# tkwa/iit

Hardware: AMD Instinct MI355X
Metric: IIT (base,source) intervened pairs/sec, IOI GPT-2-small, IOI_ModelPair IIT+strict+behavior step (higher is better)
Workload: dtype bf16; 1 GPU; model=gpt2-small 12L/768d/12H (TL GPT-2 cfg, LNPre, gelu_new, V=50257), global_batch=256, seq_len=16, parallelism=dp1, engine=native, graphs=True

## Files before the change

### csrc/ioi_hl.hip

```cpp
#include "common.h"

namespace {

constexpr int MAXS = 64;

__global__ __launch_bounds__(64) void ioi_hl_label_kernel(const long* __restrict__ base, const long* __restrict__ src,
                                                          const float* __restrict__ name_table, int table_n, int B,
                                                          int S, int V, int node, long* __restrict__ label) {
  __shared__ long tok_s[MAXS], dtok_s[MAXS], key_s[2 * MAXS];
  __shared__ float d_s[2 * MAXS];
  const int b = blockIdx.x, lane = threadIdx.x;
  const long* tb = base + (long)b * S;
  const long* ts = src + (long)b * S;
  const long* tok = (node == 0 || node == 3) ? ts : tb;
  const long* dtok = (node == 1 || node == 2) ? ts : tok;
  if (lane < S) {
    tok_s[lane] = tok[lane];
    dtok_s[lane] = dtok[lane];
  }
  __syncthreads();
  if (lane < S) {
    int dup = -1;
    for (int j = 0; j < lane; ++j)
      if (dtok_s[j] == dtok_s[lane]) dup = j;
    const long inh = dup == -1 ? -1 : (node == 1 ? tok_s[lane] : dtok_s[lane]);
    const long v = tok_s[lane];
    key_s[lane] = v;
    d_s[lane] = (v >= 0 && v < table_n && name_table[v] != 0.f) ? 10.f : 0.f;
    key_s[S + lane] = inh != -1 ? inh : (long)(V - 1);
    d_s[S + lane] = inh != -1 ? -15.f : 0.f;
  }
  __syncthreads();
  const int n = 2 * S;
  float my_val = -INFINITY, my_zero_key = INFINITY;
  long my_key = -1;
  for (int e = lane; e < n; e += 64) {
    const long k = key_s[e];
    float sum = 0.f;
    for (int f = 0; f < n; ++f)
      if (key_s[f] == k) sum += d_s[f];
    if (sum > my_val || (sum == my_val && k < my_key)) {
      my_val = sum;
      my_key = k;
    }
    if (sum == 0.f) my_zero_key = fminf(my_zero_key, (float)k);
  }
  float untouched = INFINITY;
  for (int u = lane; u <= n; u += 64) {
    bool hit = false;
    for (int f = 0; f < n; ++f) hit |= key_s[f] == (long)u;
    if (!hit) untouched = fminf(untouched, (float)u);
  }
  for (int off = 32; off > 0; off >>= 1) {
    const float ov = __shfl_xor(my_val, off);
    const long ok = __shfl_xor(my_key, off);
    if (ov > my_val || (ov == my_val && ok >= 0 && (my_key < 0 || ok < my_key))) {
      my_val = ov;
      my_key = ok;
    }
    my_zero_key = fminf(my_zero_key, __shfl_xor(my_zero_key, off));
    untouched = fminf(untouched, __shfl_xor(untouched, off));
  }
  if (lane == 0) {
    long out;
    if (my_val > 0.f) {
      out = my_key;
    } else {
      out = (long)untouched;
      if (my_zero_key < untouched) out = (long)my_zero_key;
    }
    label[b] = out;
  }
}

}

IIT_EXPORT int iit_ioi_hl_label(const void* base, const void* src, const float* name_table, int table_n, int B, int S,
                                int V, int node, void* label, void* stream) {
  if (S < 1 || S > MAXS || node < 0 || node > 3 || V <= 2 * S) return (int)hipErrorInvalidValue;
  hipLaunchKernelGGL(ioi_hl_label_kernel, dim3(B), dim3(64), 0, (hipStream_t)stream,
                     (const long*)base, (const long*)src, name_table, table_n, B, S, V, node, (long*)label);
  return hipGetLastError();
}
```

### csrc/kernels.hip

```cpp
#include "common.h"
#include <stdlib.h>

__global__ void embed_pos_fwd_kernel(const long* __restrict__ tok, const float* __restrict__ WE,
                                     const float* __restrict__ Wpos, float* __restrict__ out, int T, int S, int d) {
  const int t = blockIdx.x;
  if (t >= T) return;
  const long v = tok[t];
  const int s = t % S;
  const float4* e = (const float4*)(WE + v * (long)d);
  const float4* p = (const float4*)(Wpos + (long)s * d);
  float4* o = (float4*)(out + (long)t * d);
  for (int i = threadIdx.x; i < d / 4; i += blockDim.x) {
    float4 a = e[i], b = p[i];
    o[i] = make_float4(a.x + b.x, a.y + b.y, a.z + b.z, a.w + b.w);
  }
}

__global__ void embed_pos_fwd_scalar_kernel(const long* __restrict__ tok, const float* __restrict__ WE,
                                            const float* __restrict__ Wpos, float* __restrict__ out, int T, int S,
                                            int d) {
  const int t = blockIdx.x;
  if (t >= T) return;
  const float* e = WE + tok[t] * (long)d;
  const float* p = Wpos + (long)(t % S) * d;
  float* o = out + (long)t * d;
  for (int i = threadIdx.x; i < d; i += blockDim.x) o[i] = e[i] + p[i];
}

IIT_EXPORT int iit_embed_pos_fwd(const long* tok, const float* WE, const float* Wpos, float* out, int T, int S,
                                 int d, void* stream) {
  if (d % 4 == 0 && ((((uintptr_t)WE) | ((uintptr_t)Wpos) | ((uintptr_t)out)) & 15) == 0)
    hipLaunchKernelGGL(embed_pos_fwd_kernel, dim3(T), dim3(64), 0, (hipStream_t)stream, tok, WE, Wpos, out, T, S, d);
  else
    hipLaunchKernelGGL(embed_pos_fwd_scalar_kernel, dim3(T), dim3(256), 0, (hipStream_t)stream, tok, WE, Wpos, out,
                       T, S, d);
  return hipGetLastError();
}

__global__ void embed_bwd_kernel(const long* __restrict__ tok, const float* __restrict__ g, float* __restrict__ dWE,
                                 int T, int d) {
  const int t = blockIdx.x;
  const long v = tok[t];
  for (int i = threadIdx.x; i < d; i += blockDim.x) atomicAdd(dWE + v * (long)d + i, g[(long)t * d + i]);
}

constexpr int EB = 32;
__global__ __launch_bounds__(256) void embed_bwd_pos_kernel(const long* __restrict__ tok, const float* __restrict__ g,
                                                            float* __restrict__ dWE, int B, int S, int d) {
  const int s = blockIdx.x, c = blockIdx.y * 256 + threadIdx.x, b0 = blockIdx.z * EB;
  if (c >= d) return;
  const int b1 = min(B, b0 + EB);
  long cur = -1;
  float acc = 0.f;
  for (int bb = b0; bb < b1; bb += 8) {
    long vv[8];
    float xx[8];
#pragma unroll
    for (int k = 0; k < 8; ++k) {
      const int b = bb + k;
      vv[k] = -1;
      xx[k] = 0.f;
      if (b < b1) {
        const long t = (long)b * S + s;
        vv[k] = tok[t];
        xx[k] = g[t * d + c];
      }
    }
#pragma unroll
    for (int k = 0; k < 8; ++k) {
      if (vv[k] < 0) break;
      if (vv[k] != cur) {
        if (cur >= 0) atomicAdd(dWE + cur * (long)d + c, acc);
        cur = vv[k];
        acc = xx[k];
      } else {
        acc += xx[k];
      }
    }
  }
  if (cur >= 0) atomicAdd(dWE + cur * (long)d + c, acc);
}

__global__ __launch_bounds__(256) void pos_bwd_kernel(const float* __restrict__ g, float* __restrict__ dWpos, int B,
                                                      int S, int d) {
  __shared__ float part[4][64 * 4];
  const int s = blockIdx.x, w = threadIdx.x >> 6, lane = threadIdx.x & 63;
  const int c = blockIdx.y * 256 + lane * 4;
  float4 acc = make_float4(0.f, 0.f, 0.f, 0.f);
  if (c < d)
#pragma unroll 8
    for (int b = w; b < B; b += 4) {
      const float4 v = *(const float4*)(g + ((long)b * S + s) * d + c);
      acc.x += v.x; acc.y += v.y; acc.z += v.z; acc.w += v.w;
    }
  *(float4*)&part[w][lane * 4] = acc;
  __syncthreads();
  const int col = blockIdx.y * 256 + threadIdx.x;
  if (col < d)
    dWpos[(long)s * d + col] += part[0][threadIdx.x] + part[1][threadIdx.x] + part[2][threadIdx.x] + part[3][threadIdx.x];
}

__global__ void pos_bwd_scalar_kernel(const float* __restrict__ g, float* __restrict__ dWpos, int B, int S, int d) {
  const int s = blockIdx.x;
  for (int i = threadIdx.x; i < d; i += blockDim.x) {
    float acc = 0.f;
    for (int b = 0; b < B; ++b) acc += g[((long)b * S + s) * d + i];
    dWpos[(long)s * d + i] += acc;
  }
}

IIT_EXPORT int iit_embed_pos_bwd(const long* tok, const float* g, float* dWE, float* dWpos, int B, int S, int d,
                                 void* stream) {
  hipStream_t st = (hipStream_t)stream;
  static const bool pos_major = [] {
    const char* e = getenv("IIT_EMBED_BWD_POS");
    return !(e && e[0] == '0');
  }();
  if (dWE && pos_major)
    hipLaunchKernelGGL(embed_bwd_pos_kernel, dim3(S, (d + 255) / 256, (B + EB - 1) / EB), dim3(256), 0, st, tok, g,
                       dWE, B, S, d);
  else if (dWE)
    hipLaunchKernelGGL(embed_bwd_kernel, dim3(B * S), dim3(256), 0, st, tok, g, dWE, B * S, d);
  if (dWpos) {
    if (d % 4 == 0 && (((uintptr_t)g) & 15) == 0)
      hipLaunchKernelGGL(pos_bwd_kernel, dim3(S, (d + 255) / 256), dim3(256), 0, st, g, dWpos, B, S, d);
    else
      hipLaunchKernelGGL(pos_bwd_scalar_kernel, dim3(S), dim3(256), 0, st, g, dWpos, B, S, d);
  }
  return hipGetLastError();
}

constexpr size_t kAttnSmallLdsMax = 160 * 1024;
__global__ __launch_bounds__(64) void attn_small_fwd_kernel(const __bf16* __restrict__ qkv, __bf16* __restrict__ z,
                                                            float* __restrict__ lse, const __bf16* __restrict__ zsrc,
                                                            unsigned long long head_mask, int B, int S, int H, int dh,
                                                            long ld_qkv, long ld_z, long ld_src, float scale, int causal) {
  extern __shared__ __attribute__((aligned(16))) float sm[];
  const int bh = blockIdx.x, b = bh / H, h = bh % H;
  const int lane = threadIdx.x;
  const int HD = H * dh;
  const long row0 = (long)b * S;
  if ((head_mask >> h) & 1ull) {
    for (int i = lane; i < S * dh; i += 64) {
      const int s = i / dh, e = i % dh;
      z[(row0 + s) * ld_z + h * dh + e] = zsrc[(row0 + s) * ld_src + h * dh + e];
    }
    if (lse)
      for (int s = lane; s < S; s += 64) lse[(long)bh * S + s] = 0.f;
    return;
  }
  const int P = dh + 1;
  float* q = sm;
  float* k = q + S * P;
  float* v = k + S * P;
  float* pr = v + S * P;
  for (int i = lane; i < S * dh; i += 64) {
    const int s = i / dh, e = i % dh;
    const __bf16* r = qkv + (row0 + s) * ld_qkv + h * dh + e;
    q[s * P + e] = bf2f(r[0]);
    k[s * P + e] = bf2f(r[HD]);
    v[s * P + e] = bf2f(r[2 * HD]);
  }
  __syncthreads();
  const int SP = S + 1;
  for (int i = lane; i < S * S; i += 64) {
    const int qi = i / S, kj = i % S;
    float acc = -INFINITY;
    if (!causal || kj <= qi) {
      acc = 0.f;
      for (int e = 0; e < dh; ++e) acc += q[qi * P + e] * k[kj * P + e];
      acc *= scale;
    }
    pr[qi * SP + kj] = acc;
  }
  __syncthreads();
  for (int qi = lane; qi < S; qi += 64) {
    float m = -INFINITY;
    for (int kj = 0; kj < S; ++kj) m = fmaxf(m, pr[qi * SP + kj]);
    float sum = 0.f;
    for (int kj = 0; kj < S; ++kj) {
      const float e = pr[qi * SP + kj] == -INFINITY ? 0.f : __expf(pr[qi * SP + kj] - m);
      pr[qi * SP + kj] = e;
      sum += e;
    }
    const float inv = sum > 0.f ? 1.f / sum : 0.f;
    for (int kj = 0; kj < S; ++kj) pr[qi * SP + kj] *= inv;
    if (lse) lse[(long)bh * S + qi] = m + __logf(sum);
  }
  __syncthreads();
  for (int i = lane; i < S * dh; i += 64) {
    const int qi = i / dh, e = i % dh;
    float acc = 0.f;
    const int kmax = causal ? qi + 1 : S;
    for (int kj = 0; kj < kmax; ++kj) acc += pr[qi * SP + kj] * v[kj * P + e];
    z[(row0 + qi) * ld_z + h * dh + e] = f2bf(acc);
  }
}

IIT_EXPORT int iit_attn_small_fwd(const void* qkv, void* z, float* lse, const void* zsrc, unsigned long long head_mask,
                                  int B, int S, int H, int dh, long ld_qkv, long ld_z, long ld_src, float scale,
                                  int causal, void* stream) {
  if (S > 64 || dh > 128) return (int)hipErrorInvalidValue;
  const size_t lds = (size_t)(3 * S * (dh + 1) + S * (S + 1)) * sizeof(float);
  if (lds > kAttnSmallLdsMax) return (int)hipErrorInvalidValue;
  hipLaunchKernelGGL(attn_small_fwd_kernel, dim3(B * H), dim3(64), lds, (hipStream_t)stream, (const __bf16*)qkv,
                     (__bf16*)z, lse, (const __bf16*)zsrc, head_mask, B, S, H, dh, ld_qkv, ld_z, ld_src, scale, causal);
  return hipGetLastError();
}

__global__ __launch_bounds__(64) void attn_small_bwd_kernel(const __bf16* __restrict__ qkv, const __bf16* __restrict__ dz,
                                                            const float* __restrict__ lse, __bf16* __restrict__ dqkv,
                                                            unsigned long long head_mask, int B, int S, int H, int dh,
                                                            long ld_qkv, long ld_dz, float scale, int causal) {
  extern __shared__ __attribute__((aligned(16))) float sm[];
  const int bh = blockIdx.x, b = bh / H, h = bh % H;
  const int lane = threadIdx.x;
  const int HD = H * dh;
  const long row0 = (long)b * S;
  if ((head_mask >> h) & 1ull) {
    for (int i = lane; i < S * dh; i += 64) {
      const int s = i / dh, e = i % dh;
      __bf16* r = dqkv + (row0 + s) * ld_qkv + h * dh + e;
      r[0] = f2bf(0.f);
      r[HD] = f2bf(0.f);
      r[2 * HD] = f2bf(0.f);
    }
    return;
  }
  const int P = dh + 1, SP = S + 1;
  float* q = sm;
  float* k = q + S * P;
  float* v = k + S * P;
  float* g = v + S * P;
  float* pm = g + S * P;
  float* ds = pm + S * SP;
  for (int i = lane; i < S * dh; i += 64) {
    const int s = i / dh, e = i % dh;
    const __bf16* r = qkv + (row0 + s) * ld_qkv + h * dh + e;
    q[s * P + e] = bf2f(r[0]);
    k[s * P + e] = bf2f(r[HD]);
    v[s * P + e] = bf2f(r[2 * HD]);
    g[s * P + e] = bf2f(dz[(row0 + s) * ld_dz + h * dh + e]);
  }
  __syncthreads();
  for (int i = lane; i < S * S; i += 64) {
    const int qi = i / S, kj = i % S;
    float p = 0.f, dp = 0.f;
    if (!causal || kj <= qi) {
      float sc = 0.f;
      for (int e = 0; e < dh; ++e) sc += q[qi * P + e] * k[kj * P + e];
      p = __expf(sc * scale - lse[(long)bh * S + qi]);
      for (int e = 0; e < dh; ++e) dp += g[qi * P + e] * v[kj * P + e];
    }
    pm[qi * SP + kj] = p;
    ds[qi * SP + kj] = dp;
  }
  __syncthreads();
  for (int qi = lane; qi < S; qi += 64) {
    float dsum = 0.f;
    for (int kj = 0; kj < S; ++kj) dsum += pm[qi * SP + kj] * ds[qi * SP + kj];
    for (int kj = 0; kj < S; ++kj) ds[qi * SP + kj] = pm[qi * SP + kj] * (ds[qi * SP + kj] - dsum) * scale;
  }
  __syncthreads();
  for (int i = lane; i < S * dh; i += 64) {
    const int s = i / dh, e = i % dh;
    float dq = 0.f, dk = 0.f, dv = 0.f;
    for (int j = 0; j < S; ++j) {
      dq += ds[s * SP + j] * k[j * P + e];
      dk += ds[j * SP + s] * q[j * P + e];
      dv += pm[j * SP + s] * g[j * P + e];
    }
    __bf16* r = dqkv + (row0 + s) * ld_qkv + h * dh + e;
    r[0] = f2bf(dq);
    r[HD] = f2bf(dk);
    r[2 * HD] = f2bf(dv);
  }
}

IIT_EXPORT int iit_attn_small_bwd(const void* qkv, const void* dz, const float* lse, void* dqkv,
                                  unsigned long long head_mask, int B, int S, int H, int dh, long ld_qkv, long ld_dz,
                                  float scale, int causal, void* stream) {
  if (S > 64 || dh > 128) return (int)hipErrorInvalidValue;
  const size_t lds = (size_t)(4 * S * (dh + 1) + 2 * S * (S + 1)) * sizeof(float);
  if (lds > kAttnSmallLdsMax) return (int)hipErrorInvalidValue;
  hipLaunchKernelGGL(attn_small_bwd_kernel, dim3(B * H), dim3(64), lds, (hipStream_t)stream, (const __bf16*)qkv,
                     (const __bf16*)dz, lse, (__bf16*)dqkv, head_mask, B, S, H, dh, ld_qkv, ld_dz, scale, causal);
  return hipGetLastError();
}

__device__ __forceinline__ void online_add(float& m, float& s, int& mi, float v, int i) {
  if (v > m) {
    s = s * __expf(m - v) + 1.f;
    m = v;
    mi = i;
  } else if (v != -INFINITY) {
    s += __expf(v - m);
  }
}

__device__ __forceinline__ void online_merge(float& m, float& s, int& mi, float om, float os, int oi) {
  if (om > m || (om == m && oi < mi)) {
    s = os + (m == -INFINITY ? 0.f : s * __expf(m - om));
    m = om;
    mi = oi;
  } else {
    s += (om == -INFINITY ? 0.f : os * __expf(om - m));
  }
}

__global__ __launch_bounds__(1024) void ce_fwd_kernel(const float* __restrict__ logits, long ld, const long* __restrict__ labels,
                                                      float* __restrict__ loss, float* __restrict__ lse_out,
                                                      long* __restrict__ amax, int V) {
  __shared__ float sm_m[16], sm_s[16];
  __shared__ int sm_i[16];
  const int row = blockIdx.x, tid = threadIdx.x, lane = tid & 63, w = tid >> 6;
  const float* x = logits + (long)row * ld;
  float m = -INFINITY, s = 0.f;
  int mi = 0x7fffffff;
  int head = 0;
  if ((((uintptr_t)x) & 15) == 0) {
    const int v4 = V / 4;
    for (int i = tid; i < v4; i += 1024) {
      const float4 q = ((const float4*)x)[i];
      online_add(m, s, mi, q.x, 4 * i);
      online_add(m, s, mi, q.y, 4 * i + 1);
      online_add(m, s, mi, q.z, 4 * i + 2);
      online_add(m, s, mi, q.w, 4 * i + 3);
    }
    head = v4 * 4;
  }
  for (int i = head + tid; i < V; i += 1024) online_add(m, s, mi, x[i], i);
#pragma unroll
  for (int o = 32; o > 0; o >>= 1) {
    const float om = __shfl_xor(m, o, 64), os = __shfl_xor(s, o, 64);
    const int oi = __shfl_xor(mi, o, 64);
    online_merge(m, s, mi, om, os, oi);
  }
  if (lane == 0) { sm_m[w] = m; sm_s[w] = s; sm_i[w] = mi; }
  __syncthreads();
  if (tid == 0) {
    for (int j = 1; j < 16; ++j) online_merge(m, s, mi, sm_m[j], sm_s[j], sm_i[j]);
    const float l = m + __logf(s);
    if (lse_out) lse_out[row] = l;
    if (loss && labels) loss[row] = l - x[labels[row]];
    if (amax) amax[row] = mi;
  }
}

IIT_EXPORT int iit_ce_fwd(const float* logits, long ld, const long* labels, float* loss, float* lse, long* amax, int R,
                          int V, void* stream) {
  hipLaunchKernelGGL(ce_fwd_kernel, dim3(R), dim3(1024), 0, (hipStream_t)stream, logits, ld, labels, loss, lse, amax, V);
  return hipGetLastError();
}

template <typename OUT>
__global__ __launch_bounds__(256) void ce_bwd_kernel(const float* __restrict__ logits, long ld, const long* __restrict__ labels,
                                                     const float* __restrict__ lse, const float* __restrict__ gscale,
                                                     float inv_rows, OUT* __restrict__ out, long ld_out, int V,
                                                     __bf16* __restrict__ out16) {
  const int row = blockIdx.y;
  const int i = blockIdx.x * 256 + threadIdx.x;
  if (i >= ld_out) return;
  float v = 0.f;
  if (i < V) {
    const float p = __expf(logits[(long)row * ld + i] - lse[row]);
    v = (p - (i == labels[row] ? 1.f : 0.f)) * gscale[0] * inv_rows;
  }
  out[(long)row * ld_out + i] = (OUT)v;
  if (out16) out16[(long)row * ld_out + i] = f2bf(v);
}

IIT_EXPORT int iit_ce_bwd(const float* logits, long ld, const long* labels, const float* lse, const float* gscale,
                          float inv_rows, void* out, long ld_out, int R, int V, int out_bf16, void* out16,
                          void* stream) {
  dim3 grid((unsigned)((ld_out + 255) / 256), R);
  if (out_bf16)
    hipLaunchKernelGGL(ce_bwd_kernel<__bf16>, grid, dim3(256), 0, (hipStream_t)stream, logits, ld, labels, lse, gscale,
                       inv_rows, (__bf16*)out, ld_out, V, (__bf16*)nullptr);
  else
    hipLaunchKernelGGL(ce_bwd_kernel<float>, grid, dim3(256), 0, (hipStream_t)stream, logits, ld, labels, lse, gscale,
                       inv_rows, (float*)out, ld_out, V, (__bf16*)out16);
  return hipGetLastError();
}

template <bool VEC>
__global__ __launch_bounds__(256) void ce_bwd16_kernel(const float* __restrict__ logits, long ld,
                                                       const long* __restrict__ labels, const float* __restrict__ lse,
                                                       const float* __restrict__ gscale, float inv_rows,
                                                       __bf16* __restrict__ out16, long ld_out, int V) {
  const int row = blockIdx.y;
  const int c0 = (blockIdx.x * 256 + threadIdx.x) * 8;
  if (c0 >= ld_out) return;
  const float* x = logits + (long)row * ld;
  const float l = lse[row], gs = gscale[0];
  const long lab = labels[row];
  float v[8];
  if (VEC && c0 + 8 <= V) {
    const float4 a = *(const float4*)(x + c0), b = *(const float4*)(x + c0 + 4);
    v[0] = a.x; v[1] = a.y; v[2] = a.z; v[3] = a.w; v[4] = b.x; v[5] = b.y; v[6] = b.z; v[7] = b.w;
  } else {
#pragma unroll
    for (int e = 0; e < 8; ++e) v[e] = c0 + e < V ? x[c0 + e] : 0.f;
  }
  bf16x8 o;
#pragma unroll
  for (int e = 0; e < 8; ++e) {
    const int i = c0 + e;
    float g = 0.f;
    if (i < V) {
      const float p = __expf(v[e] - l);
      g = (p - (i == lab ? 1.f : 0.f)) * gs * inv_rows;
    }
    o[e] = f2bf(g);
  }
  *(bf16x8*)(out16 + (long)row * ld_out + c0) = o;
}

IIT_EXPORT int iit_ce_bwd16(const float* logits, long ld, const long* labels, const float* lse, const float* gscale,
                            float inv_rows, void* out16, long ld_out, int R, int V, void* stream) {
  if (R <= 0 || V <= 0 || ld < V || ld_out < V || ld_out % 8 || ((uintptr_t)out16 & 15)) return (int)hipErrorInvalidValue;
  dim3 grid((unsigned)((ld_out / 8 + 255) / 256), R);
  const bool vec = (((uintptr_t)logits | (uintptr_t)(ld * 4)) & 15) == 0;
  if (vec)
    hipLaunchKernelGGL(ce_bwd16_kernel<true>, grid, dim3(256), 0, (hipStream_t)stream, logits, ld, labels, lse, gscale,
                       inv_rows, (__bf16*)out16, ld_out, V);
  else
    hipLaunchKernelGGL(ce_bwd16_kernel<false>, grid, dim3(256), 0, (hipStream_t)stream, logits, ld, labels, lse,
                       gscale, inv_rows, (__bf16*)out16, ld_out, V);
  return hipGetLastError();
}

struct Span {
  long start4;
  long local4;
  int len4;
  int pad;
};

__global__ __launch_bounds__(256) void sumsq_span_kernel(const float* __restrict__ g, const Span* __restrict__ spans,
                                                         int nspans, float* __restrict__ part, int do_norm,
                                                         int* __restrict__ step, float* __restrict__ gsq) {
  __shared__ float sm[4];
  if (blockIdx.x == 0 && threadIdx.x == 0 && step) step[0] += 1;
  float s = 0.f;
  if (gsq && blockIdx.x == 0 && threadIdx.x < 64) {
    s = gsq[threadIdx.x];
    gsq[threadIdx.x] = 0.f;
  }
  if (!do_norm) return;
  const float4* g4 = (const float4*)g;
  for (int e = blockIdx.x; e < nspans; e += gridDim.x) {
    const Span sp = spans[e];
    for (int i = threadIdx.x; i < sp.len4; i += 256) {
      const float4 v = g4[sp.local4 + i];
      s += (v.x * v.x + v.y * v.y) + (v.z * v.z + v.w * v.w);
    }
  }
  s = wave_sum(s);
  if ((threadIdx.x & 63) == 0) sm[threadIdx.x >> 6] = s;
  __syncthreads();
  if (threadIdx.x == 0) part[blockIdx.x] = sm[0] + sm[1] + sm[2] + sm[3];
}

template <bool NT, int U>
__global__ __launch_bounds__(256) void adam_span_kernel(float* __restrict__ p, const float* __restrict__ g,
                                                        float* __restrict__ m, float* __restrict__ v,
                                                        __bf16* __restrict__ mirror, const Span* __restrict__ spans,
                                                        int nspans, const float* __restrict__ part, int nparts,
                                                        float clip, float lr, float b1, float b2, float eps, float wd,
                                                        const float* __restrict__ hyper, int* __restrict__ step,
                                                        int* __restrict__ skipped) {
  if (hyper) {
    lr = hyper[0];
    b1 = hyper[1];
    b2 = hyper[2];
    eps = hyper[3];
    wd = hyper[4];
  }
  __shared__ float coef_s;
  __shared__ int bad_s;
  if (threadIdx.x < 64) {
    float s = 0.f;
    if (clip > 0.f || skipped)
      for (int i = threadIdx.x; i < nparts; i += 64) s += part[i];
    s = wave_sum(s);
    if (threadIdx.x == 0) {
      coef_s = clip > 0.f ? fminf(1.f, clip / (sqrtf(s) + 1e-6f)) : 1.f;
      bad_s = skipped != nullptr && !isfinite(s);
    }
  }
  __syncthreads();
  if (bad_s) {
    if (blockIdx.x == 0 && threadIdx.x == 0) {
      step[0] -= 1;
      skipped[0] += 1;
    }
    return;
  }
  const float coef = coef_s;
  const float t = (float)step[0];
  const float bc1 = 1.f - powf(b1, t);
  const float bc2_sqrt = sqrtf(1.f - powf(b2, t));
  const float stepsz = lr / bc1;
  const float4* g4 = (const float4*)g;
  float4* p4 = (float4*)p;
  float4* m4 = (float4*)m;
  float4* v4 = (float4*)v;
  for (int e = blockIdx.x; e < nspans; e += gridDim.x) {
    const Span sp = spans[e];
    for (int j0 = threadIdx.x; j0 < sp.len4; j0 += 256 * U) {
      float4 gg[U], pp[U], mm[U], vv[U];
#pragma unroll
      for (int u = 0; u < U; ++u) {
        const int j = j0 + u * 256;
        if (j < sp.len4) {
          const long i = sp.start4 + j;
          const long li = sp.local4 + j;
          pp[u] = p4[i];
          if (NT) {
            gg[u] = __builtin_bit_cast(float4, __builtin_nontemporal_load((const f32x4*)g4 + li));
            mm[u] = __builtin_bit_cast(float4, __builtin_nontemporal_load((const f32x4*)m4 + li));
            vv[u] = __builtin_bit_cast(float4, __builtin_nontemporal_load((const f32x4*)v4 + li));
          } else {
            gg[u] = g4[li];
            mm[u] = m4[li];
            vv[u] = v4[li];
          }
        }
      }
#pragma unroll
      for (int u = 0; u < U; ++u) {
        const int j = j0 + u * 256;
        if (j >= sp.len4) break;
        const long i = sp.start4 + j;
        const long li = sp.local4 + j;
        float* gs = (float*)&gg[u];
        float* ps = (float*)&pp[u];
        float* ms = (float*)&mm[u];
        float* vs = (float*)&vv[u];
#pragma unroll
        for (int k = 0; k < 4; ++k) {
          float gr = gs[k] * coef;
          if (wd != 0.f) gr += wd * ps[k];
          ms[k] = b1 * ms[k] + (1.f - b1) * gr;
          vs[k] = b2 * vs[k] + (1.f - b2) * gr * gr;
          ps[k] -= stepsz * ms[k] / (sqrtf(vs[k]) / bc2_sqrt + eps);
        }
        p4[i] = pp[u];
        if (NT) {
          __builtin_nontemporal_store(__builtin_bit_cast(f32x4, mm[u]), (f32x4*)m4 + li);
          __builtin_nontemporal_store(__builtin_bit_cast(f32x4, vv[u]), (f32x4*)v4 + li);
        } else {
          m4[li] = mm[u];
          v4[li] = vv[u];
        }
        if (mirror) {
          bf16x4 o = {f2bf(ps[0]), f2bf(ps[1]), f2bf(ps[2]), f2bf(ps[3])};
          ((bf16x4*)mirror)[i] = o;
        }
      }
    }
  }
}

IIT_EXPORT int iit_adam_flat(float* p, float* g, float* m, float* v, void* mirror, const void* spans, int nspans,
                             float* part, int nparts, float clip, float lr, float b1, float b2, float eps, float wd,
                             const float* hyper, int* step, int* skipped, const void* sq_spans, int n_sq_spans,
                             float* gsq, void* stream) {
  hipStream_t s = (hipStream_t)stream;
  const bool norm = clip > 0.f || skipped != nullptr;
  const Span* sp = (const Span*)spans;
  const Span* ssp = sq_spans ? (const Span*)sq_spans : sp;
  hipLaunchKernelGGL(sumsq_span_kernel, dim3(norm ? nparts : 1), dim3(256), 0, s, g, ssp,
                     sq_spans ? n_sq_spans : nspans, part, (int)norm, step, gsq);
  static const int max_blocks = [] {
    const char* e = getenv("IIT_ADAM_MAX_BLOCKS");
    return e ? atoi(e) : 65536;
  }();
  const int blocks = min(nspans, max_blocks);
  static const int nt = [] {
    const char* e = getenv("IIT_ADAM_NT");
    return e ? atoi(e) : 1;
  }();
  static const int unroll = [] {
    const char* e = getenv("IIT_ADAM_UNROLL");
    return e ? atoi(e) : 4;
  }();
#define ADAM_LAUNCH(NT_, U_)                                                                                        \
  hipLaunchKernelGGL((adam_span_kernel<NT_, U_>), dim3(blocks), dim3(256), 0, s, p, g, m, v, (__bf16*)mirror, sp, \
                     nspans, part, nparts, clip, lr, b1, b2, eps, wd, hyper, step, skipped)
  if (nt) {
    if (unroll >= 4) ADAM_LAUNCH(true, 4);
    else if (unroll == 2) ADAM_LAUNCH(true, 2);
    else ADAM_LAUNCH(true, 1);
  } else {
    if (unroll >= 4) ADAM_LAUNCH(false, 4);
    else if (unroll == 2) ADAM_LAUNCH(false, 2);
    else ADAM_LAUNCH(false, 1);
  }
#undef ADAM_LAUNCH
  return hipGetLastError();
}

IIT_EXPORT int iit_adam_span_size() { return (int)sizeof(Span); }

__global__ __launch_bounds__(256) void sumsq_2d_kernel(const float* __restrict__ c, long ldc, int M, int N,
                                                       float* __restrict__ gsq) {
  __shared__ float sm[4];
  const int chunks = (N + 2047) / 2048;
  float s = 0.f;
  for (long it = blockIdx.x; it < (long)M * chunks; it += gridDim.x) {
    const int r = (int)(it / chunks), c0 = (int)(it % chunks) * 2048;
    const float* row = c + (long)r * ldc;
    float v[8];
#pragma unroll
    for (int k = 0; k < 8; ++k) {
      const int j = c0 + k * 256 + threadIdx.x;
      v[k] = j < N ? row[j] : 0.f;
    }
#pragma unroll
    for (int k = 0; k < 8; ++k) s += v[k] * v[k];
  }
  s = wave_sum(s);
  if ((threadIdx.x & 63) == 0) sm[threadIdx.x >> 6] = s;
  __syncthreads();
  if (threadIdx.x == 0) atomicAdd(gsq + (blockIdx.x & 63), (sm[0] + sm[1]) + (sm[2] + sm[3]));
}

IIT_EXPORT int iit_sumsq_2d(const float* c, long ldc, int M, int N, float* gsq, void* stream) {
  const long items = (long)M * ((N + 2047) / 2048);
  hipLaunchKernelGGL(sumsq_2d_kernel, dim3((unsigned)(items < 2048 ? items : 2048)), dim3(256), 0,
                     (hipStream_t)stream, c, ldc, M, N, gsq);
  return hipGetLastError();
}

IIT_EXPORT int iit_sumsq_spans(const float* g, const void* spans, int nspans, float* part, int nparts, int do_norm,
                               int* step, void* stream) {
  hipLaunchKernelGGL(sumsq_span_kernel, dim3(do_norm ? nparts : 1), dim3(256), 0, (hipStream_t)stream, g,
                     (const Span*)spans, nspans, part, do_norm, step, (float*)nullptr);
  return hipGetLastError();
}

IIT_EXPORT int iit_adam_spans(float* p, const float* g, float* m, float* v, void* mirror, const void* spans,
                              int nspans, const float* total, float clip, float lr, float b1, float b2, float eps,
                              float wd, const float* hyper, int* step, int* skipped, void* stream) {
  const int blocks = max(1, min(nspans, 65536));
  hipLaunchKernelGGL((adam_span_kernel<true, 2>), dim3(blocks), dim3(256), 0, (hipStream_t)stream, p, g, m, v,
                     (__bf16*)mirror, (const Span*)spans, nspans, total, 1, clip, lr, b1, b2, eps, wd, hyper, step,
                     skipped);
  return hipGetLastError();
}

struct ShadowDesc {
  const float* src;
  __bf16* dst;
  int rows, cols;
  long ld;
  int heads;
  int transpose;
  long src_hs, dst_hs;
};

__global__ __launch_bounds__(256) void shadow_refresh_kernel(const ShadowDesc* __restrict__ descs) {
  __shared__ float tile[32][33];
  const ShadowDesc d = descs[blockIdx.y];
  if (!d.transpose) {
    const long total = (long)d.heads * d.rows;
    for (long r = blockIdx.x; r < total; r += gridDim.x) {
      const int h = (int)(r / d.rows), i = (int)(r % d.rows);
      const float* s = d.src + h * d.src_hs + (long)i * d.cols;
      __bf16* o = d.dst + h * d.dst_hs + (long)i * d.ld;
      const bool vec = ((((uintptr_t)s) & 15) == 0) && ((((uintptr_t)o) & 7) == 0);
      if (vec) {
        const int c4 = d.cols / 4;
        for (int j = threadIdx.x; j < c4; j += 256) {
          const float4 v = ((const float4*)s)[j];
          bf16x4 b = {f2bf(v.x), f2bf(v.y), f2bf(v.z), f2bf(v.w)};
          *(bf16x4*)(o + 4 * j) = b;
        }
        for (int j = c4 * 4 + threadIdx.x; j < d.cols; j += 256) o[j] = f2bf(s[j]);
      } else {
        for (int j = threadIdx.x; j < d.cols; j += 256) o[j] = f2bf(s[j]);
      }
    }
    return;
  }
  const int tiles_c = (d.cols + 31) / 32;
  const int ntiles = tiles_c * ((d.rows + 31) / 32);
  const int tx = threadIdx.x & 31, ty = threadIdx.x >> 5;
  for (int t = blockIdx.x; t < ntiles; t += gridDim.x) {
    const int r0 = (t / tiles_c) * 32, c0 = (t % tiles_c) * 32;
    {
      for (int i = ty; i < 32; i += 8) {
        const int r = r0 + i, c = c0 + tx;
        tile[i][tx] = (r < d.rows && c < d.cols) ? d.src[(long)r * d.cols + c] : 0.f;
      }
      __syncthreads();
      for (int i = ty; i < 32; i += 8) {
        const int c = c0 + i, r = r0 + tx;
        if (r < d.rows && c < d.cols) d.dst[(long)c * d.ld + r] = f2bf(tile[tx][i]);
      }
      __syncthreads();
    }
  }
}

IIT_EXPORT int iit_shadow_refresh(const void* descs, int n, void* stream) {
  if (n <= 0) return 0;
  hipLaunchKernelGGL(shadow_refresh_kernel, dim3(512, n), dim3(256), 0, (hipStream_t)stream, (const ShadowDesc*)descs);
  return hipGetLastError();
}

IIT_EXPORT int iit_shadow_desc_size() { return (int)sizeof(ShadowDesc); }

template <bool F32>
__global__ __launch_bounds__(256) void colsum_kernel(const void* __restrict__ x, long ld, float* __restrict__ out, int T, int N) {
  __shared__ float part[4][64];
  const int c = threadIdx.x & 63, w = threadIdx.x >> 6;
  const int n = blockIdx.x * 64 + c;
  const int t0 = blockIdx.y * 64;
  float s = 0.f;
  if (n < N) {
#pragma unroll 4
    for (int i = 0; i < 16; ++i) {
      const int t = t0 + w + 4 * i;
      if (t < T) s += F32 ? ((const float*)x)[(long)t * ld + n] : bf2f(((const __bf16*)x)[(long)t * ld + n]);
    }
  }
  part[w][c] = s;
  __syncthreads();
  if (w == 0 && n < N) atomicAdd(out + n, part[0][c] + part[1][c] + part[2][c] + part[3][c]);
// ... 410 lines not shown
```

### iit_amd/data/iit_dataset.py

```python
from __future__ import annotations

from typing import Iterator, Optional, Sequence, Tuple

import numpy as np
import torch
from torch.utils.data import DataLoader, Dataset, Subset

from ..config import DEVICE


def _gather_fn(ds):
    if hasattr(ds, "gather"):
        return ds.gather
    if isinstance(ds, Subset):
        inner = _gather_fn(ds.dataset)
        if inner is None:
            return None
        table = torch.as_tensor(list(ds.indices), dtype=torch.long)
        cache = {}

        def f(idx, _inner=inner, _table=table, _cache=cache):
            dev = idx.device
            t = _cache.get(dev)
            if t is None:
                t = _cache[dev] = _table.to(dev)
            return _inner(t.index_select(0, idx))

        return f
    return None


def _dist_info() -> Tuple[int, int]:
    if torch.distributed.is_available() and torch.distributed.is_initialized():
        return torch.distributed.get_rank(), torch.distributed.get_world_size()
    return 0, 1


def loader_epoch_permutation(n: int) -> torch.Tensor:
    torch.empty((), dtype=torch.int64).random_()
    seed = int(torch.empty((), dtype=torch.int64).random_().item())
    g = torch.Generator()
    g.manual_seed(seed)
    return torch.randperm(n, generator=g)


class IITDataset(Dataset):
    def __init__(self, base_data, ablation_data, seed: int = 0, every_combination: bool = False, device=DEVICE):
        self.base_data = base_data
        self.ablation_data = ablation_data
        self.seed = seed
        self.every_combination = every_combination
        self.device = device
        self._pair_table: Optional[Tuple[np.ndarray, np.ndarray]] = None

    def pair_indices(self, index: int) -> Tuple[int, int]:
        if self.every_combination:
            n_abl = len(self.ablation_data)
            return index // n_abl, index % n_abl
        rng = np.random.default_rng(self.seed * 1000000 + index)
        base = rng.choice(len(self.base_data))
        abl = rng.choice(len(self.ablation_data))
        return int(base), int(abl)

    def pair_table(self) -> Tuple[np.ndarray, np.ndarray]:
        if self._pair_table is None:
            n = len(self)
            if self.every_combination:
                idx = np.arange(n)
                n_abl = len(self.ablation_data)
                self._pair_table = (idx // n_abl, idx % n_abl)
            else:
                pairs = np.array([self.pair_indices(i) for i in range(n)], dtype=np.int64).reshape(n, 2)
                self._pair_table = (pairs[:, 0], pairs[:, 1])
        return self._pair_table

    def __getitem__(self, index):
        b, a = self.pair_indices(index)
        return self.base_data[b], self.ablation_data[a]

    def __len__(self) -> int:
        if self.every_combination:
            return len(self.base_data) * len(self.ablation_data)
        return len(self.base_data)

    @staticmethod
    def get_encoded_input_from_torch_input(xy, device=DEVICE):
        x, y, iv = zip(*xy)
        stack = lambda seq: torch.stack([torch.as_tensor(s).to(device) for s in seq])
        return stack(x), stack(y), stack(iv)

    @staticmethod
    def collate_fn(batch, device=DEVICE):
        base, abl = zip(*batch)
        return (IITDataset.get_encoded_input_from_torch_input(base, device),
                IITDataset.get_encoded_input_from_torch_input(abl, device))

    def supports_device_loader(self) -> bool:
        return _gather_fn(self.base_data) is not None and _gather_fn(self.ablation_data) is not None

    def make_loader(self, batch_size: int, num_workers: int = 0, shuffle: bool = True, fast: Optional[bool] = None):
        if fast is None:
            fast = self.supports_device_loader()
        if fast:
            return DeviceIITLoader(self, batch_size, shuffle=shuffle)
        return DataLoader(self, batch_size=batch_size, shuffle=shuffle, num_workers=num_workers,
                          collate_fn=lambda b: self.collate_fn(b, self.device))


class DeviceIITLoader:

    def __init__(self, dataset: IITDataset, batch_size: int, shuffle: bool = True, drop_last: bool = False,
                 device=None):
        self.dataset = dataset
        self.batch_size = batch_size
        self.shuffle = shuffle
        self.drop_last = drop_last
        self.rank, self.world = _dist_info()
        self.device = torch.device(device) if device is not None else torch.device(dataset.device)
        self._base_gather = _gather_fn(dataset.base_data)
        self._abl_gather = _gather_fn(dataset.ablation_data)
        self._unique = isinstance(dataset, IITUniqueDataset)
        self._tables = None

    def _device_tables(self):
        if self._tables is None:
            if self._unique:
                self._tables = (None, None)
            else:
                b, a = self.dataset.pair_table()
                self._tables = (torch.as_tensor(b).to(self.device), torch.as_tensor(a).to(self.device))
        return self._tables

    @property
    def global_batch(self) -> int:
        return self.batch_size * self.world

    def __len__(self) -> int:
        n = len(self.dataset)
        gb = self.global_batch
        if self.drop_last or (self.world > 1 and 0 < n % gb < self.world):
            return n // gb
        return (n + gb - 1) // gb

    def __iter__(self) -> Iterator:
        n = len(self.dataset)
        perm = loader_epoch_permutation(n) if self.shuffle else torch.arange(n)
        if self.device.type == "cuda":
            perm = perm.pin_memory().to(self.device, non_blocking=True)
        else:
            perm = perm.to(self.device)
        base_t, abl_t = self._device_tables()
        gb = self.global_batch
        for start in range(0, n, gb):
            chunk = perm[start:start + gb]
            if chunk.numel() < gb and self.drop_last:
                break
            if self.world > 1:
                if chunk.numel() < self.world:
                    break
                chunk = torch.tensor_split(chunk, self.world)[self.rank]
            if self._unique:
                yield self._base_gather(chunk)
            else:
                yield (self._base_gather(base_t.index_select(0, chunk)),
                       self._abl_gather(abl_t.index_select(0, chunk)))


class IITUniqueDataset(IITDataset):

    def __getitem__(self, index):
        return self.base_data[index]

    def __len__(self) -> int:
        return len(self.base_data)

    @staticmethod
    def collate_fn(batch, device=DEVICE):
        return IITDataset.get_encoded_input_from_torch_input(batch, device)

    def supports_device_loader(self) -> bool:
        return _gather_fn(self.base_data) is not None

    def make_loader(self, batch_size: int, num_workers: int = 0, shuffle: bool = True, fast: Optional[bool] = None):
        if fast is None:
            fast = self.supports_device_loader()
        if fast:
            return DeviceIITLoader(self, batch_size, shuffle=shuffle)
        return DataLoader(self, batch_size=batch_size, shuffle=shuffle, num_workers=num_workers,
                          collate_fn=lambda b: self.collate_fn(b, self.device))


def train_test_split(dataset, test_size: float = 0.2, random_state: Optional[int] = None):
    n = len(dataset)
    split = int(n * test_size)
    if random_state is None:
        return torch.utils.data.random_split(dataset, [n - split, split])
    return torch.utils.data.random_split(dataset, [n - split, split],
                                         generator=torch.Generator().manual_seed(random_state))
```

### iit_amd/engine/graphs.py

```python
from __future__ import annotations

import os
from typing import Dict, Optional, Tuple

import torch

from ..utils.tracing import sync_point, trace_range


_CAPTURE_MODE = "thread_local"
_SYNC_BEFORE_REPLAY = os.environ.get("IIT_GRAPH_SYNC_BEFORE_REPLAY") == "1"
_RECAPTURE_ALL = os.environ.get("IIT_GRAPH_RECAPTURE_ALL") == "1"


def _join_gathers(optimizer) -> None:
    wait = getattr(optimizer, "wait_gathers", None)
    if wait is not None:
        wait()


def _sync_gemm_decisions() -> None:
    from ..ops.gemm_dispatch import sync_decisions
    sync_decisions()


def _sync_hyper(optimizer) -> None:
    sync = getattr(optimizer, "sync_hyper", None)
    if sync is not None:
        sync()
    _join_gathers(optimizer)


def _clone_out(out):
    if isinstance(out, tuple):
        loss, extras = out
        ts = [loss] + list(extras.values())
        if all(t.dim() == 0 and t.dtype == loss.dtype and t.device == loss.device for t in ts):
            vals = torch.stack(ts).unbind(0)
            return vals[0], dict(zip(extras.keys(), vals[1:]))
        return loss.clone(), {k: v.clone() for k, v in extras.items()}
    return out.clone()


def _detach_out(out):
    if isinstance(out, tuple):
        loss, extras = out
        return loss.detach(), {k: v.detach() for k, v in extras.items()}
    return out.detach()



_FOREACH_COPY = os.environ.get("IIT_FOREACH_COPY", "1") != "0"


def _copy_all(dst, src) -> None:
    if _FOREACH_COPY:
        try:
            torch._foreach_copy_(list(dst), list(src), non_blocking=True)
            return
        except (RuntimeError, TypeError, AttributeError):
            pass
    for d, s_ in zip(dst, src):
        d.copy_(s_, non_blocking=True)

class _CaptureGC:

    def __init__(self, collect: bool = True):
        self.collect = collect

    def __enter__(self):
        import gc
        if self.collect:
            gc.collect()
        self._was = gc.isenabled()
        gc.disable()
        return self

    def __exit__(self, *exc):
        import gc
        if self._was:
            gc.enable()
        return False


def _fused_backend(pair) -> bool:
    module = pair._ll_module() if hasattr(pair, "_ll_module") else getattr(pair, "ll_model", None)
    ops = getattr(module, "ops", None)
    try:
        return bool(getattr(ops() if callable(ops) else ops, "fused", False))
    except Exception:
        return False


class _TrainState:

    def __init__(self, pair, optimizer):
        import copy
        _join_gathers(optimizer)
        ll = pair._ll_module() if hasattr(pair, "_ll_module") else pair.ll_model
        flat = getattr(ll, "_flat_params", None)
        self.ll, self.flat = ll, flat
        self.pairs = []
        if flat is not None:
            self.pairs.append((flat.data, flat.data.clone()))
            if flat.shadow is not None:
                self.pairs.append((flat.shadow, flat.shadow.clone()))
        else:
            self.pairs += [(p.data, p.data.clone()) for p in ll.parameters()]
        self.pairs += [(b, b.clone()) for b in ll.buffers() if b is not None]
        self.opt = optimizer
        self.scalars = {}
        if optimizer is not None and hasattr(optimizer, "exp_avg"):
            for t in (optimizer.exp_avg, optimizer.exp_avg_sq, optimizer._step_dev, optimizer._skipped_dev):
                if t is not None:
                    self.pairs.append((t, t.clone()))
            self.scalars = {"step_count": optimizer.step_count}
        elif optimizer is not None:
            self.opt_state = {}
            for p, st in optimizer.state.items():
                saved = {}
                for k, v in st.items():
                    if torch.is_tensor(v):
                        self.pairs.append((v, v.clone()))
                    else:
                        saved[k] = copy.deepcopy(v)
                self.opt_state[p] = (set(st.keys()), saved)
        self.cpu_rng = torch.get_rng_state()
        self.cuda_rng = torch.cuda.get_rng_state() if torch.cuda.is_available() else None

    @torch.no_grad()
    def restore(self) -> None:
        opt = self.opt
        _join_gathers(opt)
        for live, saved in self.pairs:
            live.copy_(saved)
        for k, v in self.scalars.items():
            setattr(opt, k, v)
        if opt is not None and hasattr(self, "opt_state"):
            for p, st in opt.state.items():
                if p not in self.opt_state:
                    for k, v in st.items():
                        if torch.is_tensor(v):
                            v.zero_()
                        elif isinstance(v, (int, float)):
                            st[k] = type(v)(0)
            for p, (keys, saved) in self.opt_state.items():
                st = opt.state[p]
                for k in list(st.keys()):
                    if k not in keys:
                        del st[k]
                st.update(saved)
        torch.set_rng_state(self.cpu_rng)
        if self.cuda_rng is not None:
            torch.cuda.set_rng_state(self.cuda_rng)
        if self.flat is not None:
            self.flat.after_step(mirror_written=self.flat.shadow is not None)
        elif hasattr(self.ll, "mark_weights_changed"):
            self.ll.mark_weights_changed()


class TrainStateSnapshot(_TrainState):

    def __init__(self, pair, optimizer):
        import copy
        super().__init__(pair, optimizer)
        self.pair = pair
        self.pair_rng = copy.deepcopy(getattr(pair, "rng", None))

    @torch.no_grad()
    def restore(self) -> None:
        import copy
        super().restore()
        if self.flat is not None:
            self.flat.refresh_shadow()
        if self.pair_rng is not None:
            self.pair.rng = copy.deepcopy(self.pair_rng)


class GraphedTrainStep:
    def __init__(self, pair, optimizer=None, loss_fn=None, warmup: int = 1, enabled: Optional[bool] = None):
        self.pair = pair
        self.optimizer = optimizer
        self.loss_fn = loss_fn
        self.warmup = warmup
        ws = torch.distributed.get_world_size() if (torch.distributed.is_available()
                                                   and torch.distributed.is_initialized()) else 1
        if enabled is None:
            enabled = torch.cuda.is_available()
            if ws > 1 and os.environ.get("IIT_GRAPHS_DP", "1") == "0":
                enabled = False
        self.enabled = enabled
        from ..parallel.dist import force_reducer
        self.split = ws > 1 or force_reducer()
        self.staged = None
        self.force_staged = False
        if self.split and enabled:
            from .staged import staged_for
            self.staged = staged_for(pair)
            reducer = getattr(pair, "_reducer", None)
            if self.staged is not None and reducer is not None:
                reducer.segment_buckets(self.staged.edges)
        self.graphs: Dict[Tuple, Tuple[torch.cuda.CUDAGraph, object]] = {}
        self.seen: Dict[Tuple, int] = {}
        self.pool = None
        mode = os.environ.get("IIT_GRAPH_STREAM", "auto")
        dedicated = mode == "1" or (mode == "auto" and not _fused_backend(pair))
        self.stream = torch.cuda.Stream() if (enabled and torch.cuda.is_available() and dedicated) else None
        if enabled:
            from ..ops.gemm_dispatch import select_graph_safe_blas
            select_graph_safe_blas()
        self._static = None
        self._sig = None
        self.captures = 0
        self.replays = 0
        self.calls = 0
        self.failed: Dict[Tuple, str] = {}
        pair._phase_runner = self._run_phase

    def _stage(self, base, abl):
        if not self.enabled:
            return base, abl, True
        sig = tuple((tuple(t.shape), t.dtype, t.device) for t in tuple(base) + tuple(abl))
        if self._static is None:
            self._static = (tuple(t.clone() for t in base), tuple(t.clone() for t in abl))
            self._sig = sig
            return self._static[0], self._static[1], False
        if sig != self._sig:
            return base, abl, True
        sb, sa = self._static
        _copy_all(sb + sa, tuple(base) + tuple(abl))
        return sb, sa, False

    @staticmethod
    def _eager(compute_loss, optimizer, step_fn):
        out = compute_loss()
        loss = out[0] if isinstance(out, tuple) else out
        step_fn(loss, optimizer)
        return _detach_out(out)

    def _splittable(self, step_fn) -> bool:
        from ..model_pairs.iit_behavior_model_pair import IITBehaviorModelPair
        return getattr(step_fn, "__func__", None) is IITBehaviorModelPair.step_on_loss

    def _run_split_phase(self, full, key, compute_loss, optimizer):
        pair = self.pair
        reducer = getattr(pair, "_reducer", None)
        stg = self.staged if (reducer is not None and reducer.enabled) or self.force_staged else None

        def fwd_bwd():
            if stg is not None:
                stg.arm()
            try:
                out = compute_loss()
            finally:
                if stg is not None:
                    stg.disarm()
            loss = out[0] if isinstance(out, tuple) else out
            optimizer.zero_grad()
            if reducer is not None:
                reducer.paused = True
            try:
                loss.backward()
            finally:
                if reducer is not None:
                    reducer.paused = False
            return _detach_out(out)

        def update():
            pair.clip_grad_fn(optimizer)
            pair.optimizer_step(optimizer)

        def reduce_eagerly(run_stage):
            if reducer is None:
                for i, k in enumerate(stg.stages() if stg is not None else ()):
                    run_stage(i, k)
                return
            reducer.start()
            reducer.paused = True
            try:
                if stg is None:
                    reducer.launch_range(0, reducer.flat.numel)
                else:
                    rng = stg.ranges()
                    reducer.launch_range(*rng[0])
                    for i, k in enumerate(stg.stages()):
                        run_stage(i, k)
                        reducer.launch_range(*rng[i + 1])
            finally:
                reducer.paused = False
            reducer.finish()

        def eager_phase():
            out = fwd_bwd()
            reduce_eagerly(lambda i, k: stg.run_stage(k))
            if stg is not None:
                stg.release()
            update()
            return out

        ent = self.graphs.get(full)
        if ent is None:
            n = self.seen.get(full, 0)
            if n < self.warmup or full in self.failed:
                self.seen[full] = n + 1
                return eager_phase()
            if self.pool is None or os.environ.get("IIT_GRAPH_POOL") == "private":
                self.pool = torch.cuda.graph_pool_handle()
            ga, gb = torch.cuda.CUDAGraph(), torch.cuda.CUDAGraph()
            parts = None
            if getattr(optimizer, "sharded", False):
                gb = None
                clip = self.pair.training_args.get("clip_grad_norm") or None
                spec = optimizer.step_parts(clip_norm=clip) if hasattr(optimizer, "step_parts") else None
                if spec is not None:
                    parts = [(torch.cuda.CUDAGraph() if cap else None, fn) for cap, fn in spec]
            gs = []
            _join_gathers(optimizer)
            _sync_gemm_decisions()
            try:
                with _CaptureGC(), torch.cuda.graph(ga, pool=self.pool, stream=self.stream, capture_error_mode=_CAPTURE_MODE):
                    static_out = fwd_bwd()
                for k in (stg.stages() if stg is not None else ()):
                    g = torch.cuda.CUDAGraph()
                    with _CaptureGC(), torch.cuda.graph(g, pool=self.pool, stream=self.stream, capture_error_mode=_CAPTURE_MODE):
                        stg.run_stage(k)
                    gs.append(g)
                if stg is not None:
                    stg.release()
                if gb is not None:
                    with _CaptureGC(), torch.cuda.graph(gb, pool=self.pool, stream=self.stream,
                                                        capture_error_mode=_CAPTURE_MODE):
                        update()
                elif parts is not None:
                    for g_, fn in parts:
                        if g_ is not None:
                            with _CaptureGC(), torch.cuda.graph(g_, pool=self.pool, stream=self.stream,
                                                                capture_error_mode=_CAPTURE_MODE):
                                fn()
            except Exception as e:
                self.failed[full] = repr(e)
                self.pool = None
                print(f"[iit graphs] DP phase {key} not captured ({type(e).__name__}: {str(e)[:160]}); eager")
                torch.cuda.synchronize()
                if stg is not None:
                    stg.release()
                return eager_phase()
            ent = self.graphs[full] = ((ga, gs, gb, parts), static_out)
            self.captures += 1
        (ga, gs, gb, parts), static_out = ent
        _sync_hyper(optimizer)
        with trace_range("graph:fwd_bwd"):
            ga.replay()
        sync_point()
        with trace_range("grad_allreduce"):
            reduce_eagerly(lambda i, k: gs[i].replay())
        sync_point()
        with trace_range("graph:clip_adam"):
            if gb is not None:
                gb.replay()
            elif parts is not None:
                self.pair.clip_grad_fn(optimizer)
                optimizer.pending_clip = None
                for g_, fn in parts:
                    if g_ is not None:
                        g_.replay()
                    else:
                        fn()
            else:
                update()
        sync_point()
        self.replays += 1
        return _clone_out(static_out)

    def _graph_key(self, key, optimizer=None):
        module = self.pair._ll_module() if hasattr(self.pair, "_ll_module") else getattr(self.pair, "ll_model", None)
        training = bool(getattr(module, "training", True))
        opt = optimizer if optimizer is not None else self.optimizer
        flat = getattr(opt, "flat", None)
        rv = getattr(flat, "restrict_version", 0) if flat is not None else 0
        return (key, self._sig, training, rv)

    def _run_phase(self, key, compute_loss, optimizer, step_fn):
        full = self._graph_key(key, optimizer)
        if not self.enabled or self._current_eager:
            return self._eager(compute_loss, optimizer, step_fn)
        if self.split:
            if not self._splittable(step_fn):
                return self._eager(compute_loss, optimizer, step_fn)
            return self._run_split_phase(full, key, compute_loss, optimizer)
        ent = self.graphs.get(full)
        if ent is None:
            n = self.seen.get(full, 0)
            if n < self.warmup:
                self.seen[full] = n + 1
                return self._eager(compute_loss, optimizer, step_fn)
            if full in self.failed:
                return self._eager(compute_loss, optimizer, step_fn)
            if self.pool is None or os.environ.get("IIT_GRAPH_POOL") == "private":
                self.pool = torch.cuda.graph_pool_handle()
            g = torch.cuda.CUDAGraph()
            _join_gathers(optimizer)
            try:
                with _CaptureGC(), torch.cuda.graph(g, pool=self.pool, stream=self.stream, capture_error_mode=_CAPTURE_MODE):
                    out = compute_loss()
                    loss = out[0] if isinstance(out, tuple) else out
                    step_fn(loss, optimizer)
                    static_out = _detach_out(out)
            except Exception as e:
                self.failed[full] = repr(e)
                self.pool = None
                import traceback
                tb = "".join(traceback.format_exc(limit=12)) if len(self.failed) == 1 else ""
                print(f"[iit graphs] phase {key} not captured ({type(e).__name__}: {str(e)[:160]}); "
                      f"running it eagerly\n{tb}")
                torch.cuda.synchronize()
                return self._eager(compute_loss, optimizer, step_fn)
            if _RECAPTURE_ALL:
                self.graphs.clear()
            ent = self.graphs[full] = (g, static_out)
            self.captures += 1
        g, static_out = ent
        _sync_hyper(optimizer)
        if _SYNC_BEFORE_REPLAY:
            torch.cuda.current_stream().synchronize()
        with trace_range("graph:phase"):
            g.replay()
        sync_point()
        self.replays += 1
        return _clone_out(static_out)

    def __call__(self, base_input, ablation_input, loss_fn=None, optimizer=None):
        loss_fn = loss_fn or self.loss_fn
        optimizer = optimizer or self.optimizer
        self.calls += 1
        if self.stream is None or torch.cuda.current_stream() == self.stream:
            return self._step(base_input, ablation_input, loss_fn, optimizer)
        if not self._handoff_warned:
            self._handoff_warned = True
            print("[iit graphs] train step called from another stream: run the loop (and any evaluation between "
                  "steps) inside `with step.stream_context():` -- mixing streams between captured phases and other "
                  "work has been seen to corrupt later replays (scripts/diag_graph_node.py)")
        cur = torch.cuda.current_stream()
        self.stream.wait_stream(cur)
        for t in tuple(base_input) + tuple(ablation_input):
            if isinstance(t, torch.Tensor) and t.is_cuda:
                t.record_stream(self.stream)
        try:
            with torch.cuda.stream(self.stream):
                return self._step(base_input, ablation_input, loss_fn, optimizer)
        finally:
            cur.wait_stream(self.stream)

    def _step(self, base_input, ablation_input, loss_fn, optimizer):
        sb, sa, eager = self._stage(base_input, ablation_input)
        self._current_eager = eager
        try:
            return self.pair.run_train_step(sb, sa, loss_fn, optimizer)
        finally:
            self._current_eager = False

    _current_eager = False
    _handoff_warned = False

    def stream_context(self):
        import contextlib
        if self.stream is None:
            return contextlib.nullcontext()

        @contextlib.contextmanager
        def ctx():
            cur = torch.cuda.current_stream()
            self.stream.wait_stream(cur)
            try:
                with torch.cuda.stream(self.stream):
                    yield
            finally:
                cur.wait_stream(self.stream)
        return ctx()

    def prime(self, base_input, ablation_input, loss_fn=None, optimizer=None) -> int:
        import copy
        pair = self.pair
        rng_state = copy.deepcopy(pair.rng)
        hl_nodes = list(pair.corr.keys())
        ll_nodes = list(getattr(pair, "nodes_not_in_circuit", []) or [None])
        orig_hl = pair.__dict__.get("sample_hl_name")
        orig_ll = pair.__dict__.get("sample_ll_node")
        try:
            n = max(len(hl_nodes), len(ll_nodes))
            for rep in range(self.warmup + 1):
                for i in range(n):
                    pair.sample_hl_name = lambda i=i: hl_nodes[i % len(hl_nodes)]
                    if ll_nodes[0] is not None:
                        pair.sample_ll_node = lambda i=i: ll_nodes[i % len(ll_nodes)]
                    self(base_input, ablation_input, loss_fn, optimizer)
        finally:
            for name, orig in (("sample_hl_name", orig_hl), ("sample_ll_node", orig_ll)):
                if orig is None:
                    pair.__dict__.pop(name, None)
                else:
                    setattr(pair, name, orig)
            pair.rng = rng_state
        return self.captures

    def prime_preserving(self, base_input, ablation_input, loss_fn=None, optimizer=None) -> int:
        optimizer = optimizer or self.optimizer
        if not self.enabled:
            return 0
        snap = _TrainState(self.pair, optimizer)
        try:
            return self.prime(base_input, ablation_input, loss_fn, optimizer)
        finally:
            snap.restore()

    def detach(self) -> None:
        if getattr(self.pair, "_phase_runner", None) == self._run_phase:
            self.pair._phase_runner = None
        self.graphs.clear()


class GraphedEvalStep:

    def __init__(self, pair, loss_fn, warmup: int = 1, stream=None):
        self.pair = pair
        self.loss_fn = loss_fn
        self.warmup = warmup
        self.stream = stream
        self.graphs: Dict[Tuple, Tuple[torch.cuda.CUDAGraph, dict]] = {}
        self.seen: Dict[Tuple, int] = {}
        self.failed: Dict[Tuple, str] = {}
        self.pool = None
        self._static = None
        self._sig = None
# ... 73 lines not shown
```

### iit_amd/model_pairs/base_model_pair.py

```python
from __future__ import annotations

from abc import ABC, abstractmethod
from typing import Any, Callable, Dict, Iterable, List, Optional, Tuple, final

import numpy as np
import torch
from torch import Tensor

from ..config import WANDB_ENTITY
from ..core.correspondence import Correspondence
from ..core.index import EVERYTHING, Ix, TorchIndex
from ..core.metric import MetricStoreCollection, MetricType
from ..core.nodes import HLNode, HookName, LLNode
from ..data.iit_dataset import IITDataset
from ..engine.plan import RunPlan
from ..hooks.hook_points import ActivationCache, HookPoint
from ..parallel import dist as pdist
from ..utils.progress import progress
from ..utils.sinks import make_sink
from ..utils.tracing import StepTimer, sync_point, trace_range


def _is_native(model) -> bool:
    return getattr(model, "supports_run_plan", False) or hasattr(model, "run_capture")
# ... 20 lines not shown
    except Exception:
        return None
    if isinstance(x, (tuple, list)):
        x = x[0]
    if isinstance(x, Tensor) and x.dim() == 1 and not x.dtype.is_floating_point:
        return int(x.shape[0])
    return None


def _ll_nodes_of(corr, hl_node) -> List[LLNode]:
    v = corr[hl_node]
    if isinstance(v, LLNode):
        return [v]
    return sorted(v, key=lambda n: (n.name, repr(n.index)))


class BaseModelPair(ABC):
    hl_model: Any
    ll_model: Any
    hl_cache: Any
    ll_cache: Any
    corr: Correspondence
    training_args: Dict[str, Any]
    wandb_method: str
    rng: np.random.Generator
    dataset_class = IITDataset

    @property
    @abstractmethod
    def loss_fn(self) -> Callable[[Tensor, Tensor], Tensor]:
        ...

    @staticmethod
    @abstractmethod
    def make_train_metrics() -> MetricStoreCollection:
        ...

    @staticmethod
    @abstractmethod
    def make_test_metrics() -> MetricStoreCollection:
        ...

    @abstractmethod
    def run_train_step(self, base_input, ablation_input, loss_fn, optimizer) -> Dict[str, Any]:
        ...

    @abstractmethod
    def run_eval_step(self, base_input, ablation_input, loss_fn) -> Dict[str, Any]:
        ...

    def hl_run_kwargs(self) -> Dict[str, Any]:
        return {}

    def ll_logits_mode(self) -> str:
        return "full"

    def native(self) -> bool:
        return self.training_args.get("engine", "native") != "reference" and _is_native(self.ll_model)

    def ll_source_cache(self, x: Tensor, ll_nodes: Iterable[LLNode]):
        names = sorted({n.name for n in ll_nodes})
        model = self.ll_model
        if self.native():
            pf = getattr(self, "_source_prefetch", None)
            if pf is not None:
                cached = pf.lookup(x, names)
                if cached is not None:
                    return ActivationCache(cached, model)
            return ActivationCache(model.run_capture(x, names), model)
        _, cache = model.run_with_cache(x)
        return cache

    def ll_intervened_forward(self, x: Tensor, ll_nodes: Iterable[LLNode], logits: Optional[str] = None):
        logits = logits or self.ll_logits_mode()
        model = self.ll_model
        if self.native():
            plan = RunPlan.with_splices(
                [(n.name, n.index, self.ll_cache[n.name]) for n in ll_nodes], logits=logits)
            return model(x, plan=plan)
        out = model.run_with_hooks(x, fwd_hooks=[(n.name, self.make_ll_ablation_hook(n)) for n in ll_nodes])
        return out[:, -1] if logits == "last" and out.dim() == 3 else out

    def ll_intervention(self, base_x: Tensor, ablation_x: Tensor, ll_nodes: Iterable[LLNode]) -> Tensor:
        with trace_range("ll_paired_fwd"):
            ll_output = self.ll_paired_intervention(base_x, ablation_x, ll_nodes)
        if ll_output is None:
            with trace_range("ll_source_cache"):
                self.ll_cache = self.ll_source_cache(ablation_x, ll_nodes)
            sync_point()
            with trace_range("ll_spliced_fwd"):
                ll_output = self.ll_intervened_forward(base_x, ll_nodes)
        sync_point()
        return ll_output

    def ll_paired_intervention(self, base_x: Tensor, ablation_x: Tensor, ll_nodes: Iterable[LLNode],
                               logits: Optional[str] = None):
        if not self.native() or self.training_args.get("paired", True) is False:
            return None
        if getattr(self, "_source_prefetch", None) is not None:
            return None
        cls = type(self)
        if (cls.ll_intervened_forward is not BaseModelPair.ll_intervened_forward
                or cls.ll_source_cache is not BaseModelPair.ll_source_cache):
            return None
        fn = getattr(self.ll_model, "run_paired", None)
        if fn is None:
            return None
        sites = {}
        for n in ll_nodes:
            if n.subspace is not None:
                return None
            sites.setdefault(n.name, []).append(n.index)
        res = fn(base_x, ablation_x, sites, logits=logits or self.ll_logits_mode())
        if res is None:
            return None
        out, caps = res
        self.ll_cache = ActivationCache(caps, self.ll_model)
        return out

    def ll_forward(self, x: Tensor, logits: Optional[str] = None):
        logits = logits or self.ll_logits_mode()
        model = self.ll_model
        if logits in ("last", "argmax") and self.native():
            return model(x, plan=RunPlan(logits=logits))
        out = model(x)
        if logits == "argmax":
            return out.argmax(dim=-1)
        return out[:, -1] if logits == "last" and out.dim() == 3 else out

    def do_intervention(self, base_input, ablation_input, hl_node: HLNode, verbose: bool = False
                        ) -> Tuple[Tensor, Tensor]:
        ablation_x = ablation_input[0]
        base_x = base_input[0]
        hl_kw = self.hl_run_kwargs()
        with trace_range("hl_source_cache"):
            hl_ablation_output, self.hl_cache = self.hl_model.run_with_cache(ablation_input, **hl_kw)
        with trace_range("hl_intervened_fwd"):
            hl_output = self.hl_model.run_with_hooks(
                base_input, fwd_hooks=[(hl_node.name, self.make_hl_ablation_hook(hl_node))], **hl_kw)
        ll_nodes = _ll_nodes_of(self.corr, hl_node)
        ll_output = self.ll_intervention(base_x, ablation_x, ll_nodes)
        if verbose:
            print(f"{hl_node=}, {ll_nodes=}\n{hl_output=}")
        return hl_output, ll_output

    @staticmethod
    def get_label_idxs():
        return Ix[[None]]

    def make_hl_model(self, hl_graph):
        raise NotImplementedError

    def set_corr(self, corr):
        self.corr = corr

    def sample_hl_name(self) -> HLNode:
        return self.rng.choice(list(self.corr.keys()))

    def make_hl_ablation_hook(self, hl_node: HLNode):
        if not isinstance(hl_node, HLNode):
            raise AssertionError(f"hl_node is not an instance of HLNode, but {type(hl_node)}")
        if hl_node.index is None:
            return self.hl_ablation_hook
        index = hl_node.index

        def hl_ablation_hook(act: Tensor, hook: HookPoint) -> Tensor:
            src = self.hl_cache[hook.name]
            if isinstance(act, (int, float)):
                return src
            if index == EVERYTHING:
                return src.clone()
            out = act.clone()
            out[index.as_index] = src[index.as_index]
            return out

        return hl_ablation_hook

    def hl_ablation_hook(self, act: Tensor, hook: HookPoint) -> Tensor:
        return self.hl_cache[hook.name]

    def make_ll_ablation_hook(self, ll_node: LLNode) -> Callable[[Tensor, HookPoint], Tensor]:
        if ll_node.subspace is not None:
            raise NotImplementedError("subspace interventions are not supported")
        index = ll_node.index if ll_node.index is not None else EVERYTHING

        def ll_ablation_hook(act: Tensor, hook: HookPoint) -> Tensor:
            out = act.clone()
            out[index.as_index] = self.ll_cache[hook.name][index.as_index].to(out.dtype)
            return out

        return ll_ablation_hook

    def run_phase(self, key, compute_loss: Callable[[], Tensor], optimizer, step_fn):
        runner = getattr(self, "_phase_runner", None)
        if runner is not None:
            with trace_range(f"phase:{key[0]}"):
                return runner(key, compute_loss, optimizer, step_fn)
        out = compute_loss()
        if isinstance(out, tuple):
            loss, extras = out
            step_fn(loss, optimizer)
            return loss.detach(), {k: v.detach() for k, v in extras.items()}
        step_fn(out, optimizer)
        return out.detach()

    def get_IIT_loss_over_batch(self, base_input, ablation_input, hl_node: HookName, loss_fn):
        hl_output, ll_output = self.do_intervention(base_input, ablation_input, hl_node)
        return loss_fn(ll_output, hl_output)

    def _ll_module(self) -> torch.nn.Module:
        return _underlying_module(self.ll_model)

    def make_optimizer(self, lr: float):
        module = self._ll_module()
        fused = self.training_args.get("fused_optimizer", None)
        if fused is None:
            fused = next(module.parameters()).is_cuda
        if fused:
            from ..engine.flat import FlatParams
            from ..ops.optim import FusedAdam
            flat = getattr(module, "_flat_params", None)
            if flat is None:
                flat = FlatParams(module, with_bf16_shadow=getattr(module, "wants_bf16_shadow", False))
                module._flat_params = flat
            if self._zero_requested():
                from ..parallel.zero import ShardedFusedAdam
                opt = ShardedFusedAdam(flat, flat.buckets(int(self.training_args.get("bucket_mb", 64.0) * (1 << 20))),
                                       lr=lr)
                if self.training_args.get("zero_overlap_gather", True):
                    opt.attach_gates(module)
            else:
                opt = FusedAdam(flat, lr=lr)
        else:
            opt = torch.optim.Adam(module.parameters(), lr=lr)
        self._setup_reducer(opt)
        if fused:
            import os
            opt.flat.norm_fuse = ((self._reducer is None or pdist.world_size() == 1)
                                  and not getattr(opt, "sharded", False)
                                  and not self.rewrites_grads_before_step()
                                  and os.environ.get("IIT_FUSED_NORM", "1") != "0")
        return opt

    def sync_params(self) -> None:
        wait = getattr(getattr(self, "optimizer", None), "wait_gathers", None)
        if wait is not None:
            wait()

    def rewrites_grads_before_step(self) -> bool:
        return False

    def _zero_requested(self) -> bool:
        import os
        want = self.training_args.get("zero", os.environ.get("IIT_ZERO", "0") == "1")
        return bool(want) and (pdist.world_size() > 1 or pdist.force_reducer())

    def _setup_reducer(self, optimizer):
        self._reducer = None
        if pdist.world_size() > 1 or pdist.force_reducer():
            from ..engine.flat import FlatParams
            from ..parallel.ddp import GradReducer
            flat = getattr(optimizer, "flat", None)
            if flat is None:
                module = self._ll_module()
                flat = getattr(module, "_flat_params", None) or FlatParams(module)
                module._flat_params = flat
            wire = self.training_args.get("grad_wire_dtype")
            self._reducer = GradReducer(flat, bucket_mb=self.training_args.get("bucket_mb", 64.0),
                                        overlap=self.training_args.get("overlap_allreduce", True),
                                        wire_dtype={"bf16": torch.bfloat16, "fp32": torch.float32}.get(wire),
                                        module=self._ll_module())
            if getattr(optimizer, "sharded", False):
                self._reducer.attach_shard(optimizer)

    def restrict_sparse_rows(self, dataset, optimizer_rows: bool = True) -> None:
        module = self._ll_module()
        flat = getattr(module, "_flat_params", None)
        reducer = getattr(self, "_reducer", None)
        embed = getattr(getattr(module, "embed", None), "W_E", None)
        pos = getattr(getattr(module, "pos_embed", None), "W_pos", None)
        ids = dataset_token_ids(dataset) if dataset is not None else None
        seq = dataset_seq_len(dataset) if dataset is not None else None
        rows = []
        if embed is not None and ids is not None:
            rows.append((embed, ids))
        if pos is not None and seq is not None:
            rows.append((pos, torch.arange(min(seq, pos.shape[0]))))
        if dataset is None:
            rows = [(p, None) for p in (embed, pos) if p is not None]
        for p, r in rows:
            if reducer is not None and id(p) in reducer.flat.index and r is not None:
                reducer.set_row_subset(p, r.to(p.device))
            if optimizer_rows and flat is not None:
                flat.restrict_rows(p, r)

    def restrict_embedding_reduce(self, dataset) -> None:
        self.restrict_sparse_rows(dataset, optimizer_rows=False)

    def backward(self, loss: Tensor) -> None:
        reducer = getattr(self, "_reducer", None)
        if reducer is not None:
            reducer.start()
        with trace_range("backward"):
            loss.backward()
        sync_point()
        if reducer is not None:
            with trace_range("grad_allreduce"):
                reducer.finish()
            sync_point()
        module = self._ll_module()
        flat = getattr(module, "_flat_params", None)
        if flat is not None and not getattr(flat, "zeroes_missing_on_step", False):
            flat = None
        for p in module.parameters():
            if p.requires_grad and p.grad is None and not (flat is not None and flat.owns(p)):
                p.grad = torch.zeros_like(p)

    def clip_grad_fn(self, optimizer=None):
        max_norm = self.training_args.get("clip_grad_norm")
        if not max_norm:
            return
        if optimizer is not None and hasattr(optimizer, "flat"):
            optimizer.pending_clip = max_norm
            return
        from ..ops.optim import clip_grad_norm_
        clip_grad_norm_(list(self._ll_module().parameters()), max_norm)

    def optimizer_step(self, optimizer):
        clip = getattr(optimizer, "pending_clip", None)
        with trace_range("clip_adam"):
            if clip is not None and hasattr(optimizer, "flat"):
                optimizer.pending_clip = None
                optimizer.step(clip_norm=clip)
            else:
                optimizer.step()
        sync_point()

    def step_scheduler(self, lr_scheduler, test_metrics):
        if isinstance(lr_scheduler, torch.optim.lr_scheduler.ReduceLROnPlateau):
            val_metric = self.training_args.get("scheduler_val_metric", "val/accuracy")
            values = test_metrics.to_dict()
            if val_metric not in values:
                raise ValueError(f"val_metric {val_metric} not found in test_metrics {test_metrics}")
            lr_scheduler.step(values[val_metric])
            return
        try:
            lr_scheduler.step()
        except Exception as e:
            print(f"WARNING: Could not step lr_scheduler {lr_scheduler} with exception {e}")

    def train(self, train_set, test_set, epochs: int = 1000, use_wandb: bool = False,
              checkpoint_dir: Optional[str] = None, resume: bool = False, max_steps: Optional[int] = None,
              fault_hook: Optional[Callable[[int], None]] = None):
        training_args = self.training_args
        if pdist.is_main():
            print(f"{training_args=}")
        if not isinstance(train_set, IITDataset):
            raise AssertionError(f"train_set is not an instance of IITDataset, but {type(train_set)}")
        if not isinstance(test_set, IITDataset):
            raise AssertionError(f"test_set is not an instance of IITDataset, but {type(test_set)}")
        pdist.broadcast_module(self._ll_module())
        train_loader, test_loader = self.make_loaders(train_set, test_set, training_args["batch_size"],
                                                      training_args["num_workers"])
        early_stop = training_args["early_stop"]
        optimizer = self.make_optimizer(training_args["lr"])
        self.restrict_sparse_rows(train_set)
        loss_fn = self.loss_fn
        scheduler_cls = training_args.get("lr_scheduler", None)
        lr_scheduler = None
        if scheduler_cls == torch.optim.lr_scheduler.ReduceLROnPlateau:
            lr_scheduler = scheduler_cls(optimizer, mode=training_args.get("scheduler_mode", "max"),
                                         factor=0.1, patience=10)
        elif scheduler_cls:
            lr_scheduler = scheduler_cls(optimizer)
        sink = make_sink(use_wandb and pdist.is_main(), project="iit", entity=WANDB_ENTITY,
                         config={**{k: str(v) for k, v in training_args.items()}, "method": self.wandb_method})
        start_epoch = 0
        if checkpoint_dir and resume:
            from ..utils.checkpoint import load_resume_state
            start_epoch = load_resume_state(checkpoint_dir, self, optimizer, lr_scheduler)
        self.optimizer = optimizer
        self._prime_train_graphs(train_loader, loss_fn, optimizer)
        epoch = start_epoch
        for epoch in progress(range(start_epoch, epochs), disable=not pdist.is_main()):
            train_metrics = self._run_train_epoch(train_loader, loss_fn, optimizer, max_steps=max_steps)
            step = getattr(self, "_graph_step", None)
            import contextlib
            with (step.stream_context() if step is not None else contextlib.nullcontext()):
                test_metrics = self._run_eval_epoch(test_loader, loss_fn)
            self._reduce_metrics(train_metrics)
            self._reduce_metrics(test_metrics)
            if lr_scheduler is not None:
                self.step_scheduler(lr_scheduler, test_metrics)
            self.test_metrics = test_metrics
            self.train_metrics = train_metrics
            if pdist.is_main():
                self._print_and_log_metrics(epoch, train_metrics.metrics + test_metrics.metrics, sink)
                self._log_throughput(epoch, sink)
            if checkpoint_dir:
                from ..utils.checkpoint import save_resume_state
                save_resume_state(checkpoint_dir, self, optimizer, lr_scheduler, epoch + 1)
                pdist.barrier()
            if fault_hook is not None:
                fault_hook(epoch)
            if early_stop and self._check_early_stop_condition(test_metrics.metrics):
                break
        self.sync_params()
        self.restrict_sparse_rows(None)
        if sink is not None:
            sink.log({"final epoch": epoch})
            sink.close()

    def _prime_train_graphs(self, train_loader, loss_fn, optimizer) -> None:
        import os
        want = self.training_args.get("prime_graphs", None)
        if want is None:
            want = os.environ.get("IIT_PRIME_GRAPHS", "1") == "1"
        if not want:
            return
        step = self.train_step_fn(optimizer, loss_fn)
        if not hasattr(step, "prime_preserving"):
            return
        import time
        t0 = time.perf_counter()
        rng = torch.get_rng_state()
        try:
            base, abl = next(iter(train_loader))
        finally:
            torch.set_rng_state(rng)
        module = self._ll_module()
        was_training = module.training
        module.train()
        try:
            with step.stream_context():
                n = step.prime_preserving(base, abl, loss_fn, optimizer)
        finally:
            module.train(was_training)
        if torch.cuda.is_available():
            torch.cuda.synchronize()
        from ..utils import tracing
        if tracing.PROFILE and pdist.is_main():
            print(f"[perf] primed {n} phase graphs in {time.perf_counter() - t0:.2f} s before epoch 0")

    def _log_throughput(self, epoch: int, sink) -> None:
        tp = getattr(self, "throughput", None)
        if not tp:
            return
        if sink is not None:
            sink.log({"perf/pairs_per_s": tp["pairs_per_s"], "perf/ms_per_step": tp["ms_per_step"]})
        from ..utils import tracing
        if tracing.PROFILE:
            print(f"[perf] epoch {epoch}: {tp['ms_per_step']:.2f} ms/step, {tp['pairs_per_s']:.0f} pairs/s "
                  f"({int(tp['steps'])} timed steps, {pdist.world_size()} rank(s))")

    @final
    @staticmethod
    def make_loaders(dataset: IITDataset, test_dataset: IITDataset, batch_size: int, num_workers: int):
        return dataset.make_loader(batch_size, num_workers), test_dataset.make_loader(batch_size, num_workers)

    def train_step_fn(self, optimizer, loss_fn) -> Callable:
        runner = getattr(self, "_graph_step", None)
        if runner is not None and runner.optimizer is optimizer:
            return runner
        import os
        use = self.training_args.get("graphs", None)
        if use is None:
            module = self._ll_module()
            n_params = sum(p.numel() for p in module.parameters())
            use = (os.environ.get("IIT_GRAPHS", "1") != "0" and self.native()
                   and next(module.parameters()).is_cuda and n_params < 2_000_000_000)
        if use:
            from ..engine.graphs import GraphedTrainStep
            g = GraphedTrainStep(self, optimizer, loss_fn)
            if g.enabled:
                self._graph_step = g
                return g
        return self.run_train_step

    def _run_train_epoch(self, loader, loss_fn, optimizer, max_steps: Optional[int] = None) -> MetricStoreCollection:
        self._ll_module().train()
        metrics = self.make_train_metrics()
        step = self.train_step_fn(optimizer, loss_fn)
        import contextlib
        ctx = step.stream_context() if hasattr(step, "stream_context") else contextlib.nullcontext()
        timer = StepTimer(pdist.world_size())
        with ctx:
            for i, (base_input, ablation_input) in enumerate(progress(loader, total=len(loader),
                                                                      disable=not pdist.is_main(), leave=False)):
                timer.start()
                with trace_range("train_step"):
                    out = step(base_input, ablation_input, loss_fn, optimizer)
                timer.stop(len(base_input[0]))
                metrics.update(out)
                if max_steps is not None and i + 1 >= max_steps:
                    break
            self.throughput = timer.summary()
        return metrics

    def _run_eval_epoch(self, loader, loss_fn) -> MetricStoreCollection:
        self._ll_module().eval()
        metrics = self.make_test_metrics()
        from ..engine import prefetch
        use_prefetch = prefetch.supported(self)
        batches = prefetch.prefetched_batches(self, loader) if use_prefetch else loader
        step = self.eval_step_fn(loss_fn) if not use_prefetch else None
        with torch.no_grad(), trace_range("eval_epoch"):
            for base_input, ablation_input in batches:
                if step is not None:
                    metrics.update(step(base_input, ablation_input))
                else:
                    metrics.update(self.run_eval_step(base_input, ablation_input, loss_fn))
        return metrics

    def eval_step_fn(self, loss_fn):
        train_step = getattr(self, "_graph_step", None)
        if train_step is None or not self.training_args.get("eval_graphs", True):
            return None
        ev = getattr(self, "_graph_eval", None)
        if ev is None or ev.loss_fn is not loss_fn:
            from ..engine.graphs import GraphedEvalStep
            ev = self._graph_eval = GraphedEvalStep(self, loss_fn, stream=train_step.stream)
        return ev

    @staticmethod
    def _reduce_metrics(collection: MetricStoreCollection) -> None:
        if pdist.world_size() <= 1:
            return
        stores, parts = [], []
        for m in collection.metrics:
            if len(m) == 0:
                continue
            vals = np.stack([np.atleast_1d(np.asarray(v, dtype=np.float64)) for v in m._values()])
            stores.append((m, vals.shape[1]))
            parts.append(vals.sum(axis=0))
            parts.append(np.array([float(len(vals))]))
        if not parts:
            return
        flat = torch.tensor(np.concatenate(parts), dtype=torch.float64)
        if torch.distributed.get_backend() == "nccl":
            flat = flat.cuda()
        torch.distributed.all_reduce(flat, op=torch.distributed.ReduceOp.SUM)
        flat = flat.cpu().numpy()
        off = 0
        for m, n in stores:
            total, count = flat[off:off + n], flat[off + n]
            off += n + 1
            mean = total / count
            m._store = [mean if (m.type == MetricType.LOG) else float(mean[0])]

    @staticmethod
    def _check_early_stop_condition(test_metrics) -> bool:
        got = False
        for metric in test_metrics:
            if metric.type == MetricType.ACCURACY:
                got = True
                if metric.get_value() < 100:
                    return False
        if not got:
            raise ValueError("No accuracy metric found in test_metrics!")
        return True

    @staticmethod
    def _print_and_log_metrics(epoch, metrics, sink=None):
        line = ", ".join(str(m) for m in metrics)
        print(f"\nEpoch {epoch}: {line}")
        if sink is not None:
            sink.log({"epoch": epoch})
            for m in metrics:
                v = m.get_value()
                sink.log({m.get_name(): v.tolist() if isinstance(v, np.ndarray) else v})
```

### iit_amd/model_pairs/iit_behavior_model_pair.py

```python
from __future__ import annotations

import torch
from torch import Tensor

from ..core.metric import MetricStore, MetricStoreCollection, MetricType
from .iit_model_pair import IITModelPair, labels_of


class IITBehaviorModelPair(IITModelPair):
    def __init__(self, hl_model, ll_model, corr, training_args=None):
        defaults = {
            "lr": 0.001,
            "atol": 5e-2,
            "early_stop": True,
            "use_single_loss": False,
            "iit_weight": 1.0,
            "behavior_weight": 1.0,
        }
        super().__init__(hl_model, ll_model, corr=corr, training_args={**defaults, **(training_args or {})})
        self.wandb_method = "iit_and_behavior"

    def _categorical(self) -> bool:
        try:
            return bool(self.hl_model.is_categorical())
        except AttributeError:
            return True

    @property
    def loss_fn(self):
        if self._loss_fn_override is not None:
            return self._loss_fn_override
        return torch.nn.CrossEntropyLoss() if self._categorical() else torch.nn.MSELoss()

    @loss_fn.setter
    def loss_fn(self, value):
        self._loss_fn_override = value

    @staticmethod
    def make_train_metrics():
        return MetricStoreCollection([
            MetricStore("train/iit_loss", MetricType.LOSS),
            MetricStore("train/behavior_loss", MetricType.LOSS),
        ])

    @staticmethod
    def make_test_metrics():
        return MetricStoreCollection([
            MetricStore("val/iit_loss", MetricType.LOSS),
            MetricStore("val/IIA", MetricType.ACCURACY),
            MetricStore("val/accuracy", MetricType.ACCURACY),
        ])

    def get_behaviour_loss_over_batch(self, base_input, loss_fn):
        base_x, base_y = base_input[0], base_input[1]
        output = self.ll_forward(base_x)
        if output.dim() > 1 and output.shape[0] == 1:
            return loss_fn(output, base_y)
        return loss_fn(output.squeeze() if 1 in output.shape else output, base_y)

    def step_on_loss(self, loss: Tensor, optimizer) -> None:
        optimizer.zero_grad()
        self.backward(loss)
        self.clip_grad_fn(optimizer)
        self.optimizer_step(optimizer)

    def run_train_step(self, base_input, ablation_input, loss_fn, optimizer):
        args = self.training_args
        hl_node = self.sample_hl_name()

        def iit():
            return self.get_IIT_loss_over_batch(base_input, ablation_input, hl_node, loss_fn) * args["iit_weight"]

        def behavior():
            return self.get_behaviour_loss_over_batch(base_input, loss_fn) * args["behavior_weight"]

        if args["use_single_loss"]:
            def total():
                parts = {"iit": iit(), "behavior": behavior()}
                return parts["iit"] + parts["behavior"], parts

            _, parts = self.run_phase(("single", hl_node.name), total, optimizer, self.step_on_loss)
            return {"train/iit_loss": parts["iit"], "train/behavior_loss": parts["behavior"]}
        iit_loss = self.run_phase(("iit", hl_node.name), iit, optimizer, self.step_on_loss)
        behavior_loss = self.run_phase(("behavior",), behavior, optimizer, self.step_on_loss)
        return {"train/iit_loss": iit_loss, "train/behavior_loss": behavior_loss}

    def run_eval_step(self, base_input, ablation_input, loss_fn):
        atol = self.training_args["atol"]
        hl_node = self.sample_hl_name()
        hl_output, ll_output = self.do_intervention(base_input, ablation_input, hl_node)
        loss = loss_fn(ll_output, hl_output)
        if self._categorical():
            top1 = torch.argmax(ll_output, dim=-1)
            iia = (top1 == labels_of(hl_output, ll_output)).float().mean()
        else:
            iia = ((ll_output - hl_output).abs() < atol).float().mean()
        base_x, base_y = base_input[0], base_input[1]
        output = self.ll_forward(base_x)
        if self._categorical():
            accuracy = (torch.argmax(output, dim=-1) == labels_of(base_y, output)).float().mean()
        else:
            accuracy = ((output.squeeze() - base_y).abs() < atol).float().mean()
        return {"val/iit_loss": loss.detach(), "val/IIA": iia, "val/accuracy": accuracy}
```

### iit_amd/model_pairs/ioi_model_pair.py

```python
from __future__ import annotations

import numpy as np
import torch
import torch.nn.functional as F
from torch import Tensor

from ..config import DEVICE
from ..core import index as index_mod
from ..core.metric import MetricStore, MetricStoreCollection, MetricType, PerTokenMetricStore
from .base_model_pair import _ll_nodes_of
from .strict_iit_model_pair import StrictIITModelPair


def _last(t: Tensor, seq_dim_present: bool) -> Tensor:
    return t[:, -1] if seq_dim_present else t


class IOI_ModelPair(StrictIITModelPair):
    def __init__(self, hl_model, ll_model, corr, training_args=None):
        super().__init__(hl_model, ll_model, corr, training_args=training_args)
        defaults = {"next_token": False, "non_ioi_thresh": 0.65, "use_per_token_check": False}
        self.training_args = {**defaults, **self.training_args}
        self.next_token = bool(self.training_args["next_token"])

    def ll_logits_mode(self) -> str:
        return "full" if (self.next_token or not self.native()) else "last"

    def hl_run_kwargs(self):
        if self.native() and not self.next_token and getattr(self.hl_model, "supports_last_only", False):
            return {"last_only": True}
        return {}

    @property
    def loss_fn(self):
        if self._loss_fn_override is not None:
            return self._loss_fn_override
        return self.per_token_weighted_cross_entropy

    @loss_fn.setter
    def loss_fn(self, value):
        self._loss_fn_override = value

    def per_token_weighted_cross_entropy(self, output: Tensor, target: Tensor) -> Tensor:
        output = output.float()
        if output.dim() == 2:
            if target.dim() == 3 or (target.dim() == 2 and not target.dtype.is_floating_point):
                target = target[:, -1]
            if target.dtype.is_floating_point and target.dim() == 2:
                target = target.argmax(-1) if bool((target.sum(-1) == 1).all()) else target
            if not target.dtype.is_floating_point:
                from ..ops import cross_entropy
                return cross_entropy(output, target)
            return F.cross_entropy(output, target)
        if self.next_token:
            B, S, V = output.shape
            if target.dtype.is_floating_point:
                per = -(target * F.log_softmax(output, -1)).sum(-1)
            else:
                per = F.cross_entropy(output.reshape(B * S, V), target.reshape(B * S), reduction="none").view(B, S)
            w = torch.ones(S, device=output.device)
            w[-1] = 10
            return (per * w).sum() / (w.sum() * B)
        return F.cross_entropy(output[:, -1, :], target[:, -1])

    @staticmethod
    def get_label_idxs():
        return index_mod.Ix[:, -1]

    @staticmethod
    def make_test_metrics():
        return MetricStoreCollection([
            MetricStore("val/iit_loss", MetricType.LOSS),
            MetricStore("val/IIA", MetricType.ACCURACY),
            MetricStore("val/accuracy", MetricType.ACCURACY),
            PerTokenMetricStore("val/per_token_accuracy"),
        ])

    @staticmethod
    def _hl_label(hl_output: Tensor) -> Tensor:
        return torch.argmax(hl_output[:, -1] if hl_output.dim() == 3 else hl_output, dim=-1)

    def fast_hl_label(self, base_x: Tensor, ablation_x: Tensor, hl_node):
        from ..tasks.ioi.ioi_hl import IOI_HL
        hl = self.hl_model
        if not (self.native() and self.training_args.get("fast_hl", True) and type(hl) is IOI_HL
                and base_x.is_cuda and base_x.dtype == torch.long and ablation_x.dtype == torch.long):
            return None
        from ..ops import hip_kernels as K
        node = K.IOI_HL_NODES.get(hl_node.name)
        if node is None or not (hl_node.index is None or hl_node.index.is_everything()):
            return None
        if base_x.dim() != 2 or base_x.shape != ablation_x.shape or base_x.shape[1] > 64:
            return None
        if any(hp.is_live for hp in hl.hook_dict.values()):
            return None
        nm = hl.name_mover_head
        table = nm.name_table
        if table.device != base_x.device:
            table = nm.name_table = table.to(base_x.device)
        out = torch.empty(base_x.shape[0], dtype=torch.long, device=base_x.device)
        K.ioi_hl_label(base_x.contiguous(), ablation_x.contiguous(), table, nm.d_vocab_out, node, out)
        return out

    def _label_and_ll(self, base_input, ablation_input, hl_node):
        label = self.fast_hl_label(base_input[0], ablation_input[0], hl_node)
        if label is None:
            hl_output, ll_output = self.do_intervention(base_input, ablation_input, hl_node)
            return self._hl_label(hl_output), ll_output
        return label, self.ll_intervention(base_input[0], ablation_input[0], _ll_nodes_of(self.corr, hl_node))

    def get_IIT_loss_over_batch(self, base_input, ablation_input, hl_node, loss_fn):
        hl_label, ll_output = self._label_and_ll(base_input, ablation_input, hl_node)
        ll_last = ll_output[:, -1] if ll_output.dim() == 3 else ll_output
        return loss_fn(ll_last, hl_label)

    def run_eval_step(self, base_input, ablation_input, loss_fn):
        hl_node = self.sample_hl_name()
        hl_label, ll_output = self._label_and_ll(base_input, ablation_input, hl_node)
        ll_last = ll_output[:, -1] if ll_output.dim() == 3 else ll_output
        loss = loss_fn(ll_last, hl_label)
        iia = (torch.argmax(ll_last, dim=-1) == hl_label).float().mean()
        base_x, base_y = base_input[0], base_input[1]
        top1 = self.ll_forward(base_x, logits="argmax")
        if base_y.dtype.is_floating_point and base_y.dim() == 3:
            base_y = torch.argmax(base_y, dim=-1)
        per_token = (top1 == base_y).float().mean(dim=0)
        accuracy = per_token.mean() if self.next_token else per_token[-1]
        return {"val/iit_loss": loss.detach(), "val/IIA": iia, "val/accuracy": accuracy,
                "val/per_token_accuracy": per_token}

    @staticmethod
    def _check_early_stop_fn(test_metrics, verbose: bool = False, non_ioi_thresh: float = 0.65,
                             use_per_token_check: bool = False) -> bool:
        say = print if verbose else (lambda *a, **k: None)
        for metric in test_metrics:
            if metric.get_name() == "val/IIA" and metric.get_value() < 100:
                say(f"IIA is not enough: {metric.get_value()}")
                return False
            if metric.get_name() == "val/per_token_accuracy":
                acc = np.asarray(metric.get_value())
                if acc[-1] < 1:
                    say(f"per_token_acc at IOI index is not enough: {acc[-1]}")
                    return False
                if np.mean(acc) < non_ioi_thresh:
                    say(f"mean per_token_acc is not enough: {np.mean(acc)}")
                    return False
                if use_per_token_check:
                    for i, a in enumerate(acc):
                        if i in (2, 4, 5, 8, 10, 13):
                            continue
                        if a < non_ioi_thresh:
                            say(f"per_token_acc at {i} is not enough: {a}")
                            return False
        return True

    def _check_early_stop_condition(self, *args, **kwargs):
        if not self.training_args["next_token"]:
            return super()._check_early_stop_condition(*args, **kwargs)
        return self._check_early_stop_fn(*args, **kwargs, non_ioi_thresh=self.training_args["non_ioi_thresh"],
                                         use_per_token_check=self.training_args["use_per_token_check"])
```

### iit_amd/model_pairs/strict_iit_model_pair.py

```python
from __future__ import annotations

from ..core.metric import MetricStore, MetricStoreCollection, MetricType
from ..core.nodes import LLNode
from ..utils import node_picker
from .iit_behavior_model_pair import IITBehaviorModelPair


class StrictIITModelPair(IITBehaviorModelPair):
    def __init__(self, hl_model, ll_model, corr, training_args=None):
        defaults = {
            "batch_size": 256,
            "lr": 0.001,
            "num_workers": 0,
            "use_single_loss": False,
            "iit_weight": 1.0,
            "behavior_weight": 1.0,
            "strict_weight": 1.0,
            "clip_grad_norm": 1.0,
        }
        super().__init__(hl_model, ll_model, corr=corr, training_args={**defaults, **(training_args or {})})
        self.nodes_not_in_circuit = node_picker.get_nodes_not_in_circuit(self.ll_model, self.corr)

    @staticmethod
    def make_train_metrics():
        return MetricStoreCollection([
            MetricStore("train/iit_loss", MetricType.LOSS),
            MetricStore("train/behavior_loss", MetricType.LOSS),
            MetricStore("train/strict_loss", MetricType.LOSS),
        ])

    def sample_ll_node(self) -> LLNode:
        return self.rng.choice(self.nodes_not_in_circuit)

    def get_strict_loss_over_batch(self, base_input, ablation_input, ll_node: LLNode, loss_fn):
        base_x, base_y = base_input[0], base_input[1]
        out = self.ll_paired_intervention(base_x, ablation_input[0], [ll_node])
        if out is None:
            self.ll_cache = self.ll_source_cache(ablation_input[0], [ll_node])
            out = self.ll_intervened_forward(base_x, [ll_node])
        if out.dim() > 1 and out.shape[0] == 1:
            return loss_fn(out, base_y)
        return loss_fn(out.squeeze() if 1 in out.shape else out, base_y)

    def run_train_step(self, base_input, ablation_input, loss_fn, optimizer):
        args = self.training_args
        hl_node = self.sample_hl_name()

        def iit():
            return self.get_IIT_loss_over_batch(base_input, ablation_input, hl_node, loss_fn) * args["iit_weight"]

        if args["use_single_loss"]:
            ll_node = self.sample_ll_node()

            def total():
                parts = {"iit": iit(),
                         "strict": self.get_strict_loss_over_batch(base_input, ablation_input, ll_node, loss_fn)
                         * args["strict_weight"],
                         "behavior": self.get_behaviour_loss_over_batch(base_input, loss_fn) * args["behavior_weight"]}
                return parts["iit"] + parts["behavior"] + parts["strict"], parts

            _, parts = self.run_phase(("single", hl_node.name, ll_node.name, repr(ll_node.index)), total, optimizer,
                                      self.step_on_loss)
            return {"train/iit_loss": parts["iit"], "train/behavior_loss": parts["behavior"],
                    "train/strict_loss": parts["strict"]}
        iit_loss = self.run_phase(("iit", hl_node.name), iit, optimizer, self.step_on_loss)
        ll_node = self.sample_ll_node()
        strict_loss = self.run_phase(
            ("strict", ll_node.name, repr(ll_node.index)),
            lambda: self.get_strict_loss_over_batch(base_input, ablation_input, ll_node, loss_fn) * args["strict_weight"],
            optimizer, self.step_on_loss)
        behavior_loss = self.run_phase(
            ("behavior",), lambda: self.get_behaviour_loss_over_batch(base_input, loss_fn) * args["behavior_weight"],
            optimizer, self.step_on_loss)
        return {"train/iit_loss": iit_loss, "train/behavior_loss": behavior_loss, "train/strict_loss": strict_loss}
```

### iit_amd/ops/__init__.py

```python
from __future__ import annotations

from typing import Optional

import torch

from .torch_ops import TorchOps, gelu_new

_TORCH_OPS_CACHE = {}


def _torch_ops(dtype):
    ops = _TORCH_OPS_CACHE.get(dtype)
    if ops is None:
        ops = _TORCH_OPS_CACHE[dtype] = TorchOps(dtype)
    return ops


def hip_supported(cfg) -> bool:
    return (cfg.positional_embedding_type == "standard" and cfg.normalization_type in ("LN", "LNPre", None)
            and not cfg.gated_mlp and (cfg.n_key_value_heads in (None, cfg.n_heads))
            and not cfg.parallel_attn_mlp and not cfg.final_rms
            and cfg.act_fn in ("gelu_new", "gelu_fast", "gelu_pytorch_tanh", "gelu", "relu"))


def select_ops(model, backend: Optional[str] = None):
    cfg = model.cfg
    dtype = cfg.dtype
    on_gpu = next(model.parameters()).is_cuda
    if backend is None:
        from .. import config as _config
        env = _config.backend()
        backend = "hip" if (on_gpu and dtype == torch.bfloat16 and env == "hip" and hip_supported(cfg)) else "torch"
    if backend == "torch":
        return _torch_ops(dtype)
    if backend == "hip":
        if not on_gpu:
            raise RuntimeError("hip op backend requires the model on a GPU")
        from .hip_ops import get_hip_ops
        return get_hip_ops(model)
    if backend in ("hip32", "hip32x", "hip32n", "hip32p"):
        if not on_gpu:
            raise RuntimeError(f"{backend} op backend requires the model on a GPU")
        from .hip32_ops import get_hip32_ops, get_hip32n_ops, get_hip32p_ops, get_hip32x_ops
        return {"hip32": get_hip32_ops, "hip32x": get_hip32x_ops, "hip32n": get_hip32n_ops,
                "hip32p": get_hip32p_ops}[backend](model)
    raise ValueError(f"unknown op backend {backend}")


def cross_entropy(logits: torch.Tensor, target: torch.Tensor) -> torch.Tensor:
    if logits.is_cuda and logits.dim() == 2 and not target.dtype.is_floating_point:
        from .hip_ops import cross_entropy as _hip_ce
        return _hip_ce(logits, target)
    return torch.nn.functional.cross_entropy(logits.float(), target)
```

### iit_amd/ops/hip_kernels.py

```python
from __future__ import annotations

import ctypes
import math
import os
from typing import Optional, Sequence

import numpy as np
import torch

from . import build as _build

c_void_p, c_long, c_int, c_float, c_ull = ctypes.c_void_p, ctypes.c_long, ctypes.c_int, ctypes.c_float, ctypes.c_ulonglong

EPI_BF16, EPI_BF16_BIAS3, EPI_F32_RESID, EPI_GELU, EPI_DGELU, EPI_F32_ACC, EPI_F32_ACC_QKV, EPI_F32_STORE = range(8)
EPI_GELU_ERF = 8
EPI_DGELU_ERF = 9
MODE_NN, MODE_AKM, MODE_BKM, MODE_AF32, MODE_BF32 = 0, 1, 2, 4, 8

_LIB = None
GEMM_GROUP_M = 4
GEMM_DUAL_GROUP_M = 2

_SIGS = {
    "iit_gemm": [c_void_p] * 10 + [c_long] * 5 + [c_int] * 12 + [c_void_p],
    "iit_gemm_f32": [c_void_p] * 6 + [c_long] * 4 + [c_int] * 7 + [c_void_p],
    "iit_gemm_f32_ok": [c_void_p] * 6 + [c_long] * 4 + [c_int] * 7,
    "iit_gemm_f32_aux": [c_void_p] * 7 + [c_long] * 5 + [c_int] * 7 + [c_void_p],
    "iit_gemm_f32_aux_ok": [c_void_p] * 7 + [c_long] * 5 + [c_int] * 7,
    "iit_ln_f32_part_rows": [],
    "iit_ln_f32_fwd_ok": [c_void_p] * 6 + [c_int, c_int, c_long, c_long],
    "iit_ln_f32_fwd": [c_void_p] * 6 + [c_int, c_int, c_long, c_long, c_float, c_void_p],
    "iit_ln_f32_bwd_ok": [c_void_p] * 9 + [c_int, c_int, c_long, c_long, c_long],
    "iit_ln_f32_bwd": [c_void_p] * 9 + [c_int, c_int, c_long, c_long, c_long, c_void_p],
    "iit_dgelu_f32_ok": [c_void_p] * 3 + [c_long],
    "iit_dgelu_f32": [c_void_p] * 3 + [c_long, c_void_p],
    "iit_attn_f32_lds": [c_int] * 3,
    "iit_attn_f32_waves": [c_int] * 3,
    "iit_attn_f32_ok": [c_void_p] * 4 + [c_int] * 4,
    "iit_attn_f32_fwd": [c_void_p] * 6 + [c_int] * 4 + [c_float, c_int, c_void_p],
    "iit_attn_f32_bwd": [c_void_p] * 9 + [c_int] * 4 + [c_float, c_int, c_void_p],
    "iit_attn_f32_fwd_pair": [c_void_p] * 6 + [c_int] * 4 + [c_float, c_int, c_void_p, c_void_p],
    "iit_attn_f32_bwd_masked": [c_void_p] * 9 + [c_int] * 4 + [c_float, c_int, c_void_p, c_void_p],
    "iit_sparse_pair_f32": [c_void_p, c_long, c_long, c_void_p, c_int, c_void_p],
    "iit_gemm_glds_ok": [c_void_p] * 5 + [c_long] * 5 + [c_int] * 9,
    "iit_gemm_glds_sm": [c_void_p] * 8 + [c_long] * 5 + [c_int] * 8 + [c_void_p] * 3 + [c_int] + [c_void_p] * 3,
    "iit_embed_pos_fwd": [c_void_p, c_void_p, c_void_p, c_void_p, c_int, c_int, c_int, c_void_p],
    "iit_embed_pos_bwd": [c_void_p, c_void_p, c_void_p, c_void_p, c_int, c_int, c_int, c_void_p],
    "iit_ln_fwd": [c_void_p] * 7 + [c_int, c_int, c_float, c_ull, c_int, c_int, c_void_p],
    "iit_ln_fwd_pf": [c_void_p] * 7 + [c_int, c_int, c_float, c_ull, c_int, c_int, c_void_p, c_long, c_void_p, c_long,
                      c_int, c_void_p],
    "iit_ln_bwd": [c_void_p, c_int, c_void_p, c_int] + [c_void_p] * 10 + [c_int, c_int, c_int, c_ull, c_int, c_void_p],
    "iit_ln_bwd_part_rows": [],
    "iit_attn_small_fwd": [c_void_p] * 4 + [c_ull, c_int, c_int, c_int, c_int, c_long, c_long, c_long, c_float, c_int,
                                            c_void_p],
    "iit_attn_small_bwd": [c_void_p] * 4 + [c_ull, c_int, c_int, c_int, c_int, c_long, c_long, c_float, c_int, c_void_p],
    "iit_attn_mfma_fwd": [c_void_p] * 4 + [c_ull, c_int, c_int, c_int, c_int, c_long, c_long, c_long, c_float, c_int,
                                           c_void_p],
    "iit_attn_mfma_fwd_pair": [c_void_p] * 4 + [c_ull, c_int, c_int, c_int, c_int, c_long, c_long, c_long, c_float,
                                                c_int, c_void_p, c_int, c_ull, c_void_p],
    "iit_attn_mfma_bwd": [c_void_p] * 4 + [c_ull, c_int, c_int, c_int, c_int, c_long, c_long, c_float, c_int, c_void_p],
    "iit_attn_mfma_fwd_spec": [c_void_p] * 3 + [c_int] * 4 + [c_long, c_long, c_float, c_int, c_int, c_void_p,
                                                               c_void_p],
    "iit_attn_mfma_bwd_spec": [c_void_p] * 4 + [c_int] * 4 + [c_long, c_long, c_float, c_int, c_void_p, c_void_p],
    "iit_ce_fwd": [c_void_p, c_long, c_void_p, c_void_p, c_void_p, c_void_p, c_int, c_int, c_void_p],
    "iit_ce_bwd": [c_void_p, c_long, c_void_p, c_void_p, c_void_p, c_float, c_void_p, c_long, c_int, c_int, c_int,
                   c_void_p, c_void_p],
    "iit_gemm_glds_edge_ok": [c_void_p] * 4 + [c_long] * 3 + [c_int] * 6,
    "iit_gemm_glds_edge": [c_void_p] * 4 + [c_long] * 3 + [c_int] * 7 + [c_void_p, c_void_p, c_int, c_void_p],
    "iit_gemm_edge_plan": [c_int, c_int, c_long, c_int, c_int, c_void_p],
    "iit_ce_bwd16": [c_void_p, c_long, c_void_p, c_void_p, c_void_p, c_float, c_void_p, c_long, c_int, c_int, c_void_p],
    "iit_adam_flat": [c_void_p] * 6 + [c_int, c_void_p, c_int] + [c_float] * 6 + [c_void_p] * 3
                     + [c_void_p, c_int, c_void_p, c_void_p],
    "iit_sumsq_2d": [c_void_p, c_long, c_int, c_int, c_void_p, c_void_p],
    "iit_kl_rows": [c_void_p, c_long, c_void_p, c_long, c_int, c_int, c_void_p, c_void_p],
    "iit_adam_span_size": [],
    "iit_sumsq_spans": [c_void_p, c_void_p, c_int, c_void_p, c_int, c_int, c_void_p, c_void_p],
    "iit_adam_spans": [c_void_p] * 6 + [c_int, c_void_p] + [c_float] * 6 + [c_void_p] * 4,
    "iit_gelu_fwd": [c_void_p, c_long, c_void_p, c_long, c_int, c_int, c_int, c_void_p],
    "iit_shadow_refresh": [c_void_p, c_int, c_void_p],
    "iit_shadow_desc_size": [],
    "iit_colsum_accum": [c_void_p, c_int, c_long, c_void_p, c_int, c_int, c_void_p],
    "iit_dgelu": [c_void_p, c_void_p, c_void_p, c_long, c_int, c_void_p],
    "iit_add_bf16": [c_void_p, c_long, c_void_p, c_long, c_void_p, c_long, c_void_p, c_int, c_int, c_void_p],
    "iit_device_sync": [],
    "iit_zero_chunks": [c_void_p, c_void_p, c_int, c_void_p],
    "iit_zero_ranges": [c_void_p, c_void_p, c_void_p, c_int, c_void_p],
    "iit_colsum_multi": [c_void_p] * 6 + [c_int, c_void_p],
    "iit_rms_fwd": [c_void_p, c_int, c_void_p, c_void_p, c_void_p, c_int, c_int, c_float, c_void_p],
    "iit_rms_bwd": [c_void_p, c_void_p, c_int, c_void_p, c_void_p, c_void_p, c_void_p, c_int, c_int, c_void_p],
    "iit_rms_bwd_res": [c_void_p, c_void_p, c_int, c_void_p, c_void_p, c_void_p, c_void_p, c_void_p, c_int, c_int,
                        c_void_p],
    "iit_rotary": [c_void_p, c_long, c_long, c_long, c_void_p, c_void_p, c_void_p] + [c_int] * 8 + [c_void_p],
    "iit_swiglu_fwd": [c_void_p, c_void_p, c_void_p, c_long, c_void_p],
    "iit_swiglu_bwd": [c_void_p] * 5 + [c_long, c_void_p],
    "iit_swiglu_splice_fwd": [c_void_p] * 4 + [c_long, c_void_p, c_void_p],
    "iit_sparse_pair": [c_void_p, c_long, c_long, c_void_p, c_int, c_void_p],
    "iit_gemm_dual_set_group_m": [c_int],
    "iit_swiglu_splice_bwd": [c_void_p] * 5 + [c_long, c_void_p, c_void_p],
    "iit_embed_splice_fwd": [c_void_p, c_void_p, c_long, c_void_p, c_void_p, c_long, c_int, c_void_p, c_void_p],
    "iit_embed_splice_bwd": [c_void_p, c_void_p, c_int, c_void_p, c_long, c_long, c_int, c_void_p, c_void_p],
    "iit_flash_fwd": [c_void_p] * 3 + [c_void_p, c_void_p, c_void_p, c_void_p, c_void_p, c_void_p, c_ull] + [c_int] * 5
                     + [c_float, c_int, c_void_p, c_void_p],
    "iit_flash_bwd": [c_void_p] * 3 + [c_void_p] * 11 + [c_ull] + [c_int] * 5 + [c_float, c_int, c_void_p, c_void_p],
    "iit_flash_fwd_blocks": [c_void_p] * 3 + [c_void_p, c_void_p, c_void_p, c_void_p, c_void_p, c_void_p, c_ull]
                            + [c_int] * 5 + [c_float, c_int, c_void_p, c_void_p, c_int],
    "iit_flash_bwd_blocks": [c_void_p] * 3 + [c_void_p] * 11 + [c_ull] + [c_int] * 5 + [c_float, c_int, c_void_p,
                                                                                       c_void_p, c_int],
    "iit_flash_plan": [c_int] * 6 + [c_void_p],
    "iit_splice": [c_void_p, c_void_p, c_void_p, c_long, c_void_p, c_int, c_int, c_float, c_void_p],
    "iit_splice_spec_size": [],
    "iit_bn_fwd": [c_void_p] * 8 + [c_long, c_int, c_float, c_int, c_int, c_void_p, c_float, c_void_p, c_void_p,
                                    c_void_p, c_int, c_int, c_int, c_int, c_void_p],
    "iit_bn_bwd": [c_void_p] * 7 + [c_long, c_int, c_int, c_void_p, c_void_p, c_void_p, c_void_p, c_void_p, c_void_p,
                                    c_int, c_int, c_int, c_int, c_void_p],
    "iit_gemm_glds_set_prof": [c_void_p],
    "iit_maxpool3s2_fwd": [c_void_p] * 3 + [c_int] * 5 + [c_void_p],
    "iit_bn_ws_floats": [c_int],
    "iit_maxpool3s2_bwd": [c_void_p] * 3 + [c_int] * 5 + [c_void_p],
    "iit_gemm_dual_ok": [c_void_p] * 3 + [c_long] * 3 + [c_int] * 7 + [c_void_p] * 4 + [c_long] * 4 + [c_int] * 5,
    "iit_gemm_dual": [c_void_p] * 3 + [c_long] * 3 + [c_int] * 6 + [c_void_p] * 2 + [c_void_p] * 4 + [c_long] * 4
                     + [c_int] * 5 + [c_void_p] * 3 + [c_void_p, c_long, c_void_p, c_long, c_int, c_void_p],
    "iit_gemm_glds_set_group_m": [c_int],
    "iit_ioi_hl_label": [c_void_p, c_void_p, c_void_p, c_int, c_int, c_int, c_int, c_int, c_void_p, c_void_p],
    "iit_tile_table": [c_int, c_void_p, c_int],
    "iit_conv2d_ok": [c_long] + [c_int] * 12,
    "iit_conv2d": [c_void_p] * 4 + [c_long] + [c_int] * 12 + [c_void_p] * 4,
    "iit_conv2d_wgrad_ok": [c_long] + [c_int] * 11,
    "iit_conv2d_wgrad": [c_void_p] * 4 + [c_long] + [c_int] * 12 + [c_void_p] * 3,
    "iit_bn_fwd_tiles": [c_void_p] * 4 + [c_int, c_int] + [c_void_p] * 4 + [c_long, c_int, c_float, c_int, c_void_p,
                                                                           c_float, c_void_p, c_void_p],
}


def lib():
    global _LIB
    if _LIB is None:
        if not _build.is_up_to_date():
            _build.build()
        L = ctypes.CDLL(_build.LIB)
        for name, argtypes in _SIGS.items():
            fn = getattr(L, name)
            fn.argtypes = argtypes
            fn.restype = c_int
        check_tile_tables(L)
        _LIB = L
        gm = os.environ.get("IIT_GEMM_GROUP_M", str(GEMM_GROUP_M))
        if gm:
            L.iit_gemm_glds_set_group_m(int(gm))
        dgm = os.environ.get("IIT_GEMM_DUAL_GROUP_M", str(GEMM_DUAL_GROUP_M))
        if dgm:
            L.iit_gemm_dual_set_group_m(int(dgm))
    return _LIB


TILE_FAMILIES = ("glds", "edge", "dual_w", "dual_x", "conv", "conv_wgrad")
TILE_FIELDS = ("bm", "bn", "bk", "ns", "nw", "occ", "aux")


def tile_table(family: str, L=None) -> dict:
    L = L or lib()
    fam = TILE_FAMILIES.index(family)
    n = L.iit_tile_table(fam, None, 0)
    buf = (c_int * (8 * n))()
    L.iit_tile_table(fam, buf, n)
    return {buf[8 * i]: dict(zip(TILE_FIELDS, buf[8 * i + 1:8 * i + 8])) for i in range(n)}


def check_tile_tables(L=None) -> None:
    ours = {"glds": GLDS_TILES, "edge": {t: GLDS_TILES.get(t) for t in GLDS_EDGE_TILES}, "conv": CONV_TILES,
            "conv_wgrad": CONV_WG_TILES, "dual_w": {t: v + DUAL_W_WAVES.get(t, ()) for t, v in DUAL_W_TILES.items()},
            "dual_x": {t: v + DUAL_X_WAVES.get(t, ()) for t, v in DUAL_X_TILES.items()}}
    for family, mine in ours.items():
        theirs = {t: (r["bm"], r["bn"], r["nw"], r["occ"])[:4 if family.startswith("dual") else 2]
                  for t, r in tile_table(family, L).items()}
        for t in sorted(set(mine) | set(theirs)):
            if mine.get(t) != theirs.get(t):
                raise RuntimeError(f"tile table {family!r}, tile {t}: hip_kernels.py has {mine.get(t)}, the library "
                                   f"has {theirs.get(t)} (csrc/gemm_tiles.h)")


def available() -> bool:
    try:
        lib()
        return True
    except Exception:
        return False


def _p(t: Optional[torch.Tensor]):
    return None if t is None else t.data_ptr()


def _stream():
    return torch.cuda.current_stream().cuda_stream


CHECK_BOUNDS = os.environ.get("IIT_CHECK_BOUNDS", "0") == "1"


def _avail(t: torch.Tensor) -> int:
    st = t.untyped_storage()
    return (st.nbytes() - (t.data_ptr() - st.data_ptr())) // t.element_size()


def _bounds(what: str, *spans):
    for name, t, rows, cols, ld in spans:
        if t is None or rows <= 0 or cols <= 0:
            continue
        need = (rows - 1) * ld + cols
        have = _avail(t)
        if need > have or ld < cols and rows > 1:
            raise RuntimeError(f"{what}: operand {name} needs {rows}x{cols} (ld {ld}) = {need} elements, "
                               f"storage holds {have} (shape {tuple(t.shape)}, stride {t.stride()})")


def _check(rc: int, what: str):
    if rc != 0:
        raise RuntimeError(f"{what} failed with hip error {rc}")


N_CU = 256


def _tiling(M: int, N: int, K: int, allow_split: bool):
    t128 = math.ceil(M / 128) * math.ceil(N / 128)
    if t128 >= 240:
        return 1, 1
    t64 = math.ceil(M / 64) * math.ceil(N / 64)
    splits = 1
    if allow_split and t64 < 240 and K >= 1024:
        splits = max(1, min(math.ceil(480 / t64), K // 512))
    return 0, splits


def gemm(A, B, C, *, M: int, N: int, K: int, lda: int, ldb: int, ldc: int, mode: int = MODE_NN, epi: int = EPI_BF16,
         C2=None, C3=None, bias0=None, bias1=None, bias2=None, resid=None, ldr: int = 0, aux=None, ldc2: int = 0,
         bias_cols: int = 0, qkv=(0, 0, 0), atomic: bool = False, splits: Optional[int] = None):
    can_split = epi in (EPI_F32_ACC, EPI_F32_ACC_QKV)
    big, auto_splits = _tiling(M, N, K, can_split)
    if splits is None:
        splits = auto_splits
    if CHECK_BOUNDS:
        _gemm_bounds("iit_gemm", A, B, C, C2, resid, M, N, K, lda, ldb, ldc, ldc2, ldr, mode, qkv)
    rc = lib().iit_gemm(_p(A), _p(B), _p(C), _p(C2), _p(C3), _p(bias0), _p(bias1), _p(bias2), _p(resid), _p(aux),
                        lda, ldb, ldc, ldc2, ldr, M, N, K, mode, epi, splits, big, bias_cols, qkv[0], qkv[1], qkv[2],
                        int(atomic), _stream())
    _check(rc, "iit_gemm")


GLDS_TILES = {0: (128, 128), 1: (128, 64), 2: (64, 128), 3: (64, 64), 4: (128, 128),
              5: (256, 192),
              6: (128, 128), 7: (256, 128),
              8: (96, 96),
              9: (128, 96),
              10: (96, 192), 11: (192, 96),
              12: (96, 96), 13: (128, 96), 14: (64, 64),
              15: (128, 96), 16: (96, 96), 17: (64, 64), 18: (128, 128),
              20: (192, 192),
              21: (192, 128), 22: (128, 192),
              23: (128, 96), 24: (64, 96), 25: (128, 128), 26: (96, 96), 27: (128, 192), 28: (64, 192),
              29: (64, 96), 30: (64, 64), 31: (64, 128),
              32: (256, 128), 33: (128, 256), 34: (256, 256),
              40: (256, 256),
              41: (256, 256), 42: (256, 256)}
GLDS_DISPATCH_TILES = tuple(t for t in GLDS_TILES if t not in (12, 13, 14, 32, 33, 34, 42))


def _gemm_bounds(what, A, B, C, C2, resid, M, N, K, lda, ldb, ldc, ldc2, ldr, mode, qkv=(0, 0, 0)):
    a = ("A", A, K, M, lda) if mode & MODE_AKM else ("A", A, M, K, lda)
    b = ("B", B, K, N, ldb) if mode & MODE_BKM else ("B", B, N, K, ldb)
    if qkv[0]:
        dh, H, d = qkv
        per = ("C", C, 1, H * d * dh, H * d * dh)
        _bounds(what, a, b, per, ("C2",) + per[1:] if C2 is None else ("C2", C2, 1, H * d * dh, H * d * dh))
        return
    _bounds(what, a, b, ("C", C, M, N, ldc), ("C2", C2, M, N, ldc2 or ldc), ("resid", resid, M, N, ldr or ldc))


def gemm_glds_ok(A, B, C, *, M, N, K, lda, ldb, ldc, mode, epi, C2=None, resid=None, ldc2=0, ldr=0, bias_cols=0,
                 tile=0, splits=1, reduce=False) -> bool:
    if any(t is not None and (not t.is_cuda or t.dtype not in (torch.bfloat16,)) for t in (A, B)):
        return False
    return bool(lib().iit_gemm_glds_ok(_p(A), _p(B), _p(C), _p(C2), _p(resid), lda, ldb, ldc, ldc2, ldr, M, N, K,
                                       mode, epi, bias_cols, tile, splits, int(reduce)))


_SPLIT_WS = {}


def split_workspace(M: int, N: int, tile, splits: int, device) -> tuple:
    stream = torch.cuda.current_stream(device).cuda_stream
    key = (str(device), stream)
    ent = _SPLIT_WS.get(key)
    bm, bn = GLDS_TILES[tile] if isinstance(tile, int) else tile
    need_ws, need_cnt = splits * M * N, (M // bm) * (N // bn)
    if ent is None:
        ent = _SPLIT_WS[key] = [None, None, []]
    if ent[0] is None or ent[0].numel() < need_ws:
        if ent[0] is not None:
            ent[2].append(ent[0])
        ent[0] = torch.empty(need_ws, dtype=torch.float32, device=device)
    if ent[1] is None or ent[1].numel() < need_cnt:
        if ent[1] is not None:
            ent[2].append(ent[1])
        ent[1] = torch.zeros(max(need_cnt, 1024), dtype=torch.int32, device=device)
    return ent[0], ent[1]


GLDS_STORE_MODE = int(os.environ.get("IIT_GEMM_STORE", "0"))


def gemm_glds(A, B, C, *, M, N, K, lda, ldb, ldc, mode, epi, C2=None, bias0=None, bias1=None, bias2=None, resid=None,
              ldc2=0, ldr=0, bias_cols=0, tile=0, splits=1, csum=None, reduce=False, store_mode=None, bsum=None,
              gsq=None):
    ws = cnt = None
    if reduce:
        ws, cnt = split_workspace(M, N, tile, splits, A.device)
    if CHECK_BOUNDS:
        _gemm_bounds("iit_gemm_glds", A, B, C, C2, resid, M, N, K, lda, ldb, ldc, ldc2, ldr, mode)
        _bounds("iit_gemm_glds", ("csum", csum, 1, N, N))
    sm = GLDS_STORE_MODE if store_mode is None else store_mode
    _check(lib().iit_gemm_glds_sm(_p(A), _p(B), _p(C), _p(C2), _p(bias0), _p(bias1), _p(bias2), _p(resid), lda, ldb,
                                  ldc, ldc2, ldr, M, N, K, mode, epi, bias_cols, tile, splits, _p(csum), _p(ws),
                                  _p(cnt), int(sm), _p(bsum) if mode == 3 else None,
                                  _p(gsq) if epi == EPI_F32_STORE else None, _stream()),
           "iit_gemm_glds")


GLDS_EDGE_TILES = (0, 7, 25)


def gemm_glds_edge_ok(A, B, C, *, M, N, K, lda, ldb, ldc, mode, epi, bias0=None, tile=25) -> bool:
    if any(t is None or not t.is_cuda or t.dtype != torch.bfloat16 for t in (A, B)):
        return False
    return bool(lib().iit_gemm_glds_edge_ok(_p(A), _p(B), _p(C), _p(bias0), lda, ldb, ldc, M, N, K, mode, epi, tile))


def gemm_glds_edge(A, B, C, *, M, N, K, lda, ldb, ldc, mode, epi, bias0=None, tile=25, store_mode=None, bsum=None,
                   gsq=None):
    if CHECK_BOUNDS:
        a = ("A", A, K, M, lda) if mode & MODE_AKM else ("A", A, M, K, lda)
        _bounds("iit_gemm_glds_edge", a, ("B", B, K, (N + 7) // 8 * 8, ldb), ("C", C, M, N, ldc),
                ("bias0", bias0, 1, N, N), ("bsum", bsum, 1, N, N))
    sm = GLDS_STORE_MODE if store_mode is None else store_mode
    gm = int(os.environ.get("IIT_GEMM_GROUP_M", str(GEMM_GROUP_M)) or 0)
    _check(lib().iit_gemm_glds_edge(_p(A), _p(B), _p(C), _p(bias0), lda, ldb, ldc, M, N, K, mode, epi, tile, int(sm),
                                    _p(bsum) if mode == 3 else None, _p(gsq) if epi == EPI_F32_STORE else None, gm,
                                    _stream()), "iit_gemm_glds_edge")


def gemm_edge_plan(rows: int, N: int, ld: int, elem: int, tile: int) -> Optional[dict]:
    out = (ctypes.c_long * 6)()
    if lib().iit_gemm_edge_plan(rows, N, ld, elem, tile, ctypes.cast(out, c_void_p)) != 0:
        return None
    return dict(zip(("tiles_n", "used", "redirected", "straddle", "last_byte", "valid_bytes"), list(out)))


GEMM_F32_TILES = {0: (64, 64), 1: (128, 128)}


def _f32_cuda(*ts) -> bool:
    return all(t is None or (t.is_cuda and t.dtype == torch.float32) for t in ts)


def gemm_f32_ok(A, B, C, *, M, N, K, lda, ldb, ldc, mode, epi, bias=None, resid=None, ldr=0, tile=0, splits=1,
                aux=None, ldx=0) -> bool:
    if not _f32_cuda(A, B, C, bias, resid, aux) or tile not in GEMM_F32_TILES:
        return False
    ws = 16 if splits > 1 else None
    return bool(lib().iit_gemm_f32_aux_ok(_p(A), _p(B), _p(C), _p(bias), _p(resid), _p(aux), ws, lda, ldb, ldc, ldr,
                                          ldx, M, N, K, mode, epi, tile, splits))


def gemm_f32_splits(M: int, N: int, K: int, tile: int = 0) -> int:
    bm, bn = GEMM_F32_TILES[tile]
    tiles = math.ceil(M / bm) * math.ceil(N / bn)
    return max(1, min(N_CU // tiles, K // 128, 64))


def gemm_f32(A, B, C, *, M, N, K, lda, ldb, ldc, mode, epi, bias=None, resid=None, ldr=0, tile=0, splits=1, aux=None,
             ldx=0):
    if not gemm_f32_ok(A, B, C, M=M, N=N, K=K, lda=lda, ldb=ldb, ldc=ldc, mode=mode, epi=epi, bias=bias, resid=resid,
                       ldr=ldr, tile=tile, splits=splits, aux=aux, ldx=ldx):
        raise RuntimeError(f"iit_gemm_f32: unsupported problem M={M} N={N} K={K} lda={lda} ldb={ldb} ldc={ldc} "
                           f"ldr={ldr} ldx={ldx} mode={mode} epi={epi} tile={tile} splits={splits} (fp32 GPU operands, "
                           f"16-byte aligned pointers, leading dimensions multiples of 4)")
    if CHECK_BOUNDS:
        _gemm_bounds("iit_gemm_f32", A, B, C, None, resid, M, N, K, lda, ldb, ldc, 0, ldr, mode)
        _bounds("iit_gemm_f32", ("bias", bias, 1, N, N))
        if epi in (EPI_GELU, EPI_DGELU):
            _bounds("iit_gemm_f32", ("aux", aux, M, N, ldx))
    ws = torch.empty(splits * M * N, dtype=torch.float32, device=A.device) if splits > 1 else None
    _check(lib().iit_gemm_f32_aux(_p(A), _p(B), _p(C), _p(bias), _p(resid), _p(aux), _p(ws), lda, ldb, ldc, ldr, ldx,
                                  M, N, K, mode, epi, tile, splits, _stream()), "iit_gemm_f32")


LN_F32_MAX_D = 4096


def _rows_f32(what: str, **ts):
    shape = None
    lds = []
    for name, t in ts.items():
        if not (isinstance(t, torch.Tensor) and t.dim() == 2 and t.is_cuda and t.dtype == torch.float32):
            raise ValueError(f"{what}: {name} must be a 2-D fp32 GPU tensor")
        shape = shape or tuple(t.shape)
        if tuple(t.shape) != shape or min(shape) < 1:
            raise ValueError(f"{what}: {name} has shape {tuple(t.shape)}, expected non-empty {shape}")
        T, d = shape
        ld = d if T == 1 else t.stride(0)
        if (d > 1 and t.stride(1) != 1) or ld < d:
            raise ValueError(f"{what}: {name} needs unit column stride and a row pitch >= {d}, got {t.stride()}")
        lds.append(ld)
    return shape[0], shape[1], lds


def _vec_f32(what: str, n: int, **ts):
    for name, t in ts.items():
        if t is not None and not (t.is_cuda and t.dtype == torch.float32 and t.is_contiguous() and t.numel() == n):
            raise ValueError(f"{what}: {name} must be {n} contiguous fp32 values on the GPU")


def ln_f32_ok(x: torch.Tensor, w=None, b=None) -> bool:
    if not (isinstance(x, torch.Tensor) and x.is_cuda and x.dtype == torch.float32 and x.dim() >= 1 and x.numel() > 0
            and x.shape[-1] <= LN_F32_MAX_D and (w is None) == (b is None)):
        return False
# ... 445 lines not shown

def _bsh(t: torch.Tensor):
    assert t.stride(-1) == 1 and t.dtype == torch.bfloat16, "flash attention takes bf16 [B,S,H,dh] with unit d stride"
    return [t.stride(0), t.stride(1), t.stride(2)]


def _longs(vals):
    return (c_long * len(vals))(*vals)


def _flash_blocks(blocks: int) -> int:
    if blocks not in (0, 1, 2):
        raise ValueError(f"flash attention: blocks must be 0 (the launch policy), 1 or 2, got {blocks!r}")
    return int(blocks)


def flash_plan(B: int, S: int, Hq: int, Hkv: int, dh: int, blocks: int = 0) -> dict:
    out = (c_int * 4)()
    _check(lib().iit_flash_plan(B, S, Hq, Hkv, dh, _flash_blocks(blocks), ctypes.cast(out, c_void_p)), "flash_plan")
    return {"nb_q": out[0], "nb_kv": out[1], "grid_q": out[2], "grid_kv": out[3]}


def flash_fwd(q, k, v, z, lse, src, head_mask: int, scale: float, causal: bool, spec=None, blocks: int = 0):
    blocks = _flash_blocks(blocks)
    B, S, Hq, dh = q.shape
    Hkv = k.shape[2]
    st = _longs(_bsh(q) + _bsh(k) + _bsh(v))
    zs = _longs(_bsh(z))
    ss = _longs(_bsh(src)) if (src is not None and spec is None) else None
    _check(lib().iit_flash_fwd_blocks(_p(q), _p(k), _p(v), ctypes.cast(st, c_void_p), _p(z), ctypes.cast(zs, c_void_p),
                                      _p(lse), _p(src), None if ss is None else ctypes.cast(ss, c_void_p),
                                      head_mask if src is not None else 0, B, S, Hq, Hkv, dh, scale, int(causal),
                                      None if spec is None else spec.ptr, _stream(), blocks),
           "flash_fwd")


def flash_bwd(q, k, v, z, dz, lse, dd, dq, dk, dv, head_mask: int, scale: float, causal: bool, spec=None,
              blocks: int = 0):
    blocks = _flash_blocks(blocks)
    B, S, Hq, dh = q.shape
    Hkv = k.shape[2]
    st = _longs(_bsh(q) + _bsh(k) + _bsh(v))
    gs = _longs(_bsh(dq) + _bsh(dk) + _bsh(dv))
    zs, ds = _longs(_bsh(z)), _longs(_bsh(dz))
    _check(lib().iit_flash_bwd_blocks(_p(q), _p(k), _p(v), ctypes.cast(st, c_void_p), _p(z), ctypes.cast(zs, c_void_p),
                                      _p(dz), ctypes.cast(ds, c_void_p), _p(lse), _p(dd), _p(dq), _p(dk), _p(dv),
                                      ctypes.cast(gs, c_void_p), head_mask, B, S, Hq, Hkv, dh, scale, int(causal),
                                      None if spec is None else spec.ptr, _stream(), blocks),
           "flash_bwd")


def bn_ws_floats(C: int) -> int:
    return int(lib().iit_bn_ws_floats(C))


def maxpool3s2_fwd(x, y, idx, N: int, H: int, W: int, C: int):
    if CHECK_BOUNDS:
        OH, OW = (H - 1) // 2 + 1, (W - 1) // 2 + 1
        assert y.numel() == N * OH * OW * C and idx.numel() == y.numel() and x.numel() == N * H * W * C
    _check(lib().iit_maxpool3s2_fwd(_p(x), _p(y), _p(idx), N, H, W, C, int(x.dtype == torch.float32), _stream()),
           "maxpool3s2_fwd")


_ZERO_PAGE = {}


def zero_page(device) -> torch.Tensor:
    key = str(device)
    z = _ZERO_PAGE.get(key)
    if z is None:
        z = _ZERO_PAGE[key] = torch.zeros(256, dtype=torch.bfloat16, device=device)
    return z


CONV_TILES = {0: (128, 64), 1: (128, 128), 2: (64, 64), 3: (128, 128), 4: (64, 128), 5: (128, 64)}


def conv3x3_rows(tile: int) -> int:
    return CONV_TILES[tile][0]


def conv2d_ok(N: int, SH: int, SW: int, Cs: int, OH: int, OW: int, Co: int, k: int, s: int, pad: int,
              transposed: bool, tile: int, splits: int = 1) -> bool:
    return bool(lib().iit_conv2d_ok(N, SH, SW, Cs, OH, OW, Co, k, s, pad, int(transposed), tile, splits))


def conv2d(x, w, y, N: int, SH: int, SW: int, Cs: int, OH: int, OW: int, Co: int, k: int, s: int, pad: int,
           transposed: bool, tile: int = 0, splits: int = 1, cstat=None):
    ws = cnt = None
    if splits > 1:
        ws, cnt = split_workspace(N * OH * OW, Co, CONV_TILES[tile], splits, x.device)
    if CHECK_BOUNDS:
        assert x.numel() >= N * SH * SW * Cs and y.numel() >= N * OH * OW * Co and w.numel() >= k * k * Cs * Co
        assert x.dtype == w.dtype == y.dtype == torch.bfloat16
        if cstat is not None:
            assert cstat.dtype == torch.float32 and cstat.numel() >= 3 * Co * (N * OH * OW // conv3x3_rows(tile))
    _check(lib().iit_conv2d(_p(x), _p(w), _p(y), _p(zero_page(x.device)), N, SH, SW, Cs, OH, OW, Co, k, s, pad,
                            int(transposed), tile, splits, _p(ws), _p(cnt), _p(cstat), _stream()), "conv2d")


def conv2d_wgrad_ok(N: int, SH: int, SW: int, Cin: int, OH: int, OW: int, Cout: int, k: int, s: int, pad: int,
                    tile: int, splits: int) -> bool:
    return bool(lib().iit_conv2d_wgrad_ok(N, SH, SW, Cin, OH, OW, Cout, k, s, pad, tile, splits))


def conv2d_wgrad(dy, x, dw, N: int, SH: int, SW: int, Cin: int, OH: int, OW: int, Cout: int, k: int, s: int,
                 pad: int, acc: bool, tile: int, splits: int = 1):
    ws = cnt = None
    if splits > 1:
        ws, cnt = split_workspace(Cout, k * k * Cin, CONV_WG_TILES[tile], splits, dy.device)
    if CHECK_BOUNDS:
        assert dw.dtype == torch.float32 and dw.numel() >= k * k * Cin * Cout
        assert dy.numel() >= N * OH * OW * Cout and x.numel() >= N * SH * SW * Cin
    _check(lib().iit_conv2d_wgrad(_p(dy), _p(x), _p(dw), _p(zero_page(x.device)), N, SH, SW, Cin, OH, OW, Cout, k, s,
                                  pad, int(acc), tile, splits, _p(ws), _p(cnt), _stream()), "conv2d_wgrad")


CONV_WG_TILES = {0: (64, 64), 1: (128, 64), 2: (128, 128), 3: (64, 128)}


def conv3x3_wgrad_splits(pixels: int) -> list:
    nkt = pixels // 64
    out = []
    for target in (1, 2, 4, 8, 16, 32, 64):
        d = max(x for x in range(1, target + 1) if nkt % x == 0)
        if d not in out:
            out.append(d)
    return out


def conv3x3_tiles() -> int:
    return len(CONV_TILES)


def conv3x3_ok(N: int, H: int, W: int, Cin: int, Cout: int, tile: int, splits: int = 1) -> bool:
    return conv2d_ok(N, H, W, Cin, H, W, Cout, 3, 1, 1, False, tile, splits)


def conv3x3(x, w, y, N: int, H: int, W: int, Cin: int, Cout: int, flip: bool = False, tile: int = 0,
            splits: int = 1, cstat=None):
    conv2d(x, w, y, N, H, W, Cin, H, W, Cout, 3, 1, 1, flip, tile, splits, cstat)


def conv3x3_wgrad_ok(N: int, H: int, W: int, Cin: int, Cout: int, tile: int, splits: int) -> bool:
    return conv2d_wgrad_ok(N, H, W, Cin, H, W, Cout, 3, 1, 1, tile, splits)


def conv3x3_wgrad(dy, x, dw, N: int, H: int, W: int, Cin: int, Cout: int, acc: bool, tile: int, splits: int = 1):
    conv2d_wgrad(dy, x, dw, N, H, W, Cin, H, W, Cout, 3, 1, 1, acc, tile, splits)


def maxpool3s2_bwd(dy, idx, dx, N: int, H: int, W: int, C: int):
    _check(lib().iit_maxpool3s2_bwd(_p(dy), _p(idx), _p(dx), N, H, W, C, int(dy.dtype == torch.float32), _stream()),
           "maxpool3s2_bwd")


def bn_two_level() -> bool:
    if os.environ.get("IIT_BN_REDUCE", "") == "two":
        return True
    return os.environ.get("IIT_DETERMINISTIC", "0") == "1" or torch.are_deterministic_algorithms_enabled()


def bn_fwd(x, res, y, ws, rmean, rvar, w, b, M: int, C: int, eps: float, relu: bool, training: bool, save,
           momentum: float, nbt, src=None, spec=None, H: int = 0, W: int = 0):
    if CHECK_BOUNDS:
        for t in (x, y) + ((res,) if res is not None else ()):
            assert _avail(t) >= M * C and t.dtype == x.dtype, "bn_fwd: activation smaller than M x C / dtype"
        assert ws.numel() >= bn_ws_floats(C) and save.numel() >= 2 * C
    _check(lib().iit_bn_fwd(_p(x), _p(res), _p(y), _p(ws), _p(rmean), _p(rvar), _p(w), _p(b), M, C, eps, int(relu),
                            int(training), _p(save), momentum, _p(nbt), _p(src), None if spec is None else spec.ptr,
                            H, W, int(x.dtype == torch.float32), int(bn_two_level()), _stream()), "bn_fwd")


def bn_fwd_tiles(x, res, y, cstat, T: int, R: int, rmean, rvar, w, b, M: int, C: int, eps: float, relu: bool, save,
                 momentum: float, nbt):
    if CHECK_BOUNDS:
        for t in (x, y) + ((res,) if res is not None else ()):
            assert _avail(t) >= M * C and t.dtype == torch.bfloat16, "bn_fwd_tiles: activation smaller than M x C"
        assert T * R == M and cstat.numel() >= 3 * C * T and save.numel() >= 2 * C
    _check(lib().iit_bn_fwd_tiles(_p(x), _p(res), _p(y), _p(cstat), T, R, _p(rmean), _p(rvar), _p(w), _p(b), M, C,
                                  eps, int(relu), _p(save), momentum, _p(nbt), _stream()), "bn_fwd_tiles")


def bn_bwd(dy, y, x, save, w, ws, coef, M: int, C: int, training: bool, dx, dres, dw, db, src=None, spec=None,
           H: int = 0, W: int = 0):
    if CHECK_BOUNDS:
        for t in (dy, x, dx):
            assert _avail(t) >= M * C, "bn_bwd: activation smaller than M x C"
    _check(lib().iit_bn_bwd(_p(dy), _p(y), _p(x), _p(save), _p(w), _p(ws), _p(coef), M, C, int(training), _p(dx),
                            _p(dres), _p(dw), _p(db), _p(src), None if spec is None else spec.ptr, H, W,
                            int(x.dtype == torch.float32), int(bn_two_level()), _stream()), "bn_bwd")


def zero_ranges(base, starts, lens):
    import numpy as np
    starts = np.ascontiguousarray(starts, dtype=np.int64)
    lens = np.ascontiguousarray(lens, dtype=np.int64)
    if CHECK_BOUNDS and len(lens):
        assert int((starts + lens).max()) <= _avail(base) and int(starts.min()) >= 0, "zero_ranges out of bounds"
    _check(lib().iit_zero_ranges(_p(base), starts.ctypes.data, lens.ctypes.data, len(lens), _stream()),
           "zero_ranges")


def zero_chunks(base, chunks, n: int):
    _check(lib().iit_zero_chunks(_p(base), _p(chunks), n, _stream()), "zero_chunks")


def rms_fwd(x, w, y, rstd, T: int, d: int, eps: float):
    _check(lib().iit_rms_fwd(_p(x), int(x.dtype == torch.float32), _p(w), _p(y), _p(rstd), T, d, eps, _stream()),
           "rms_fwd")


def rms_bwd(dy, x, rstd, w, dx, dw, T: int, d: int, dres=None):
    _check(lib().iit_rms_bwd_res(_p(dy), _p(x), int(x.dtype == torch.float32), _p(rstd), _p(w), _p(dx), _p(dres),
                                 _p(dw), T, d, _stream()), "rms_bwd")


def rotary(x, out, cos, sin, rd: int, offset: int, adjacent: bool, inverse: bool):
    B, S, H, D = x.shape
    if x.dtype != torch.bfloat16 or x.stride(-1) != 1:
        raise ValueError(f"rotary: x must be bf16 with unit stride on its last dimension, got {x.dtype}, "
                         f"stride {x.stride()}")
    for name, t in (("cos", cos), ("sin", sin)):
        if t.dtype != torch.float32 or not t.is_contiguous():
            raise ValueError(f"rotary: {name} must be contiguous fp32, got {t.dtype}, stride {t.stride()}")
        if t.dim() != 2 or t.shape[1] != rd:
            raise ValueError(f"rotary: {name} must be [n_ctx, {rd}], got {tuple(t.shape)}")
        if t.shape[0] < offset + S:
            raise ValueError(f"rotary: {name} has {t.shape[0]} rows, positions {offset} .. {offset + S - 1} need "
                             f"{offset + S}")
    _check(lib().iit_rotary(_p(x), x.stride(0), x.stride(1), x.stride(2), _p(out), _p(cos), _p(sin), int(inverse),
                            B, S, H, D, rd, offset, int(adjacent), _stream()), "rotary")


def swiglu_fwd(gate, up, post):
    _check(lib().iit_swiglu_fwd(_p(gate), _p(up), _p(post), gate.numel(), _stream()), "swiglu_fwd")


def sparse_pair(act, T: int, ld: int, spec_ptr, mode: int) -> None:
    if CHECK_BOUNDS:
        _bounds("sparse_pair", ("act", act, 2 * T if mode == 0 else T, ld, ld))
    _check(lib().iit_sparse_pair(_p(act), T, ld, spec_ptr, int(mode), _stream()), "sparse_pair")


def _sparse_pair_f32_why(act, T: int, ld: int, spec, mode: int) -> Optional[str]:
    if mode not in (0, 1):
        return f"mode must be 0 (copy) or 1 (zero), got {mode}"
    if not isinstance(act, torch.Tensor) or not act.is_cuda or act.dtype != torch.float32:
        return "act must be an fp32 tensor on the GPU"
    if spec is None or not getattr(spec, "ptr", 0):
        return "spec must be a PatchSpec, got None"
    dims = spec.dims
    if len(dims) != 4 or dims[0][0] * dims[1][0] * dims[2][0] != T or T < 1:
        return f"spec shape {tuple(d[0] for d in dims)} does not flatten to T = {T} rows"
    if dims[3][0] > ld:
        return f"spec's last dimension {dims[3][0]} is wider than ld = {ld}"
    for n, runs, _ in dims:
        if len(runs) > 8 or any(lo < 0 or hi > n or lo > hi for lo, hi in runs):
            return f"spec ranges {runs} leave [0, {n})"
    rows = 2 * T if mode == 0 else T
    if act.numel() == 0 or (rows - 1) * ld + dims[3][0] > _avail(act):
        return f"act holds {_avail(act)} elements, {rows} rows of pitch {ld} need {(rows - 1) * ld + dims[3][0]}"
    return None


def sparse_pair_f32(act, T: int, ld: int, spec, mode: int) -> None:
    why = _sparse_pair_f32_why(act, T, ld, spec, mode)
    if why is not None:
        raise ValueError(f"sparse_pair_f32: {why}")
    if CHECK_BOUNDS:
        _bounds("sparse_pair_f32", ("act", act, 2 * T if mode == 0 else T, int(spec.dims[3][0]), ld))
    _check(lib().iit_sparse_pair_f32(_p(act), T, ld, spec.ptr, int(mode), _stream()), "sparse_pair_f32")


def swiglu_splice_fwd(gate, up, post, src, spec_ptr):
    _check(lib().iit_swiglu_splice_fwd(_p(gate), _p(up), _p(post), _p(src), gate.numel(), spec_ptr, _stream()),
           "swiglu_splice_fwd")


def embed_splice_fwd(tokens, W16, out, src, spec_ptr):
    T, d = tokens.numel(), out.shape[-1]
    if CHECK_BOUNDS:
        _bounds("embed_splice_fwd", ("out", out, T, d, d))
    _check(lib().iit_embed_splice_fwd(_p(tokens), _p(W16), W16.stride(0), _p(out), _p(src), T, d, spec_ptr,
                                      _stream()), "embed_splice_fwd")


def embed_splice_bwd(tokens, dout, grad, spec_ptr):
    T, d = tokens.numel(), dout.shape[-1]
    _check(lib().iit_embed_splice_bwd(_p(tokens), _p(dout), int(dout.dtype == torch.float32), _p(grad),
                                      grad.stride(0), T, d, spec_ptr, _stream()), "embed_splice_bwd")


def swiglu_splice_bwd(dpost, gate, up, dgate, dup, spec_ptr):
    _check(lib().iit_swiglu_splice_bwd(_p(dpost), _p(gate), _p(up), _p(dgate), _p(dup), gate.numel(), spec_ptr,
                                       _stream()), "swiglu_splice_bwd")


def swiglu_bwd(dpost, gate, up, dgate, dup):
    _check(lib().iit_swiglu_bwd(_p(dpost), _p(gate), _p(up), _p(dgate), _p(dup), gate.numel(), _stream()),
           "swiglu_bwd")


def ce_fwd(logits, ld, labels, loss, lse, amax, R, V):
    if CHECK_BOUNDS:
        _bounds("ce_fwd", ("logits", logits, R, V, ld))
    _check(lib().iit_ce_fwd(_p(logits), ld, _p(labels), _p(loss), _p(lse), _p(amax), R, V, _stream()), "ce_fwd")


def ce_bwd(logits, ld, labels, lse, gscale, inv_rows, out, ld_out, R, V, out16=None):
    if CHECK_BOUNDS:
        _bounds("ce_bwd", ("logits", logits, R, V, ld), ("out", out, R, V, ld_out))
    _check(lib().iit_ce_bwd(_p(logits), ld, _p(labels), _p(lse), _p(gscale), inv_rows, _p(out), ld_out, R, V,
                            int(out.dtype == torch.bfloat16), _p(out16), _stream()), "ce_bwd")


def ce_bwd16(logits, ld, labels, lse, gscale, inv_rows, out16, ld_out, R, V):
    assert logits.dtype == torch.float32 and out16.dtype == torch.bfloat16 and gscale.dtype == torch.float32
    if CHECK_BOUNDS:
        _bounds("ce_bwd16", ("logits", logits, R, V, ld), ("out16", out16, R, ld_out, ld_out))
    _check(lib().iit_ce_bwd16(_p(logits), ld, _p(labels), _p(lse), _p(gscale), inv_rows, _p(out16), ld_out, R, V,
                              _stream()), "ce_bwd16")


def colsum_accum(x, ld, out, T, N):
    if CHECK_BOUNDS:
        _bounds("colsum", ("x", x, T, N, ld), ("out", out, 1, N, N))
    _check(lib().iit_colsum_accum(_p(x), int(x.dtype == torch.float32), ld, _p(out), T, N, _stream()), "colsum")


def colsum_vec_ok(x, ld, out, N) -> bool:
    cpt = 4 if x.dtype == torch.float32 else 8
    return (x.dtype in (torch.float32, torch.bfloat16) and out.dtype == torch.float32 and N % cpt == 0
            and ld % cpt == 0 and x.data_ptr() % 16 == 0)


def colsum_multi(items):
    import numpy as np
    if not items:
        return
    xs = np.array([it[0].data_ptr() for it in items], dtype=np.int64)
    outs = np.array([it[2].data_ptr() for it in items], dtype=np.int64)
    lds = np.array([it[1] for it in items], dtype=np.int64)
    Ts = np.array([it[3] for it in items], dtype=np.int32)
    Ns = np.array([it[4] for it in items], dtype=np.int32)
    f32s = np.array([int(it[0].dtype == torch.float32) for it in items], dtype=np.int32)
    if CHECK_BOUNDS:
        for x, ld, out, T, N in items:
            _bounds("colsum_multi", ("x", x, T, N, ld), ("out", out, 1, N, N))
    _check(lib().iit_colsum_multi(xs.ctypes.data, outs.ctypes.data, lds.ctypes.data, Ts.ctypes.data, Ns.ctypes.data,
                                  f32s.ctypes.data, len(items), _stream()), "colsum_multi")


def colsum3_accum(x, ld, outs, T, N):
    for i, o in enumerate(outs):
        colsum_accum(x[:, i * N:], ld, o, T, N)


def gelu_fwd(pre, out, M, N, erf=False):
    _check(lib().iit_gelu_fwd(_p(pre), pre.stride(0), _p(out), out.stride(0), M, N, int(erf), _stream()), "gelu_fwd")


def dgelu(dpost, pre, out, erf=False):
    _check(lib().iit_dgelu(_p(dpost), _p(pre), _p(out), dpost.numel(), int(erf), _stream()), "dgelu")


def add_bf16(out, ldo, base, ldb, y, ldy, bias, M, N):
    if CHECK_BOUNDS:
        _bounds("add_bf16", ("out", out, M, N, ldo), ("base", base, M, N, ldb), ("y", y, M, N, ldy))
    _check(lib().iit_add_bf16(_p(out), ldo, _p(base), ldb, _p(y), ldy, _p(bias), M, N, _stream()), "add_bf16")


def shadow_refresh(descs: torch.Tensor, n: int):
    _check(lib().iit_shadow_refresh(_p(descs), n, _stream()), "shadow_refresh")


_SHADOW_DTYPE = np.dtype([("src", np.uint64), ("dst", np.uint64), ("rows", np.int32), ("cols", np.int32),
                          ("ld", np.int64), ("heads", np.int32), ("transpose", np.int32), ("src_hs", np.int64),
                          ("dst_hs", np.int64)])


def make_shadow_descs(entries, device) -> torch.Tensor:
    assert _SHADOW_DTYPE.itemsize == lib().iit_shadow_desc_size()
    arr = np.zeros(len(entries), dtype=_SHADOW_DTYPE)
    for i, e in enumerate(entries):
        src_ptr, dst_ptr, rows, cols, ld, tr = e[:6]
        heads, shs, dhs = (e[6], e[7], e[8]) if len(e) > 6 else (1, 0, 0)
        arr[i] = (src_ptr, dst_ptr, rows, cols, ld, heads, int(tr), shs, dhs)
    return torch.from_numpy(arr.view(np.uint8).copy()).to(device)


def adam_step(flat, exp_avg, exp_avg_sq, step_dev, *, lr, b1, b2, eps, wd, clip_norm, skipped=None, hyper=None):
    nparts = 1024
    part = getattr(flat, "_norm_parts", None)
    if part is None or part.numel() < nparts:
        part = flat._norm_parts = torch.zeros(nparts, dtype=torch.float32, device=flat.data.device)
    spans, nspans = flat.span_table(lib().iit_adam_span_size(), max_len4=_ADAM_SPAN4)
    sq_spans, n_sq, gsq = flat.norm_spans(lib().iit_adam_span_size())
    _check(lib().iit_adam_flat(_p(flat.data), _p(flat.grad), _p(exp_avg), _p(exp_avg_sq), _p(flat.shadow),
                               _p(spans), nspans, _p(part), nparts, float(clip_norm or 0.0), lr, b1, b2, eps, wd,
                               _p(hyper), _p(step_dev), _p(skipped), _p(sq_spans), n_sq, _p(gsq), _stream()),
           "adam_flat")
    flat.after_step(mirror_written=flat.shadow is not None)


IOI_HL_NODES = {"all_nodes_hook": 0, "hook_duplicate": 1, "hook_s_inhibition": 2, "hook_name_mover": 3}


def ioi_hl_label(base, src, name_table, V: int, node: int, out):
    B, S = base.shape
    _check(lib().iit_ioi_hl_label(_p(base), _p(src), _p(name_table), name_table.numel(), B, S, V, node, _p(out),
                                  _stream()), "ioi_hl_label")


def gemm_glds_set_prof(buf) -> None:
    lib().iit_gemm_glds_set_prof(_p(buf))


def gemm_glds_set_group_m(gm: int) -> None:
    lib().iit_gemm_glds_set_group_m(int(gm))


def gemm_dual_set_group_m(gm: int) -> None:
    lib().iit_gemm_dual_set_group_m(int(gm))
```

### iit_amd/ops/hip_ops.py

```python
from __future__ import annotations

import math
import os
from typing import Optional, Sequence

import torch
from torch.autograd import Function

from ..engine import grad_hooks
from . import hip_kernels as K
from .gemm_dispatch import gemm, gemm_pair
from .torch_ops import TorchOps, act_fn

BF16 = torch.bfloat16
F32 = torch.float32


def _pad8(n: int) -> int:
    return (n + 7) // 8 * 8


def _grad_slot(p: Optional[torch.Tensor]) -> Optional[torch.Tensor]:
    if p is None or not p.requires_grad:
        return None
# ... 778 lines not shown
        post = torch.empty_like(gate)
        K.swiglu_fwd(gate, up, post)
        ctx.save_for_backward(gate, up)
        return post

    @staticmethod
    def backward(ctx, dpost):
        gate, up = ctx.saved_tensors
        dg, du = torch.empty_like(gate), torch.empty_like(up)
        K.swiglu_bwd(_c16(dpost.to(BF16)), gate, up, dg, du)
        return dg, du


class SwiGLUSpliceFn(Function):

    @staticmethod
    def forward(ctx, gate, up, src, spec):
        gate, up = _c16(gate.to(BF16)), _c16(up.to(BF16))
        post = torch.empty_like(gate)
        K.swiglu_splice_fwd(gate, up, post, src, spec.ptr)
        ctx.save_for_backward(gate, up)
        ctx.spec = spec
        return post

    @staticmethod
    def backward(ctx, dpost):
        gate, up = ctx.saved_tensors
        dg, du = torch.empty_like(gate), torch.empty_like(up)
        K.swiglu_splice_bwd(_c16(dpost.to(BF16)), gate, up, dg, du, ctx.spec.ptr)
        return dg, du, None, None


def swiglu_spliced(pre, pre_linear, index, src) -> Optional[torch.Tensor]:
    from .splice import patch_spec
    if os.environ.get("IIT_SWIGLU_SPLICE", "1") == "0" or pre.shape[-1] % 8 or pre.dtype != BF16:
        return None
    if src.dtype != BF16 or src.device != pre.device:
        src = src.to(device=pre.device, dtype=BF16)
    spec = patch_spec(index, tuple(pre.shape), src)
    if spec is None or spec.dims[3][0] % 8:
        return None
    return SwiGLUSpliceFn.apply(pre, pre_linear, src, spec)


class EmbedSpliceFn(Function):

    @staticmethod
    def forward(ctx, tokens, W_E, flat, src, spec):
        tok = tokens.reshape(-1).to(torch.int64).contiguous()
        W16 = flat.shadow_view(W_E)
        out = torch.empty(*tokens.shape, W_E.shape[-1], dtype=BF16, device=W_E.device)
        K.embed_splice_fwd(tok, W16, out, src, spec.ptr)
        ctx.save_for_backward(tok)
        ctx.p, ctx.flat, ctx.spec = W_E, flat, spec
        return out

    @staticmethod
    def backward(ctx, g):
        (tok,) = ctx.saved_tensors
        from ..engine import grad_hooks
        W_E = ctx.p
        slot = W_E.grad
        if slot is None:
            slot = ctx.flat.bind_zero(W_E)
        g = g.reshape(-1, g.shape[-1])
        if g.dtype not in (BF16, torch.float32):
            g = g.float()
        K.embed_splice_bwd(tok, g.contiguous(), slot, ctx.spec.ptr)
        grad_hooks.notify(W_E)
        return None, None, None, None, None


def embed_spliced(tokens, W_E, flat, index, src) -> Optional[torch.Tensor]:
    from .splice import patch_spec
    d = W_E.shape[-1]
    if os.environ.get("IIT_EMBED_SPLICE", "1") == "0" or d % 8 or W_E.stride(-1) != 1 or W_E.stride(0) % 8:
        return None
    if src.dtype != BF16 or src.device != W_E.device:
        src = src.to(device=W_E.device, dtype=BF16)
    shape = tuple(tokens.shape) + (d,)
    spec = patch_spec(index, shape, src)
    if spec is None or spec.dims[3][0] % 8:
        return None
    return EmbedSpliceFn.apply(tokens, W_E, flat, src, spec)


def llama_fused_ok(x: torch.Tensor) -> bool:
    return x.is_cuda and x.dtype == BF16 and os.environ.get("IIT_LLAMA_FUSED", "1") != "0"


def _resid_rows(resid, resid_full):
    return _flat2((resid if resid_full is None else resid_full).float().contiguous())


def _linear_forward(ctx, x, W, b, w, ldw, resid, out_kind, x_full=None, resid_full=None):
    ctx.set_materialize_grads(False)
    lead = (x if x_full is None else x_full).shape[:-1]
    Kd = x.shape[-1]
    N = W.shape[-1]
    x2, T = _rows_bf16(x, x_full)
    T2 = x2.shape[0]
    dev = x.device
    if out_kind == "bf16":
        out = torch.empty(T2, N, dtype=BF16, device=dev)
        gemm(x2, w, out, M=T2, N=N, K=Kd, lda=Kd, ldb=ldw, ldc=N, mode=K.MODE_BKM, epi=K.EPI_BF16, bias0=b)
        res = out.view(*lead, N)
    elif out_kind == "f32":
        Np = _pad8(N)
        out = torch.empty(T2, Np, dtype=F32, device=dev)
        gemm(x2, w, out, M=T2, N=N, K=Kd, lda=Kd, ldb=ldw, ldc=Np, mode=K.MODE_BKM, epi=K.EPI_F32_STORE, bias0=b)
        res = out[:, :N]
        res = res.unflatten(0, lead) if len(lead) != 1 else res
    else:
        out = torch.empty(T2, N, dtype=F32, device=dev)
        gemm(x2, w, out, M=T2, N=N, K=Kd, lda=Kd, ldb=ldw, ldc=N, mode=K.MODE_BKM, epi=K.EPI_F32_RESID, bias0=b,
             resid=_resid_rows(resid, resid_full), ldr=N)
        res = out.view(*lead, N)
    xb = _base_rows(x2, T)
    ctx.save_for_backward(xb)
    ctx.params = (W, b)
    ctx.w = w
    _pf_register(ctx, xb, w)
    ctx.ldw = ldw
    ctx.meta = (x.shape[:-1], Kd, N, out_kind, x.dtype)
    return res


class LinearFn(Function):

    @staticmethod
    def forward(ctx, x, W, b, w, ldw, resid, out_kind):
        return _linear_forward(ctx, x, W, b, w, ldw, resid, out_kind)

    @staticmethod
    def backward(ctx, gy):
        if gy is None:
            return (None,) * 7
        (x2,) = ctx.saved_tensors
        W, b = ctx.params
        lead, Kd, N, out_kind, x_dtype = ctx.meta
        T = x2.shape[0]
        gres = gy if out_kind == "resid" else None
        g16 = _bf16_of(gy)
        g2 = _aligned_rows(g16, T, N)
        ldg = g2.stride(0)
        dx = xspec = dxb = None
        if ctx.needs_input_grad[0]:
            amode = K.MODE_NN
            _, splits = K._tiling(T, Kd, N, True)
            if splits == 1:
                dxb = torch.empty(T, Kd, dtype=BF16, device=g2.device)
                xspec = dict(A=g2, B=ctx.w, C=dxb, M=T, N=Kd, K=N, lda=ldg, ldb=ctx.ldw, ldc=Kd, mode=amode,
                             epi=K.EPI_BF16)
            else:
                dxf = torch.zeros(T, Kd, dtype=F32, device=g2.device)
                gemm(g2, ctx.w, dxf, M=T, N=Kd, K=N, lda=ldg, ldb=ctx.ldw, ldc=Kd, mode=amode, epi=K.EPI_F32_ACC,
                     splits=splits)
                dx = dxf.to(x_dtype).view(*lead, Kd)
        store, (gW,) = _wgrad_slots(True, W)
        gb = _grad_slot(b)
        bs = _wgrad_tail(ctx, xspec, x2, g2, ldg, (W,), *_wgrad_rows(gW, Kd, N), store, gb)
        if dxb is not None:
            dx = (dxb if x_dtype == BF16 else dxb.to(x_dtype)).view(*lead, Kd)
        _bias_tail(bs, gb, g2, ldg, (b,), (W,))
        return dx, None, None, None, None, gres, None


class UnembedFn(LinearFn):

    @staticmethod
    def forward(ctx, x, W, b, w, ldw):
        res = LinearFn.forward(ctx, x, W, b, w, ldw, None, "f32")
        handle = torch.empty(1, dtype=BF16, device=res.device).expand(res.shape)
        return res, handle

    @staticmethod
    def backward(ctx, gy, gh=None):
        if gh is not None:
            gy = gh if gy is None else gy.float() + gh.float()
        return LinearFn.backward(ctx, gy)[:5]


def _mlp_in_forward(ctx, x, W_in, b_in, w, erf, x_full=None, spec=None):
    ctx.set_materialize_grads(False)
    ctx.erf = erf
    ctx.zero_spec = spec
    lead = (x if x_full is None else x_full).shape[:-1]
    d = x.shape[-1]
    dm = W_in.shape[1]
    x2, T = _rows_bf16(x, x_full)
    T2 = x2.shape[0]
    post = torch.empty(T2, dm, dtype=BF16, device=x.device)
    pre = torch.empty(T2, dm, dtype=BF16, device=x.device)
    gemm(x2, w, post, C2=pre, M=T2, N=dm, K=d, lda=d, ldb=dm, ldc=dm, ldc2=dm, mode=K.MODE_BKM,
         epi=K.EPI_GELU_ERF if erf else K.EPI_GELU, bias0=b_in)
    if spec is not None:
        K.sparse_pair(post, T, dm, spec.ptr, 0)
    xb = _base_rows(x2, T)
    ctx.save_for_backward(xb, _base_rows(pre, T))
    ctx.params = (W_in, b_in)
    ctx.w = w
    _pf_register(ctx, xb, w)
    ctx.meta = (x.shape[:-1], d, dm)
    return pre.view(*lead, dm), post.view(*lead, dm)


class MLPInFn(Function):

    @staticmethod
    def forward(ctx, x, W_in, b_in, w, erf=False):
        return _mlp_in_forward(ctx, x, W_in, b_in, w, erf)

    @staticmethod
    def backward(ctx, gpre, gpost):
        if gpre is None and gpost is None:
            return None, None, None, None, None
        x2, pre = ctx.saved_tensors
        W_in, b_in = ctx.params
        lead, d, dm = ctx.meta
        T = x2.shape[0]
        if gpost is not None:
            dpre = torch.empty(T, dm, dtype=BF16, device=x2.device)
            K.dgelu(gpost.to(BF16).contiguous().view(T, dm), pre, dpre, erf=ctx.erf)
            zs = getattr(ctx, "zero_spec", None)
            if zs is not None:
                K.sparse_pair(dpre, T, dm, zs.ptr, 1)
            if gpre is not None:
                dpre = (dpre.float() + gpre.float().reshape(T, dm)).to(BF16)
        else:
            dpre = gpre.to(BF16).contiguous().view(T, dm)
        dx = torch.empty(T, d, dtype=BF16, device=x2.device)
        xspec = dict(A=dpre, B=ctx.w, C=dx, M=T, N=d, K=dm, lda=dm, ldb=dm, ldc=d, epi=K.EPI_BF16)
        store, (gW,) = _wgrad_slots(W_in.is_contiguous(), W_in)
        summed = _bias_sum_done(gpre if gpost is None else None, b_in)
        gb = None if summed else _grad_slot(b_in)
        bs = _wgrad_tail(ctx, xspec, x2, dpre, dm, (W_in,), gW, dm, store, gb)
        _bias_tail(bs, gb, dpre, dm, (b_in,), (W_in,))
        return dx.view(*lead, d), None, None, None, None


def _bias_sum_done(g: Optional[torch.Tensor], b: Optional[torch.Tensor]) -> bool:
    tag = getattr(g, "_iit_bias_sum", None) if g is not None else None
    return tag is not None and b is not None and tag == (g.data_ptr(), g._version, id(b))


def _mlp_out_forward(ctx, pre, post, W, b, w, ldw, resid, b_in, erf, post_full=None, resid_full=None):
    ctx.set_materialize_grads(False)
    ctx.erf = erf
    rows = post if post_full is None else post_full
    Kd = post.shape[-1]
    N = W.shape[-1]
    x2 = _flat2(rows)
    T2 = x2.shape[0]
    out = torch.empty(T2, N, dtype=F32, device=post.device)
    gemm(x2, w, out, M=T2, N=N, K=Kd, lda=Kd, ldb=ldw, ldc=N, mode=K.MODE_BKM, epi=K.EPI_F32_RESID, bias0=b,
         resid=_resid_rows(resid, resid_full), ldr=N)
    xb = _base_rows(x2, T2 * post.shape[0] // rows.shape[0])
    ctx.save_for_backward(xb, _flat2(pre))
    ctx.params = (W, b, b_in)
    ctx.w = w
    _pf_register(ctx, xb, w)
    ctx.ldw = ldw
    ctx.meta = (post.shape[:-1], Kd, N)
    return out.view(*rows.shape[:-1], N)


class MLPOutGeluFn(Function):

    @staticmethod
    def forward(ctx, pre, post, W, b, w, ldw, resid, b_in, erf=False):
        return _mlp_out_forward(ctx, pre, post, W, b, w, ldw, resid, b_in, erf)

    @staticmethod
    def backward(ctx, gy):
        if gy is None:
            return (None,) * 9
        x2, pre2 = ctx.saved_tensors
        W, b, b_in = ctx.params
        lead, Kd, N = ctx.meta
        T = x2.shape[0]
        g16 = _bf16_of(gy)
        g2 = _aligned_rows(g16, T, N)
        ldg = g2.stride(0)
        dpre = xspec = gbi = None
        if ctx.needs_input_grad[0]:
            dpre = torch.empty(T, Kd, dtype=BF16, device=g2.device)
            gbi = _grad_slot(b_in)
            xspec = dict(A=g2, B=ctx.w, C=dpre, M=T, N=Kd, K=N, lda=ldg, ldb=ctx.ldw, ldc=Kd, mode=K.MODE_NN,
                         epi=K.EPI_DGELU_ERF if ctx.erf else K.EPI_DGELU, aux=pre2, ldc2=pre2.stride(0), colsum=gbi)
        store, (gW,) = _wgrad_slots(True, W)
        gb = _grad_slot(b)
        bs = _wgrad_tail(ctx, xspec, x2, g2, ldg, (W,), *_wgrad_rows(gW, Kd, N), store, gb)
        if dpre is not None:
            dpre = dpre.view(*lead, Kd)
            if gbi is not None:
                dpre._iit_bias_sum = (dpre.data_ptr(), dpre._version, id(b_in))
        _bias_tail(bs, gb, g2, ldg, (b,), (W,))
        return dpre, None, None, None, None, None, gy, None, None


class CrossEntropyFn(Function):

    @staticmethod
    def forward(ctx, logits, labels, handle=None):
        ctx.set_materialize_grads(False)
        R, V = logits.shape
        if logits.stride(1) != 1:
            logits = logits.contiguous()
        ld = logits.stride(0)
        loss = torch.empty(R, dtype=F32, device=logits.device)
        lse = torch.empty(R, dtype=F32, device=logits.device)
        lab = labels.contiguous()
        K.ce_fwd(logits, ld, lab, loss, lse, None, R, V)
        ctx.save_for_backward(logits, lab, lse)
        ctx.only16 = handle is not None
        return loss.mean()

    @staticmethod
    def backward(ctx, g):
        if g is None:
            return None, None, None
        logits, lab, lse = ctx.saved_tensors
        R, V = logits.shape
        ld = logits.stride(0)
        ldo = _pad8(V)
        buf16 = torch.empty(R, ldo, dtype=BF16, device=logits.device)
        gs = g.reshape(1).float().contiguous()
        if ctx.only16:
            K.ce_bwd16(logits, ld, lab, lse, gs, 1.0 / R, buf16, ldo, R, V)
            return None, None, buf16[:, :V]
        buf = torch.empty(R, ldo, dtype=F32, device=logits.device)
        K.ce_bwd(logits, ld, lab, lse, gs, 1.0 / R, buf, ldo, R, V, out16=buf16)
        res = buf[:, :V]
        _set_bf16_twin(res, buf16[:, :V])
        return res, None, None


def _grad16_handle(logits: torch.Tensor) -> Optional[torch.Tensor]:
    tag = getattr(logits, "_iit_grad16", None)
    if tag is None or tag[0] != logits.data_ptr() or tag[1] != logits._version or tag[2].shape != logits.shape:
        return None
    if not (torch.is_grad_enabled() and tag[2].requires_grad) or logits._backward_hooks or logits.retains_grad:
        return None
    if os.environ.get("IIT_CE_BF16_ONLY", "1") == "0":
        return None
    return tag[2]


def cross_entropy(logits: torch.Tensor, labels: torch.Tensor) -> torch.Tensor:
    logits = logits.float()
    handle = _grad16_handle(logits) if logits.dim() == 2 else None
    if handle is not None:
        logits._iit_grad16 = None
        return CrossEntropyFn.apply(logits.detach(), labels, handle)
    return CrossEntropyFn.apply(logits, labels)




class Paired:

    __slots__ = ("base", "full", "f32")

    def __init__(self, base: torch.Tensor, full: torch.Tensor, f32=None):
        self.base, self.full, self.f32 = base, full, f32

    def resid_operands(self):
        if self.f32 is not None:
            return self.f32
        return self.base, self.full.float().contiguous()

    @property
    def nb(self) -> int:
        return self.base.shape[0]

    @property
    def src(self) -> torch.Tensor:
        return self.full[self.nb:]


class EmbedPosPairFn(EmbedPosFn):
    @staticmethod
    def forward(ctx, tokens, W_E, W_pos, tokens_full, box):
        ctx.set_materialize_grads(False)
        B2, S = tokens_full.shape
        d = W_E.shape[1]
        B = tokens.shape[0]
        out = torch.empty(B2, S, d, dtype=F32, device=tokens.device)
        K.embed_pos_fwd(tokens_full, W_E, W_pos, out, B2, S, d)
        ctx.save_for_backward(tokens_full[:B])
        ctx.params = (W_E, W_pos)
        box.append(out)
        return out[:B]

    @staticmethod
    def backward(ctx, g):
        return EmbedPosFn.backward(ctx, g) + (None, None)


class LayerNormForkPairFn(LayerNormForkFn):
    @staticmethod
    def forward(ctx, x, w, b, eps, x_full, box):
        yf, _ = _ln_forward(ctx, x, w, b, eps, x_full, xhat16=_xhat16(w, b, x.shape[-1]))
        box.append(yf)
        return yf[:x.shape[0]], x.view_as(x)

    @staticmethod
    def backward(ctx, dy, dpass):
        return LayerNormForkFn.backward(ctx, dy, dpass) + (None, None)


class LayerNormPairTwinFn(Function):

    @staticmethod
    def forward(ctx, x, w, b, eps, x_full, box):
        yf, yf32 = _ln_forward(ctx, x, w, b, eps, x_full, twin=True)
        box.append((yf, yf32))
        return yf[:x.shape[0]], yf32[:x.shape[0]]

    @staticmethod
    def backward(ctx, dy, dy32):
        return LayerNormTwinFn.backward(ctx, dy, dy32) + (None, None)


class LayerNormPairFn(LayerNormFn):

    @staticmethod
    def forward(ctx, x, w, b, eps, x_full, box, pos_mask=0):
        yf, _ = _ln_forward(ctx, x, w, b, eps, x_full, pos_mask=pos_mask)
        box.append(yf)
        return yf[:x.shape[0]]

    @staticmethod
    def backward(ctx, dy):
        return (_ln_backward(ctx, dy, sel=ctx.sel),) + (None,) * 6


class QKVPairFn(QKVFn):
    @staticmethod
    def forward(ctx, x, layer, bias_bf16, W_Q, W_K, W_V, b_Q, b_K, b_V, x_full, box):
        out = _qkv_forward(ctx, x, layer, bias_bf16, W_Q, W_K, W_V, b_Q, b_K, b_V, x_full)
        box.append(out)
        return out[:x.shape[0]]

    @staticmethod
    def backward(ctx, dqkv):
        return QKVFn.backward(ctx, dqkv) + (None, None)


class AttnPairFn(AttnFn):

    @staticmethod
    def forward(ctx, qkv, causal, scale, mask, qkv_full, box):
        ctx.set_materialize_grads(False)
        B = qkv.shape[0]
        B2, S, _, H, dh = qkv_full.shape
        z = torch.empty(B2, S, H, dh, dtype=BF16, device=qkv.device)
        lse = torch.empty(B2 * H * S, dtype=F32, device=qkv.device)
        if mask:
            K.attn_pair_fwd(qkv_full, z, lse, B2, S, H, dh, 3 * H * dh, H * dh, scale, causal, pair_seqs=B,
                            pair_mask=mask)
        else:
            K.attn_small_fwd(qkv_full, z, lse, None, 0, B2, S, H, dh, 3 * H * dh, H * dh, H * dh, scale, causal)
        ctx.save_for_backward(qkv_full[:B], lse[:B * H * S])
        ctx.cfg = (mask, causal, scale)
        box.append(z)
        return z[:B]

    @staticmethod
    def backward(ctx, dz):
        g = AttnFn.backward(ctx, dz)
        return (g[0], None, None, None, None, None)


class AttnPairSpecFn(Function):

    @staticmethod
    def forward(ctx, qkv, causal, scale, spec, qkv_full, box):
        ctx.set_materialize_grads(False)
        B = qkv.shape[0]
        B2, S, _, H, dh = qkv_full.shape
        z = torch.empty(B2, S, H, dh, dtype=BF16, device=qkv.device)
        lse = torch.empty(B2 * H * S, dtype=F32, device=qkv.device)
        K.attn_pair_fwd_spec(qkv_full, z, lse, B2, S, H, dh, 3 * H * dh, H * dh, scale, causal, B, spec.ptr)
        ctx.save_for_backward(qkv_full[:B], lse[:B * H * S])
        ctx.cfg = (spec, causal, scale)
        box.append(z)
        return z[:B]

    @staticmethod
    def backward(ctx, dz):
        if dz is None:
            return None, None, None, None, None, None
        qkv, lse = ctx.saved_tensors
        spec, causal, scale = ctx.cfg
        B, S, _, H, dh = qkv.shape
        qkv = qkv.contiguous()
        dz = dz.to(BF16).contiguous()
        dqkv = torch.empty_like(qkv)
        K.attn_bwd_spec(qkv, dz, lse, dqkv, B, S, H, dh, 3 * H * dh, H * dh, scale, causal, spec.ptr)
        return dqkv, None, None, None, None, None


class LinearPairFn(LinearFn):

    @staticmethod
    def forward(ctx, x, W, b, w, ldw, resid, out_kind, x_full, resid_full, box):
        of = _linear_forward(ctx, x, W, b, w, ldw, resid, out_kind, x_full, resid_full)
        box.append(of)
        return of[:x.shape[0]]

    @staticmethod
    def backward(ctx, gy):
        return LinearFn.backward(ctx, gy) + (None, None, None)


class MLPInPairFn(MLPInFn):

    @staticmethod
    def forward(ctx, x, W_in, b_in, w, erf, x_full, spec, box):
        pf, qf = _mlp_in_forward(ctx, x, W_in, b_in, w, erf, x_full, spec)
        box.append((pf, qf))
        return pf[:x.shape[0]], qf[:x.shape[0]]

    @staticmethod
    def backward(ctx, gpre, gpost):
        return MLPInFn.backward(ctx, gpre, gpost) + (None, None, None)


class MLPOutGeluPairFn(MLPOutGeluFn):
    @staticmethod
    def forward(ctx, pre, post, W, b, w, ldw, resid, b_in, erf, post_full, resid_full, box):
        of = _mlp_out_forward(ctx, pre, post, W, b, w, ldw, resid, b_in, erf, post_full, resid_full)
        box.append(of)
        return of[:post.shape[0]]

    @staticmethod
    def backward(ctx, gy):
        return MLPOutGeluFn.backward(ctx, gy) + (None, None, None)


class PairSpliceFn(Function):

    @staticmethod
    def forward(ctx, act, act_full, spec_pair, spec_base, box):
        out = torch.empty_like(act_full)
        B = act.shape[0]
        K.splice(act_full, act_full[B:], out, act_full.numel(), spec_pair.ptr, act_full.dtype == F32, 0)
        ctx.spec = spec_base
        box.append(out)
        return out[:B]

    @staticmethod
    def backward(ctx, g):
        if g is None:
            return None, None, None, None, None
        g = g.contiguous()
        out = torch.empty_like(g)
        K.splice(g, None, out, g.numel(), ctx.spec.ptr, g.dtype == F32, 1)
        return out, None, None, None, None


def _one(fn, *args):
    box = []
    out = fn.apply(*args, box)
    return out, box[0]


class HipOps(TorchOps):
    name = "hip"
    fused = True

    def __init__(self, model):
        super().__init__(BF16)
        self.model = model
        self.shadow = ModelShadow(model)
        pol = os.environ.get("IIT_DUAL_PREFETCH", "auto")
        self.prefetch = pol == "1" or (pol == "auto" and type(model).__name__ != "HookedEncoder")
        self.fwd_pf = False
        self._layer_of = {}
        self._mirror_key = {}
        for i, blk in enumerate(model.blocks):
            mats = [(blk.attn.W_Q, "qkv"), (blk.attn.W_O, "o")]
            if not model.cfg.attn_only:
                mats += [(blk.mlp.W_in, "in"), (blk.mlp.W_out, "out")]
            for W, key in mats:
                self._layer_of[id(W)] = i
                self._mirror_key[id(W)] = key

    def begin_forward(self):
        self.shadow.ensure()
        _PF_SEQ.clear()
        _PF_ON[0] = self.prefetch
        pol = os.environ.get("IIT_FWD_PREFETCH", "auto")
        self.fwd_pf = pol == "1" or (pol == "auto" and type(self.model).__name__ == "HookedTransformer")

    def _L(self, p):
        return self.shadow.layers[self._layer_of[id(p)]]

    def embed(self, tokens, W_E):
        return W_E[tokens]

    def pos_embed(self, batch, seq, W_pos, offset: int = 0):
        return W_pos[offset:offset + seq].unsqueeze(0).expand(batch, seq, W_pos.shape[-1])

    def embed_pos(self, tokens, W_E, W_pos):
        return EmbedPosFn.apply(tokens, W_E, W_pos)

    def residual(self, a, b):
        return a.float() + b.float()

    def w(self, p: torch.Tensor) -> torch.Tensor:
        return p.to(BF16)

    def fwd_prefetch(self, *Ws):
        if not self.fwd_pf:
            return None
        return tuple(self._L(W)[self._mirror_key[id(W)]] for W in Ws)

    def layer_norm(self, x, w, b, eps, prefetch=None):
        return _ln_apply(LayerNormFn, prefetch, x, w, b, eps)

    def layer_norm_twin(self, x, w, b, eps, prefetch=None):
        if os.environ.get("IIT_LN_TWIN", "1") == "0":
            return _ln_apply(LayerNormFn, prefetch, x, w, b, eps)
        y, y32 = _ln_apply(LayerNormTwinFn, prefetch, x, w, b, eps)
        y._iit_f32 = (y.data_ptr(), y._version, y32)
        return y

    def layer_norm_fork(self, x, w, b, eps, prefetch=None):
        return _ln_apply(LayerNormForkFn, prefetch, x, w, b, eps)

    def qkv(self, x, W_Q, W_K, W_V, b_Q, b_K, b_V):
        i = self._layer_of[id(W_Q)]
        packed = QKVFn.apply(x, self.shadow.layers[i], self.shadow.biases[i], W_Q, W_K, W_V, b_Q, b_K, b_V)
        q, k, v = packed[:, :, 0], packed[:, :, 1], packed[:, :, 2]
        q._iit_packed = k._iit_packed = v._iit_packed = packed
        return q, k, v

    def attention(self, q, k, v, causal, attn_scale, patch_heads: Optional[Sequence[int]] = None, patch_src=None,
                  hook_scores=None, hook_pattern=None, ignore=float("-inf")):
        S, dh = q.shape[1], q.shape[-1]
        if S > 16 and flash_supported(q):
            packed = getattr(q, "_iit_packed", None)
            if packed is not None and getattr(k, "_iit_packed", None) is packed and \
                    getattr(v, "_iit_packed", None) is packed and packed.is_contiguous():
                return FlashPackedFn.apply(packed, patch_src, K.heads_to_mask(patch_heads), causal, 1.0 / attn_scale)
            z = flash_attention(q, k, v, causal, attn_scale)
            if patch_heads:
                z = z.clone()
                z[:, :, list(patch_heads)] = patch_src[:, :, list(patch_heads)].to(z.dtype)
            return z
        if not K.attn_small_ok(S, dh):
            z = TorchOps.attention(self, q, k, v, causal, attn_scale)
            if patch_heads:
                z = z.clone()
                z[:, :, list(patch_heads)] = patch_src[:, :, list(patch_heads)].to(z.dtype)
            return z
# ... 235 lines not shown
```

### iit_amd/tasks/ioi/ioi_dataset.py

```python
from __future__ import annotations

import random
from typing import Dict, List, Optional, Sequence

import torch
from torch.utils.data import Dataset

from ...config import DEVICE
from .ioi_config import NAMES, NOUNS, TEMPLATES, vocabulary_words
from .tokenizer import SyntheticTokenizer


def default_tokenizer() -> SyntheticTokenizer:
    return SyntheticTokenizer(vocabulary_words())


class IOIDataset(Dataset):
    def __init__(self, tokenizer=None, templates: Optional[List[str]] = None, names: Optional[List[str]] = None,
                 nouns: Optional[Dict[str, List[str]]] = None, num_samples: int = 1000, symmetric: bool = False,
                 prepend_bos: bool = True, seed: int = 42, device=None):
        self.tokenizer = tokenizer if tokenizer is not None else default_tokenizer()
        self.prepend_bos = prepend_bos
        self.templates = list(templates) if templates is not None else list(TEMPLATES)
        self.names = list(names) if names is not None else list(NAMES)
        self.nouns = dict(nouns) if nouns is not None else {k: list(v) for k, v in NOUNS.items()}
        self.device = torch.device(device) if device is not None else DEVICE
        self.samples: List[Dict[str, str]] = []
        random.seed(seed)
        for _ in range(num_samples // 2 if symmetric else num_samples):
            self.samples.extend(self._draw(symmetric))
        self._build_tensors()

    def _draw(self, symmetric: bool):
        template = random.choice(self.templates)
        for slot, options in self.nouns.items():
            template = template.replace(f"[{slot}]", random.choice(options))
        a, b = random.sample(self.names, 2)
        out = [{"text": template.replace("[A]", a).replace("[B]", b), "IO": " " + a, "S": " " + b}]
        if symmetric:
            out.append({"text": template.replace("[A]", b).replace("[B]", a), "IO": " " + b, "S": " " + a})
        return out

    def _build_tensors(self):
        tok = self.tokenizer
        rows = []
        for s in self.samples:
            ids = tok.encode(s["text"])
            rows.append(([tok.bos_token_id] if self.prepend_bos else []) + ids)
        width = max(len(r) for r in rows) if rows else 0
        if any(len(r) != width for r in rows):
            rows = [r + [tok.pad_token_id] * (width - len(r)) for r in rows]
        self.prompts = torch.tensor(rows, dtype=torch.long).to(self.device)
        self.io_ids = torch.tensor([tok.encode(s["IO"])[0] for s in self.samples], dtype=torch.long).to(self.device)
        self.s_ids = torch.tensor([tok.encode(s["S"])[0] for s in self.samples], dtype=torch.long).to(self.device)

    def __len__(self) -> int:
        return len(self.samples)

    def __getitem__(self, idx):
        return {
            "prompt": self.prompts[idx],
            "IO": self.io_ids[idx:idx + 1],
            "S": self.s_ids[idx:idx + 1],
            "idx_to_ablate": int(self.prompts.shape[1]) - 2,
        }

    @staticmethod
    def get_default_names():
        return list(NAMES)

    @staticmethod
    def get_default_templates():
        return list(TEMPLATES)

    @staticmethod
    def get_default_nouns():
        return {k: list(v) for k, v in NOUNS.items()}


class IOIDatasetWrapper(IOIDataset):

    def __init__(self, *args, label_format: str = "index", **kwargs):
        if label_format not in ("index", "onehot"):
            raise ValueError("label_format must be 'index' or 'onehot'")
        self.label_format = label_format
        super().__init__(*args, **kwargs)

    def _labels(self, y: torch.Tensor) -> torch.Tensor:
        if self.label_format == "onehot":
            return torch.nn.functional.one_hot(y, num_classes=self.tokenizer.vocab_size).float()
        return y

    def __getitem__(self, idx):
        p = self.prompts[idx]
        return p[:-1], self._labels(p[1:]), self.io_ids[idx:idx + 1]

    def token_ids(self) -> torch.Tensor:
        return torch.unique(self.prompts[:, :-1])

    def gather(self, idx: torch.Tensor):
        p = self.prompts.index_select(0, idx.to(self.prompts.device))
        return p[:, :-1], self._labels(p[:, 1:]), self.io_ids.index_select(0, idx.to(self.prompts.device))[:, None]
```

Before: 17000 pairs/s.

## Fuse IOI pair gather, pack graph staging copy, fold loss weights into CE kernels

Adds a single HIP kernel that gathers base and ablation prompt rows, shifted labels and IO ids into one packed buffer. This replaces several index_select launches per step. The CUDA-graph staging step now copies that packed buffer with one copy instead of many. Cross-entropy forward and backward take a label stride and a scalar loss weight, which removes the separate weight multiply and label contiguous-copy kernels, and backward is given an explicit unit gradient. It adds code paths that depend on a Subset/root detection and on tensors sharing one packed storage, so any other layout falls back to the old path.

New measurement: 17050 pairs/s (median of 6 runs). Within noise of the previous version (+0.3%).

```diff
diff --git a/csrc/ioi_hl.hip b/csrc/ioi_hl.hip
--- a/csrc/ioi_hl.hip
+++ b/csrc/ioi_hl.hip
@@ -73,6 +73,38 @@
   }
 }
 
+__global__ __launch_bounds__(256) void ioi_batch_gather_kernel(const long* __restrict__ perm, long perm_stride,
+                                                               const long* __restrict__ tb, const long* __restrict__ ta,
+                                                               long P, const long* __restrict__ prompts,
+                                                               const long* __restrict__ io_ids, long N, int B, int S,
+                                                               long* __restrict__ out) {
+  const int W = S + 1;
+  const long t = (long)blockIdx.x * 256 + threadIdx.x;
+  if (t >= 2L * B * W) return;
+  const int side = (int)(t / ((long)B * W));
+  const int r = (int)((t / W) % B), c = (int)(t % W);
+  long pi = perm ? perm[(long)r * perm_stride] : (long)r;
+  if (pi < 0 || pi >= P) pi = 0;
+  long s = (side ? ta : tb)[pi];
+  if (s < 0 || s >= N) s = 0;
+  const long v = prompts[s * W + c];
+  long* o = out + (long)side * ((long)B * (2 * S + 1));
+  if (c < S) o[(long)r * S + c] = v;
+  if (c > 0) o[(long)B * S + (long)r * S + (c - 1)] = v;
+  if (c == 0) o[2L * B * S + r] = io_ids[s];
+}
+
+}
+
+IIT_EXPORT int iit_ioi_batch_gather(const void* perm, long perm_stride, const void* tb, const void* ta, long P,
+                                    const void* prompts, const void* io_ids, long N, int B, int S, void* out,
+                                    void* stream) {
+  if (B < 1 || S < 1 || N < 1 || P < 1 || (perm && perm_stride < 1) || (!perm && P < B)) return (int)hipErrorInvalidValue;
+  const long n = 2L * B * (S + 1);
+  hipLaunchKernelGGL(ioi_batch_gather_kernel, dim3((unsigned)((n + 255) / 256)), dim3(256), 0, (hipStream_t)stream,
+                     (const long*)perm, perm_stride, (const long*)tb, (const long*)ta, P, (const long*)prompts,
+                     (const long*)io_ids, N, B, S, (long*)out);
+  return hipGetLastError();
 }
 
 IIT_EXPORT int iit_ioi_hl_label(const void* base, const void* src, const float* name_table, int table_n, int B, int S,
diff --git a/csrc/kernels.hip b/csrc/kernels.hip
--- a/csrc/kernels.hip
+++ b/csrc/kernels.hip
@@ -309,7 +309,7 @@
 }
 
 __global__ __launch_bounds__(1024) void ce_fwd_kernel(const float* __restrict__ logits, long ld, const long* __restrict__ labels,
-                                                      float* __restrict__ loss, float* __restrict__ lse_out,
+                                                      long lab_stride, float* __restrict__ loss, float* __restrict__ lse_out,
                                                       long* __restrict__ amax, int V) {
   __shared__ float sm_m[16], sm_s[16];
   __shared__ int sm_i[16];
@@ -342,14 +342,15 @@
     for (int j = 1; j < 16; ++j) online_merge(m, s, mi, sm_m[j], sm_s[j], sm_i[j]);
     const float l = m + __logf(s);
     if (lse_out) lse_out[row] = l;
-    if (loss && labels) loss[row] = l - x[labels[row]];
+    if (loss && labels) loss[row] = l - x[labels[(long)row * lab_stride]];
     if (amax) amax[row] = mi;
   }
 }
 
-IIT_EXPORT int iit_ce_fwd(const float* logits, long ld, const long* labels, float* loss, float* lse, long* amax, int R,
-                          int V, void* stream) {
-  hipLaunchKernelGGL(ce_fwd_kernel, dim3(R), dim3(1024), 0, (hipStream_t)stream, logits, ld, labels, loss, lse, amax, V);
+IIT_EXPORT int iit_ce_fwd(const float* logits, long ld, const long* labels, long lab_stride, float* loss, float* lse,
+                          long* amax, int R, int V, void* stream) {
+  hipLaunchKernelGGL(ce_fwd_kernel, dim3(R), dim3(1024), 0, (hipStream_t)stream, logits, ld, labels, lab_stride, loss,
+                     lse, amax, V);
   return hipGetLastError();
 }
 
@@ -357,14 +358,15 @@
 __global__ __launch_bounds__(256) void ce_bwd_kernel(const float* __restrict__ logits, long ld, const long* __restrict__ labels,
                                                      const float* __restrict__ lse, const float* __restrict__ gscale,
                                                      float inv_rows, OUT* __restrict__ out, long ld_out, int V,
-                                                     __bf16* __restrict__ out16) {
+                                                     __bf16* __restrict__ out16, float weight, long lab_stride) {
   const int row = blockIdx.y;
   const int i = blockIdx.x * 256 + threadIdx.x;
   if (i >= ld_out) return;
   float v = 0.f;
   if (i < V) {
     const float p = __expf(logits[(long)row * ld + i] - lse[row]);
-    v = (p - (i == labels[row] ? 1.f : 0.f)) * gscale[0] * inv_rows;
+    const float gs = gscale[0] * weight;
+    v = (p - (i == labels[(long)row * lab_stride] ? 1.f : 0.f)) * gs * inv_rows;
   }
   out[(long)row * ld_out + i] = (OUT)v;
   if (out16) out16[(long)row * ld_out + i] = f2bf(v);
@@ -372,14 +374,14 @@
 
 IIT_EXPORT int iit_ce_bwd(const float* logits, long ld, const long* labels, const float* lse, const float* gscale,
                           float inv_rows, void* out, long ld_out, int R, int V, int out_bf16, void* out16,
-                          void* stream) {
+                          float weight, long lab_stride, void* stream) {
   dim3 grid((unsigned)((ld_out + 255) / 256), R);
   if (out_bf16)
     hipLaunchKernelGGL(ce_bwd_kernel<__bf16>, grid, dim3(256), 0, (hipStream_t)stream, logits, ld, labels, lse, gscale,
-                       inv_rows, (__bf16*)out, ld_out, V, (__bf16*)nullptr);
+                       inv_rows, (__bf16*)out, ld_out, V, (__bf16*)nullptr, weight, lab_stride);
   else
     hipLaunchKernelGGL(ce_bwd_kernel<float>, grid, dim3(256), 0, (hipStream_t)stream, logits, ld, labels, lse, gscale,
-                       inv_rows, (float*)out, ld_out, V, (__bf16*)out16);
+                       inv_rows, (float*)out, ld_out, V, (__bf16*)out16, weight, lab_stride);
   return hipGetLastError();
 }
 
@@ -387,13 +389,14 @@
 __global__ __launch_bounds__(256) void ce_bwd16_kernel(const float* __restrict__ logits, long ld,
                                                        const long* __restrict__ labels, const float* __restrict__ lse,
                                                        const float* __restrict__ gscale, float inv_rows,
-                                                       __bf16* __restrict__ out16, long ld_out, int V) {
+                                                       __bf16* __restrict__ out16, long ld_out, int V, float weight,
+                                                       long lab_stride) {
   const int row = blockIdx.y;
   const int c0 = (blockIdx.x * 256 + threadIdx.x) * 8;
   if (c0 >= ld_out) return;
   const float* x = logits + (long)row * ld;
-  const float l = lse[row], gs = gscale[0];
-  const long lab = labels[row];
+  const float l = lse[row], gs = gscale[0] * weight;
+  const long lab = labels[(long)row * lab_stride];
   float v[8];
   if (VEC && c0 + 8 <= V) {
     const float4 a = *(const float4*)(x + c0), b = *(const float4*)(x + c0 + 4);
@@ -417,16 +420,17 @@
 }
 
 IIT_EXPORT int iit_ce_bwd16(const float* logits, long ld, const long* labels, const float* lse, const float* gscale,
-                            float inv_rows, void* out16, long ld_out, int R, int V, void* stream) {
+                            float inv_rows, void* out16, long ld_out, int R, int V, float weight, long lab_stride,
+                            void* stream) {
   if (R <= 0 || V <= 0 || ld < V || ld_out < V || ld_out % 8 || ((uintptr_t)out16 & 15)) return (int)hipErrorInvalidValue;
   dim3 grid((unsigned)((ld_out / 8 + 255) / 256), R);
   const bool vec = (((uintptr_t)logits | (uintptr_t)(ld * 4)) & 15) == 0;
   if (vec)
     hipLaunchKernelGGL(ce_bwd16_kernel<true>, grid, dim3(256), 0, (hipStream_t)stream, logits, ld, labels, lse, gscale,
-                       inv_rows, (__bf16*)out16, ld_out, V);
+                       inv_rows, (__bf16*)out16, ld_out, V, weight, lab_stride);
   else
     hipLaunchKernelGGL(ce_bwd16_kernel<false>, grid, dim3(256), 0, (hipStream_t)stream, logits, ld, labels, lse,
-                       gscale, inv_rows, (__bf16*)out16, ld_out, V);
+                       gscale, inv_rows, (__bf16*)out16, ld_out, V, weight, lab_stride);
   return hipGetLastError();
 }
 
diff --git a/iit_amd/data/iit_dataset.py b/iit_amd/data/iit_dataset.py
--- a/iit_amd/data/iit_dataset.py
+++ b/iit_amd/data/iit_dataset.py
@@ -28,6 +28,15 @@
 
         return f
     return None
+
+
+def _pair_root(ds):
+    table = None
+    while isinstance(ds, Subset):
+        idx = torch.as_tensor(list(ds.indices), dtype=torch.long)
+        table = idx if table is None else idx.index_select(0, table)
+        ds = ds.dataset
+    return (ds, table) if hasattr(ds, "gather_pair") else None
 
 
 def _dist_info() -> Tuple[int, int]:
@@ -121,6 +130,7 @@
         self._abl_gather = _gather_fn(dataset.ablation_data)
         self._unique = isinstance(dataset, IITUniqueDataset)
         self._tables = None
+        self._pair = None
 
     def _device_tables(self):
         if self._tables is None:
@@ -130,6 +140,24 @@
                 b, a = self.dataset.pair_table()
                 self._tables = (torch.as_tensor(b).to(self.device), torch.as_tensor(a).to(self.device))
         return self._tables
+
+    def _pair_tables(self):
+        if self._pair is None:
+            self._pair = False
+            roots = None if self._unique else (_pair_root(self.dataset.base_data), _pair_root(self.dataset.ablation_data))
+            if roots and roots[0] and roots[1] and roots[0][0] is roots[1][0]:
+                wrapper = roots[0][0]
+                dev = getattr(getattr(wrapper, "prompts", None), "device", None)
+                if dev is not None and dev.type == self.device.type and self.device.index in (None, dev.index):
+                    tabs = []
+                    for pt, (_, sub) in zip(self.dataset.pair_table(), roots):
+                        t = torch.as_tensor(pt, dtype=torch.long)
+                        t = t if sub is None else sub.index_select(0, t)
+                        if t.numel() == 0 or int(t.min()) < 0 or int(t.max()) >= len(wrapper):
+                            raise IndexError("pair table points outside the dataset")
+                        tabs.append(t.to(dev))
+                    self._pair = (wrapper, tabs[0], tabs[1])
+        return self._pair or None
 
     @property
     def global_batch(self) -> int:
@@ -159,8 +187,11 @@
                 if chunk.numel() < self.world:
                     break
                 chunk = torch.tensor_split(chunk, self.world)[self.rank]
+            pair = None if self._unique else self._pair_tables()
             if self._unique:
                 yield self._base_gather(chunk)
+            elif pair is not None and pair[0].pair_native():
+                yield pair[0].gather_pair(pair[1], pair[2], chunk)
             else:
                 yield (self._base_gather(base_t.index_select(0, chunk)),
                        self._abl_gather(abl_t.index_select(0, chunk)))
diff --git a/iit_amd/engine/graphs.py b/iit_amd/engine/graphs.py
--- a/iit_amd/engine/graphs.py
+++ b/iit_amd/engine/graphs.py
@@ -62,6 +62,18 @@
             pass
     for d, s_ in zip(dst, src):
         d.copy_(s_, non_blocking=True)
+
+
+def _packed(ts) -> Optional[torch.Tensor]:
+    t0 = ts[0]
+    off = t0.storage_offset()
+    for t in ts:
+        if (t.dtype != t0.dtype or t.device != t0.device or not t.is_contiguous() or t.storage_offset() != off
+                or t.untyped_storage().data_ptr() != t0.untyped_storage().data_ptr()):
+            return None
+        off += t.numel()
+    return t0.new_empty(0).set_(t0.untyped_storage(), t0.storage_offset(), (off - t0.storage_offset(),))
+
 
 class _CaptureGC:
 
@@ -210,6 +222,7 @@
             from ..ops.gemm_dispatch import select_graph_safe_blas
             select_graph_safe_blas()
         self._static = None
+        self._static_flat = None
         self._sig = None
         self.captures = 0
         self.replays = 0
@@ -221,14 +234,29 @@
         if not self.enabled:
             return base, abl, True
         sig = tuple((tuple(t.shape), t.dtype, t.device) for t in tuple(base) + tuple(abl))
+        from ..ops.glue import NativeGlue
+        flat = _packed(tuple(base) + tuple(abl)) if NativeGlue.enabled(base[0].device) else None
         if self._static is None:
-            self._static = (tuple(t.clone() for t in base), tuple(t.clone() for t in abl))
+            if flat is not None:
+                self._static_flat = flat.clone()
+                views, o = [], 0
+                for t in tuple(base) + tuple(abl):
+                    views.append(self._static_flat[o:o + t.numel()].view(t.shape))
+                    o += t.numel()
+                self._static = (tuple(views[:len(base)]), tuple(views[len(base):]))
+            else:
+                self._static = (tuple(t.clone() for t in base), tuple(t.clone() for t in abl))
             self._sig = sig
             return self._static[0], self._static[1], False
         if sig != self._sig:
             return base, abl, True
         sb, sa = self._static
-        _copy_all(sb + sa, tuple(base) + tuple(abl))
+        one = flat is not None and self._static_flat is not None and flat.numel() == self._static_flat.numel()
+        NativeGlue.count("stage_copy", one)
+        if one:
+            self._static_flat.copy_(flat, non_blocking=True)
+        else:
+            _copy_all(sb + sa, tuple(base) + tuple(abl))
         return sb, sa, False
 
     @staticmethod
diff --git a/iit_amd/model_pairs/base_model_pair.py b/iit_amd/model_pairs/base_model_pair.py
--- a/iit_amd/model_pairs/base_model_pair.py
+++ b/iit_amd/model_pairs/base_model_pair.py
@@ -346,7 +346,8 @@
         if reducer is not None:
             reducer.start()
         with trace_range("backward"):
-            loss.backward()
+            from ..ops.glue import NativeGlue
+            loss.backward(gradient=NativeGlue.unit_grad(loss))
         sync_point()
         if reducer is not None:
             with trace_range("grad_allreduce"):
diff --git a/iit_amd/model_pairs/iit_behavior_model_pair.py b/iit_amd/model_pairs/iit_behavior_model_pair.py
--- a/iit_amd/model_pairs/iit_behavior_model_pair.py
+++ b/iit_amd/model_pairs/iit_behavior_model_pair.py
@@ -64,15 +64,22 @@
         self.clip_grad_fn(optimizer)
         self.optimizer_step(optimizer)
 
+    @staticmethod
+    def weighted_loss(loss_fn, weight):
+        if getattr(getattr(loss_fn, "__func__", loss_fn), "takes_weight", False):
+            return lambda output, target: loss_fn(output, target, weight=weight)
+        return lambda output, target: loss_fn(output, target) * weight
+
     def run_train_step(self, base_input, ablation_input, loss_fn, optimizer):
         args = self.training_args
         hl_node = self.sample_hl_name()
 
         def iit():
-            return self.get_IIT_loss_over_batch(base_input, ablation_input, hl_node, loss_fn) * args["iit_weight"]
+            return self.get_IIT_loss_over_batch(base_input, ablation_input, hl_node,
+                                                self.weighted_loss(loss_fn, args["iit_weight"]))
 
         def behavior():
-            return self.get_behaviour_loss_over_batch(base_input, loss_fn) * args["behavior_weight"]
+            return self.get_behaviour_loss_over_batch(base_input, self.weighted_loss(loss_fn, args["behavior_weight"]))
 
         if args["use_single_loss"]:
             def total():
diff --git a/iit_amd/model_pairs/ioi_model_pair.py b/iit_amd/model_pairs/ioi_model_pair.py
--- a/iit_amd/model_pairs/ioi_model_pair.py
+++ b/iit_amd/model_pairs/ioi_model_pair.py
@@ -41,7 +41,12 @@
     def loss_fn(self, value):
         self._loss_fn_override = value
 
-    def per_token_weighted_cross_entropy(self, output: Tensor, target: Tensor) -> Tensor:
+    def per_token_weighted_cross_entropy(self, output: Tensor, target: Tensor, weight=None) -> Tensor:
+        if weight is not None:
+            if output.dim() == 2 and not target.dtype.is_floating_point:
+                from ..ops import cross_entropy
+                return cross_entropy(output.float(), target[:, -1] if target.dim() == 2 else target, weight=weight)
+            return self.per_token_weighted_cross_entropy(output, target) * weight
         output = output.float()
         if output.dim() == 2:
             if target.dim() == 3 or (target.dim() == 2 and not target.dtype.is_floating_point):
@@ -62,6 +67,8 @@
             w[-1] = 10
             return (per * w).sum() / (w.sum() * B)
         return F.cross_entropy(output[:, -1, :], target[:, -1])
+
+    per_token_weighted_cross_entropy.takes_weight = True
 
     @staticmethod
     def get_label_idxs():
diff --git a/iit_amd/model_pairs/strict_iit_model_pair.py b/iit_amd/model_pairs/strict_iit_model_pair.py
--- a/iit_amd/model_pairs/strict_iit_model_pair.py
+++ b/iit_amd/model_pairs/strict_iit_model_pair.py
@@ -46,17 +46,23 @@
         args = self.training_args
         hl_node = self.sample_hl_name()
 
+        wl = self.weighted_loss
+
         def iit():
-            return self.get_IIT_loss_over_batch(base_input, ablation_input, hl_node, loss_fn) * args["iit_weight"]
+            return self.get_IIT_loss_over_batch(base_input, ablation_input, hl_node, wl(loss_fn, args["iit_weight"]))
+
+        def strict(ll_node):
+            return self.get_strict_loss_over_batch(base_input, ablation_input, ll_node,
+                                                   wl(loss_fn, args["strict_weight"]))
+
+        def behavior():
+            return self.get_behaviour_loss_over_batch(base_input, wl(loss_fn, args["behavior_weight"]))
 
         if args["use_single_loss"]:
             ll_node = self.sample_ll_node()
 
             def total():
-                parts = {"iit": iit(),
-                         "strict": self.get_strict_loss_over_batch(base_input, ablation_input, ll_node, loss_fn)
-                         * args["strict_weight"],
-                         "behavior": self.get_behaviour_loss_over_batch(base_input, loss_fn) * args["behavior_weight"]}
+                parts = {"iit": iit(), "strict": strict(ll_node), "behavior": behavior()}
                 return parts["iit"] + parts["behavior"] + parts["strict"], parts
 
             _, parts = self.run_phase(("single", hl_node.name, ll_node.name, repr(ll_node.index)), total, optimizer,
@@ -65,11 +71,7 @@
                     "train/strict_loss": parts["strict"]}
         iit_loss = self.run_phase(("iit", hl_node.name), iit, optimizer, self.step_on_loss)
         ll_node = self.sample_ll_node()
-        strict_loss = self.run_phase(
-            ("strict", ll_node.name, repr(ll_node.index)),
-            lambda: self.get_strict_loss_over_batch(base_input, ablation_input, ll_node, loss_fn) * args["strict_weight"],
-            optimizer, self.step_on_loss)
-        behavior_loss = self.run_phase(
-            ("behavior",), lambda: self.get_behaviour_loss_over_batch(base_input, loss_fn) * args["behavior_weight"],
-            optimizer, self.step_on_loss)
+        strict_loss = self.run_phase(("strict", ll_node.name, repr(ll_node.index)), lambda: strict(ll_node), optimizer,
+                                     self.step_on_loss)
+        behavior_loss = self.run_phase(("behavior",), behavior, optimizer, self.step_on_loss)
         return {"train/iit_loss": iit_loss, "train/behavior_loss": behavior_loss, "train/strict_loss": strict_loss}
diff --git a/iit_amd/ops/__init__.py b/iit_amd/ops/__init__.py
--- a/iit_amd/ops/__init__.py
+++ b/iit_amd/ops/__init__.py
@@ -47,8 +47,9 @@
     raise ValueError(f"unknown op backend {backend}")
 
 
-def cross_entropy(logits: torch.Tensor, target: torch.Tensor) -> torch.Tensor:
+def cross_entropy(logits: torch.Tensor, target: torch.Tensor, weight=None) -> torch.Tensor:
     if logits.is_cuda and logits.dim() == 2 and not target.dtype.is_floating_point:
         from .hip_ops import cross_entropy as _hip_ce
-        return _hip_ce(logits, target)
-    return torch.nn.functional.cross_entropy(logits.float(), target)
+        return _hip_ce(logits, target, weight)
+    loss = torch.nn.functional.cross_entropy(logits.float(), target)
+    return loss if weight is None else loss * weight
diff --git a/iit_amd/ops/glue.py b/iit_amd/ops/glue.py
--- /dev/null
+++ b/iit_amd/ops/glue.py
@@ -0,0 +1,37 @@
+from __future__ import annotations
+
+import os
+
+
+class NativeGlue:
+    calls: dict = {}
+    _units: dict = {}
+
+    @classmethod
+    def unit_grad(cls, loss):
+        import torch
+        if not (cls.enabled(loss.device) and loss.dim() == 0 and loss.is_floating_point()):
+            return None
+        key = (loss.device, loss.dtype)
+        one = cls._units.get(key)
+        if one is None:
+            if torch.cuda.is_current_stream_capturing():
+                return None
+            one = cls._units[key] = torch.ones((), dtype=loss.dtype, device=loss.device)
+        return one
+
+    @classmethod
+    def count(cls, piece: str, native: bool) -> None:
+        key = piece if native else piece + "_fallback"
+        cls.calls[key] = cls.calls.get(key, 0) + 1
+
+    @staticmethod
+    def mode() -> str:
+        m = os.environ.get("IIT_NATIVE_GLUE", "auto")
+        if m not in ("auto", "0", "1"):
+            raise ValueError(f"IIT_NATIVE_GLUE must be auto, 0 or 1 (got {m!r})")
+        return m
+
+    @classmethod
+    def enabled(cls, device) -> bool:
+        return cls.mode() != "0" and getattr(device, "type", str(device).split(":")[0]) == "cuda"
diff --git a/iit_amd/ops/hip_kernels.py b/iit_amd/ops/hip_kernels.py
--- a/iit_amd/ops/hip_kernels.py
+++ b/iit_amd/ops/hip_kernels.py
@@ -62,13 +62,14 @@
     "iit_attn_mfma_fwd_spec": [c_void_p] * 3 + [c_int] * 4 + [c_long, c_long, c_float, c_int, c_int, c_void_p,
                                                                c_void_p],
     "iit_attn_mfma_bwd_spec": [c_void_p] * 4 + [c_int] * 4 + [c_long, c_long, c_float, c_int, c_void_p, c_void_p],
-    "iit_ce_fwd": [c_void_p, c_long, c_void_p, c_void_p, c_void_p, c_void_p, c_int, c_int, c_void_p],
+    "iit_ce_fwd": [c_void_p, c_long, c_void_p, c_long, c_void_p, c_void_p, c_void_p, c_int, c_int, c_void_p],
     "iit_ce_bwd": [c_void_p, c_long, c_void_p, c_void_p, c_void_p, c_float, c_void_p, c_long, c_int, c_int, c_int,
-                   c_void_p, c_void_p],
+                   c_void_p, c_float, c_long, c_void_p],
     "iit_gemm_glds_edge_ok": [c_void_p] * 4 + [c_long] * 3 + [c_int] * 6,
     "iit_gemm_glds_edge": [c_void_p] * 4 + [c_long] * 3 + [c_int] * 7 + [c_void_p, c_void_p, c_int, c_void_p],
     "iit_gemm_edge_plan": [c_int, c_int, c_long, c_int, c_int, c_void_p],
-    "iit_ce_bwd16": [c_void_p, c_long, c_void_p, c_void_p, c_void_p, c_float, c_void_p, c_long, c_int, c_int, c_void_p],
+    "iit_ce_bwd16": [c_void_p, c_long, c_void_p, c_void_p, c_void_p, c_float, c_void_p, c_long, c_int, c_int, c_float,
+                     c_long, c_void_p],
     "iit_adam_flat": [c_void_p] * 6 + [c_int, c_void_p, c_int] + [c_float] * 6 + [c_void_p] * 3
                      + [c_void_p, c_int, c_void_p, c_void_p],
     "iit_sumsq_2d": [c_void_p, c_long, c_int, c_int, c_void_p, c_void_p],
@@ -122,6 +123,8 @@
                      + [c_int] * 5 + [c_void_p] * 3 + [c_void_p, c_long, c_void_p, c_long, c_int, c_void_p],
     "iit_gemm_glds_set_group_m": [c_int],
     "iit_ioi_hl_label": [c_void_p, c_void_p, c_void_p, c_int, c_int, c_int, c_int, c_int, c_void_p, c_void_p],
+    "iit_ioi_batch_gather": [c_void_p, c_long, c_void_p, c_void_p, c_long, c_void_p, c_void_p, c_long, c_int, c_int,
+                             c_void_p, c_void_p],
     "iit_tile_table": [c_int, c_void_p, c_int],
     "iit_conv2d_ok": [c_long] + [c_int] * 12,
     "iit_conv2d": [c_void_p] * 4 + [c_long] + [c_int] * 12 + [c_void_p] * 4,
@@ -1173,25 +1176,32 @@
            "swiglu_bwd")
 
 
-def ce_fwd(logits, ld, labels, loss, lse, amax, R, V):
+def ce_fwd(logits, ld, labels, loss, lse, amax, R, V, *, lab_stride: int = 1):
     if CHECK_BOUNDS:
         _bounds("ce_fwd", ("logits", logits, R, V, ld))
-    _check(lib().iit_ce_fwd(_p(logits), ld, _p(labels), _p(loss), _p(lse), _p(amax), R, V, _stream()), "ce_fwd")
-
-
-def ce_bwd(logits, ld, labels, lse, gscale, inv_rows, out, ld_out, R, V, out16=None):
-    if CHECK_BOUNDS:
-        _bounds("ce_bwd", ("logits", logits, R, V, ld), ("out", out, R, V, ld_out))
+        if labels is not None:
+            _bounds("ce_fwd", ("labels", labels, R, 1, lab_stride))
+    _check(lib().iit_ce_fwd(_p(logits), ld, _p(labels), lab_stride, _p(loss), _p(lse), _p(amax), R, V, _stream()),
+           "ce_fwd")
+
+
+def ce_bwd(logits, ld, labels, lse, gscale, inv_rows, out, ld_out, R, V, out16=None, *, weight: float = 1.0,
+           lab_stride: int = 1):
+    if CHECK_BOUNDS:
+        _bounds("ce_bwd", ("logits", logits, R, V, ld), ("out", out, R, V, ld_out), ("labels", labels, R, 1, lab_stride))
     _check(lib().iit_ce_bwd(_p(logits), ld, _p(labels), _p(lse), _p(gscale), inv_rows, _p(out), ld_out, R, V,
-                            int(out.dtype == torch.bfloat16), _p(out16), _stream()), "ce_bwd")
-
-
-def ce_bwd16(logits, ld, labels, lse, gscale, inv_rows, out16, ld_out, R, V):
+                            int(out.dtype == torch.bfloat16), _p(out16), float(weight), lab_stride, _stream()),
+           "ce_bwd")
+
+
+def ce_bwd16(logits, ld, labels, lse, gscale, inv_rows, out16, ld_out, R, V, *, weight: float = 1.0,
+             lab_stride: int = 1):
     assert logits.dtype == torch.float32 and out16.dtype == torch.bfloat16 and gscale.dtype == torch.float32
     if CHECK_BOUNDS:
-        _bounds("ce_bwd16", ("logits", logits, R, V, ld), ("out16", out16, R, ld_out, ld_out))
+        _bounds("ce_bwd16", ("logits", logits, R, V, ld), ("out16", out16, R, ld_out, ld_out),
+                ("labels", labels, R, 1, lab_stride))
     _check(lib().iit_ce_bwd16(_p(logits), ld, _p(labels), _p(lse), _p(gscale), inv_rows, _p(out16), ld_out, R, V,
-                              _stream()), "ce_bwd16")
+                              float(weight), lab_stride, _stream()), "ce_bwd16")
 
 
 def colsum_accum(x, ld, out, T, N):
@@ -1284,6 +1294,23 @@
                                   _stream()), "ioi_hl_label")
 
 
+def ioi_batch_gather(perm, tb, ta, prompts, io_ids, B: int, out) -> None:
+    N, W = prompts.shape
+    ts = (tb, ta, prompts, io_ids, out) + (() if perm is None else (perm,))
+    assert all(t.dtype == torch.long and t.is_cuda and t.device == out.device for t in ts)
+    assert prompts.is_contiguous() and io_ids.is_contiguous() and tb.is_contiguous() and ta.is_contiguous()
+    assert out.is_contiguous() and out.numel() >= 2 * B * (2 * W - 1) and io_ids.numel() == N and W >= 2
+    assert tb.dim() == 1 and ta.numel() == tb.numel()
+    if perm is None:
+        assert tb.numel() >= B
+        stride = 1
+    else:
+        assert perm.dim() == 1 and perm.numel() == B
+        stride = max(int(perm.stride(0)), 1)
+    _check(lib().iit_ioi_batch_gather(_p(perm), stride, _p(tb), _p(ta), tb.numel(), _p(prompts), _p(io_ids), N, B,
+                                      W - 1, _p(out), _stream()), "ioi_batch_gather")
+
+
 def gemm_glds_set_prof(buf) -> None:
     lib().iit_gemm_glds_set_prof(_p(buf))
 
diff --git a/iit_amd/ops/hip_ops.py b/iit_amd/ops/hip_ops.py
--- a/iit_amd/ops/hip_ops.py
+++ b/iit_amd/ops/hip_ops.py
@@ -1104,7 +1104,7 @@
 class CrossEntropyFn(Function):
 
     @staticmethod
-    def forward(ctx, logits, labels, handle=None):
+    def forward(ctx, logits, labels, handle=None, weight=None):
         ctx.set_materialize_grads(False)
         R, V = logits.shape
         if logits.stride(1) != 1:
@@ -1112,30 +1112,41 @@
         ld = logits.stride(0)
         loss = torch.empty(R, dtype=F32, device=logits.device)
         lse = torch.empty(R, dtype=F32, device=logits.device)
-        lab = labels.contiguous()
-        K.ce_fwd(logits, ld, lab, loss, lse, None, R, V)
+        ctx.only16 = handle is not None
+        ctx.weight = 1.0
+        if weight is None:
+            lab = labels.contiguous()
+            ctx.lab_stride = 1
+            K.ce_fwd(logits, ld, lab, loss, lse, None, R, V)
+            ctx.save_for_backward(logits, lab, lse)
+            return loss.mean()
+        lab = labels if labels.dim() == 1 and labels.dtype == torch.long else labels.reshape(-1).long()
+        ctx.lab_stride = int(lab.stride(0)) if R > 1 else 1
+        ctx.weight = float(weight)
+        K.ce_fwd(logits, ld, lab, loss, lse, None, R, V, lab_stride=ctx.lab_stride)
         ctx.save_for_backward(logits, lab, lse)
-        ctx.only16 = handle is not None
-        return loss.mean()
+        mean = loss.mean()
+        return mean if ctx.weight == 1.0 else mean * ctx.weight
 
     @staticmethod
     def backward(ctx, g):
         if g is None:
-            return None, None, None
+            return None, None, None, None
         logits, lab, lse = ctx.saved_tensors
         R, V = logits.shape
         ld = logits.stride(0)
         ldo = _pad8(V)
         buf16 = torch.empty(R, ldo, dtype=BF16, device=logits.device)
         gs = g.reshape(1).float().contiguous()
+        kw = dict(weight=ctx.weight, lab_stride=ctx.lab_stride)
         if ctx.only16:
-            K.ce_bwd16(logits, ld, lab, lse, gs, 1.0 / R, buf16, ldo, R, V)
-            return None, None, buf16[:, :V]
+            K.ce_bwd16(logits, ld, lab, lse, gs, 1.0 / R, buf16, ldo, R, V, **kw)
+            return None, None, buf16[:, :V], None
         buf = torch.empty(R, ldo, dtype=F32, device=logits.device)
-        K.ce_bwd(logits, ld, lab, lse, gs, 1.0 / R, buf, ldo, R, V, out16=buf16)
+        K.ce_bwd(logits, ld, lab, lse, gs, 1.0 / R, buf, ldo, R, V, out16=buf16, **kw)
         res = buf[:, :V]
         _set_bf16_twin(res, buf16[:, :V])
-        return res, None, None
+        return res, None, None, None
 
 
 def _grad16_handle(logits: torch.Tensor) -> Optional[torch.Tensor]:
@@ -1149,13 +1160,19 @@
     return tag[2]
 
 
-def cross_entropy(logits: torch.Tensor, labels: torch.Tensor) -> torch.Tensor:
+def cross_entropy(logits: torch.Tensor, labels: torch.Tensor, weight=None) -> torch.Tensor:
+    from .glue import NativeGlue
     logits = logits.float()
+    native = NativeGlue.enabled(logits.device) and labels.dim() == 1 and labels.shape[0] == logits.shape[0]
+    NativeGlue.count("ce_scalars", native)
+    fold = (1.0 if weight is None else float(weight)) if native else None
     handle = _grad16_handle(logits) if logits.dim() == 2 else None
     if handle is not None:
         logits._iit_grad16 = None
-        return CrossEntropyFn.apply(logits.detach(), labels, handle)
-    return CrossEntropyFn.apply(logits, labels)
+        loss = CrossEntropyFn.apply(logits.detach(), labels, handle, fold)
+    else:
+        loss = CrossEntropyFn.apply(logits, labels, None, fold)
+    return loss if native or weight is None else loss * weight
 
 
 
diff --git a/iit_amd/tasks/ioi/ioi_dataset.py b/iit_amd/tasks/ioi/ioi_dataset.py
--- a/iit_amd/tasks/ioi/ioi_dataset.py
+++ b/iit_amd/tasks/ioi/ioi_dataset.py
@@ -101,3 +101,30 @@
     def gather(self, idx: torch.Tensor):
         p = self.prompts.index_select(0, idx.to(self.prompts.device))
         return p[:, :-1], self._labels(p[:, 1:]), self.io_ids.index_select(0, idx.to(self.prompts.device))[:, None]
+
+    def pair_native(self) -> bool:
+        from ...ops.glue import NativeGlue
+        return self.label_format == "index" and NativeGlue.enabled(self.prompts.device) and len(self) > 0
+
+    def gather_pair(self, base_idx: torch.Tensor, abl_idx: torch.Tensor, chunk: Optional[torch.Tensor] = None):
+        from ...ops.glue import NativeGlue
+        dev = self.prompts.device
+        native = self.pair_native() and all(t is None or (t.dim() == 1 and t.dtype == torch.long and t.device == dev)
+                                            for t in (base_idx, abl_idx, chunk))
+        B = int((base_idx if chunk is None else chunk).numel())
+        native = native and B > 0 and base_idx.numel() == abl_idx.numel()
+        NativeGlue.count("batch_gather", native)
+        if not native:
+            if chunk is not None:
+                base_idx, abl_idx = base_idx.index_select(0, chunk), abl_idx.index_select(0, chunk)
+            return self.gather(base_idx), self.gather(abl_idx)
+        from ...ops import hip_kernels as K
+        S = int(self.prompts.shape[1]) - 1
+        buf = torch.empty(2 * B * (2 * S + 1), dtype=torch.long, device=dev)
+        K.ioi_batch_gather(chunk, base_idx.contiguous(), abl_idx.contiguous(), self.prompts, self.io_ids, B, buf)
+        side = B * (2 * S + 1)
+
+        def views(o):
+            return (buf[o:o + B * S].view(B, S), buf[o + B * S:o + 2 * B * S].view(B, S),
+                    buf[o + 2 * B * S:o + side].view(B, 1))
+        return views(0), views(side)
```
